# alexkeroro86/SampleNeRFRO

Measured on AMD Instinct MI355X. Metric: rays/sec (train step), higher is better.
Workload: dtype f16x3/fp32-acc

## Files before the change

### include/rnerf.h

```cpp
#ifndef RNERF_H_
#define RNERF_H_

#include <stddef.h>
#include <stdint.h>

#ifdef __cplusplus
extern "C" {
#endif

#define RNERF_VERSION 4

enum rnerf_status {
  RNERF_OK = 0,
  RNERF_ERR_ARG = -1,
  RNERF_ERR_HIP = -2,
  RNERF_ERR_UNSUPPORTED = -3
};

enum rnerf_precision {
  RNERF_PREC_F32 = 0,
  RNERF_PREC_F16X3 = 1,
  RNERF_PREC_BF16X3 = 2,
  RNERF_PREC_F16 = 3,
  RNERF_PREC_BF16 = 4,
  RNERF_PREC_F16X2 = 5,
  RNERF_PREC_F16F8 = 6
};

enum rnerf_backward {
  RNERF_BWD_BF16 = 0,
  RNERF_BWD_F16 = 1,
  RNERF_BWD_F16X3 = 2,
  RNERF_BWD_F16X2 = 2,
  RNERF_BWD_F16X3_LO8 = 4
};

typedef struct rnerf_grid {
  int32_t dims[3];
  double nmin[3];
  double nmax[3];
  int32_t layout;
} rnerf_grid;

enum rnerf_table_layout {
  RNERF_TABLE_REFERENCE = 0,
  RNERF_TABLE_BRICKS = 1
};
size_t rnerf_grid_table_floats(const rnerf_grid* g);

#define RNERF_NERFMLP_PARAMS 595844
#define RNERF_BKGDMLP_PARAMS 56963
#define RNERF_SO3MLP_PARAMS 65411

const char* rnerf_last_error(void);
int rnerf_version(void);
int rnerf_device_cus(void);

int rnerf_grid_prefilter(const float* src, float* dst, float* tmp, const int32_t dims[3], int ksize, double ksigma,
                         void* stream);

int rnerf_grid_build_table(const float* grid, float* table, const rnerf_grid* g, void* stream);

int rnerf_grid_query(const float* table, const rnerf_grid* g, const float* pts, int64_t n, float* out, int32_t* idx,
                     void* stream);

int rnerf_march(const float* table, const rnerf_grid* g, const float* origins, const float* viewdirs, int32_t B,
                double near, double far, int32_t num_nodes, float* path_pd, float* path_dr, float* path_ior,
                int32_t* vox, void* stream);

size_t rnerf_nerfmlp_packed_bytes(int precision);
int rnerf_nerfmlp_pack(const float* params, int precision, void* packed, void* stream);

int rnerf_nerfmlp_forward(const void* packed, int precision, const float* rows_pd, const float* rows_dr,
                          const int32_t* node_of_sample, int32_t S, int32_t B, float* out_raw, int32_t max_workgroups, void* stream);

int rnerf_bkgd_forward(const float* params, const float* dirs, int32_t dir_stride, int64_t n, double rgb_padding,
                       float* out_rgb, void* stream);

int rnerf_composite(const float* raw, const float* rows_pd, const float* rows_dr, const int32_t* node_of_sample,
                    int32_t S, int32_t B, const float* bkgd, int white_bkgd, double rgb_padding, double sigma_bias,
                    float* rgb, float* dist, float* acc, float* trans, float* trans_bkgd, float* weights,
                    float* alpha, int mask_mode, const double* bbox, void* stream);

int rnerf_resample(const float* path_pd, const float* path_dr, int32_t num_nodes, int32_t B, const int32_t* jitter,
                   int32_t S, const float* weights, const float* u, int32_t u_per_ray, int32_t num_fine, float* rows_pd,
                   float* rows_dr, int32_t* node_idx, float* scratch, void* stream);

int rnerf_stratified_u(const uint32_t* key, int32_t B, int32_t num_fine, float* u, void* stream);

int rnerf_voxelize(const double* verts, const int32_t* faces, const int32_t* bin_start, const int32_t* bin_tris, int32_t num_bins,
                   const double* bin_origin_size, const rnerf_grid* g, int32_t num_samples, double ior_inside, double ior_outside,
                   int32_t* count, float* out, int32_t* overflow, void* stream);

int rnerf_voxelize_samples(const double* verts, const int32_t* faces, const int32_t* bin_start, const int32_t* bin_tris, int32_t num_bins,
                           const double* bin_origin_size, const rnerf_grid* g, int32_t num_samples, uint8_t* inside, int32_t* overflow, void* stream);
int rnerf_voxelize_majority(const uint8_t* in_z, const uint8_t* in_x, const uint8_t* in_y, int32_t num_voxels, int32_t num_samples,
                            double ior_inside, double ior_outside, int32_t* count, float* out, void* stream);

int rnerf_so3_query(const float* table, const rnerf_grid* g, const float* so3_params, const float* window10, const float* pts,
                    const float* condition, int64_t n, float* out4, float* pred_grad, void* stream);

size_t rnerf_so3_packed_bytes(void);
int rnerf_march_all(const float* table, const rnerf_grid* g, const float* so3_params, void* so3_packed, const float* window10, const float* origins,
                    const float* viewdirs, int32_t B, double near, double far, int32_t num_nodes, float* path_pd, float* path_dr,
                    float* path_ior, const int32_t* ray_order, void* stream);

int rnerf_generate_rays(const float* camtoworld, int32_t opencv, double fx, double fy, double cx, double cy, double pixel_center,
                        int32_t W, int32_t row0, int32_t rows, float* origins, float* directions, float* viewdirs, void* stream);

int rnerf_sample_batch(const float* camtoworlds, int32_t n_img, int32_t opencv, double fx, double fy, double cx, double cy, double pixel_center,
                       int32_t W, int32_t H, const float* images, int32_t channels, const int64_t* ray_indices, int32_t B, float* origins,
                       float* directions, float* viewdirs, float* pixels, int32_t* bad_count, void* stream);

int rnerf_integrated_pos_enc(const float* rows_pd, const float* rows_dr, const int32_t* node_of_sample, int32_t S, int32_t B, const float* radii,
                             double near, int32_t min_deg, int32_t max_deg, float* out_mean4, float* out_cov4, float* out_enc, void* stream);

int rnerf_loss_reduce(const float* rgb_c, const float* rgb_f, const float* trans_f, const float* trans_bkgd_f,
                      const float* pixels, int32_t B, float* sums, void* stream);

size_t rnerf_env_smooth_sum_floats(int32_t ps);
int rnerf_env_smooth_backward(const float* rgb_env, int32_t ps, double grad_scale, float* d_out, float* loss_sum, void* stream);
int rnerf_train_stats(const float* sums, int32_t B, int32_t two_levels, double bg_scale, const float* env_loss_sum, int32_t ps, double env_on,
                      const float* theta, int64_t n_theta, double frozen_sq, int64_t n_all, float* stats8, void* stream);
int rnerf_theta_sumsq(const float* theta, int64_t n_theta, float* stats8, void* stream);

int rnerf_composite_backward(const float* raw, const float* rows_pd, const float* rows_dr, const int32_t* node_of_sample,
                             int32_t S, int32_t B, const float* bkgd, double rgb_padding, double sigma_bias, const float* rgb,
                             const float* pixels, const float* trans, const float* trans_bkgd, const float* sums,
                             double mse_scale, double bg_scale, float* d_raw, float* d_bkgd, int accumulate_bkgd, int white_bkgd,
                             int mask_mode, const double* bbox, void* stream);

size_t rnerf_nerfmlp_save_bytes(int64_t rows, int backward);
size_t rnerf_nerfmlp_dy_bytes(int64_t rows, int backward);
size_t rnerf_nerfmlp_bwd_packed_bytes(void);
size_t rnerf_nerfmlp_wgrad_workspace_bytes(void);
int rnerf_nerfmlp_forward_train(const void* packed, int precision, const float* rows_pd, const float* rows_dr,
                                const int32_t* node_of_sample, int32_t S, int32_t B, float* out_raw, void* save, int backward,
                                int32_t max_workgroups , void* stream);
int rnerf_nerfmlp_pack_bwd(const float* params, int backward, void* packed_bwd, void* stream);
int rnerf_nerfmlp_dgrad(const void* packed_bwd, const void* packed_fwd, int fwd_precision, int backward, const void* save, const float* d_raw,
                        int64_t rows, void* dy, void* stream);
int rnerf_nerfmlp_wgrad(int fwd_precision, int backward, const void* save, const void* dy, int64_t rows, float* grads, void* workspace,
                        void* stream);

size_t rnerf_bkgd_save_bytes(int64_t n);
size_t rnerf_bkgd_dy_bytes(int64_t n);
int rnerf_bkgd_forward_train(const float* params, const float* dirs, int32_t dir_stride, int64_t n, double rgb_padding,
                             float* out_rgb, void* save, void* stream);
int rnerf_bkgd_backward(const float* params, const void* save, const float* d_out, int64_t n, double rgb_padding, void* dy,
                        float* grads, float* d_dirs, void* stream);

int rnerf_march_all_train(const float* table, const rnerf_grid* g, const float* so3_params, void* so3_packed, const float* window10, const float* origins,
                          const float* viewdirs, int32_t B, double near, double far, int32_t num_nodes, float* path_pd, float* path_dr,
                          float* path_rdn, int32_t* pair_count, int32_t pair_cap, int32_t* pair_id, float* pair_x, float* pair_g,
                          int32_t* pair_of_node, const int32_t* ray_order, void* stream);
size_t rnerf_so3_save_bytes(int64_t n);
size_t rnerf_so3_dy_bytes(int64_t nb);
int rnerf_so3_forward_train(const float* so3_params, const float* window10, const float* pts4, int64_t n, void* save, void* stream);
int rnerf_so3_backward(const float* so3_params, const float* window10, const float* pts4, const void* save, int64_t n_save, const float* d_raw4,
                       int64_t nb, void* dy, float* dx4, float* grads, void* stream);
int rnerf_so3_pair_jacobian(const float* table, const rnerf_grid* g, const float* pair_x, const float* pair_g, const float* raw4, const float* J4,
                            int64_t np, float* A12, float* P12, void* stream);
int rnerf_march_adjoint(const float* table, const rnerf_grid* g, const float* path_pd, const float* path_rdn, const int32_t* pair_of_node,
                        const float* A12, const float* P12, const float* a_pos, const float* a_dir, const int32_t* sample_of_node, int32_t B,
                        double near, double far, int32_t num_nodes, float* v4, void* stream);
int rnerf_nerfmlp_input_grad(const float* params, int backward, const void* dy, const float* rows_pd, const float* rows_dr,
                             const int32_t* node_of_sample, int32_t S, int32_t B, float* d_pos4, float* d_dir4, void* stream);


typedef struct rnerf_model {
  const float* table;
  rnerf_grid grid;
  double near, far;
  int32_t num_coarse;
  int32_t num_fine;
  int32_t num_path;
  int32_t precision;
  int32_t white_bkgd;
  int32_t bd_cut;
  double rgb_padding, sigma_bias;
  double bd_cut_bbox[6];
  const void* packed_coarse;
  const void* packed_fine;
  const float* bkgd_params;
} rnerf_model;

#define RNERF_LEVEL_FLOATS 9

int rnerf_rng_split3(uint32_t* rng_state, uint32_t* keys4, void* stream);
int rnerf_rng_forward(const uint32_t* keys4, int32_t num_coarse, int32_t num_path, int32_t use_random_choice, int32_t* jitter, uint32_t* key_u,
                      void* stream);
int rnerf_stratified_u_dev(const uint32_t* key_dev, int32_t B, int32_t num_fine, float* u, void* stream);

size_t rnerf_forward_workspace_bytes(const rnerf_model* m, int32_t B);
int rnerf_forward(const rnerf_model* m, const float* origins, const float* viewdirs, int32_t B, const int32_t* jitter, const float* u_fine,
                  int32_t u_per_ray, const float* path_pd, const float* path_dr, float* out_coarse, float* out_fine, void* workspace,
                  int32_t max_workgroups, void* stream);

typedef struct rnerf_train_cfg {
  int32_t backward;
  int32_t randomized;
  int32_t use_random_choice;
  int32_t bg_patch_size;
  double bg_weight, bg_smooth_weight, annealed_alpha;
  double frozen_sq;
  int64_t frozen_count;
  void* aux_stream;
  void* grads_stream;
} rnerf_train_cfg;
typedef struct rnerf_prefetch {
  const float* origins;
  const float* viewdirs;
  float* path_pd;
  float* path_dr;
  void* side_stream;
} rnerf_prefetch;
size_t rnerf_train_workspace_bytes(const rnerf_model* m, const rnerf_train_cfg* c, int32_t B);
int rnerf_train_forward_backward(const rnerf_model* m, const rnerf_train_cfg* c, const float* theta, const float* origins, const float* viewdirs,
                                 const float* pixels, const float* env_dirs, int32_t B, const uint32_t* keys4, const int32_t* jitter_override,
                                 const float* u_override, int32_t u_per_ray, const float* path_pd, const float* path_dr, float* grads,
                                 void* workspace, int32_t max_workgroups, const rnerf_prefetch* next, void* stream);

#define RNERF_ADAM_SCRATCH_FLOATS 3076
typedef struct rnerf_adam_cfg {
  double lr_init, lr_final, lr_delay_mult;
  int64_t max_steps, lr_delay_steps;
  double b1, b2, eps;
  double weight_decay_mult, grad_max_val, grad_max_norm;
  int64_t n_all;
  double lr_override;
  int32_t use_lr_override;
  int32_t skip_nonfinite;
} rnerf_adam_cfg;
int rnerf_adam_update(const rnerf_adam_cfg* c, float* theta, float* mu, float* nu, float* grads, int64_t n_theta, const float* frozen_params,
                      int64_t n_frozen, int32_t* step_counter, float* scratch, void* stream);
int rnerf_adam_update_fused(const rnerf_adam_cfg* c, float* theta, float* mu, float* nu, float* grads, int64_t n_theta,
                            const float* frozen_params, int64_t n_frozen, int32_t* step_counter, float* scratch, float* nonfinite_out,
                            void* stream);

int rnerf_graph_begin(void* stream);
int rnerf_graph_end(void* stream, void** graph_exec);
int rnerf_graph_launch(void* graph_exec, void* stream);
int rnerf_graph_destroy(void* graph_exec);
int rnerf_fork(void* main_stream, void* side_stream);
int rnerf_join(void* main_stream, void* side_stream);

size_t rnerf_ssim_workspace_bytes(int64_t n, int32_t H, int32_t W, int32_t C, int32_t filter_size);
int rnerf_ssim(const float* img0, const float* img1, int64_t n, int32_t H, int32_t W, int32_t C, int32_t filter_size, double filter_sigma,
               double max_val, double k1, double k2, float* map, float* mean, void* workspace, void* stream);

size_t rnerf_flip_workspace_bytes(int64_t n, int32_t H, int32_t W, double pixels_per_degree);
int rnerf_flip(const float* reference, const float* test, int64_t n, int32_t H, int32_t W, double pixels_per_degree, float* map,
               float* mean, void* workspace, void* stream);

size_t rnerf_visual_hull_workspace_bytes(int64_t num_views, int32_t height, int32_t width);
int rnerf_visual_hull_pack(const uint8_t* masks, int64_t num_views, int32_t height, int32_t width, void* workspace, void* stream);
int rnerf_visual_hull_count(const uint8_t* masks, int64_t num_views, int32_t height, int32_t width, const double* pv, const rnerf_grid* g,
                            int32_t accumulate, int32_t* count, void* workspace, void* stream);
int rnerf_visual_hull_finalize(const int32_t* count, const rnerf_grid* g, int64_t total_views, double threshold, double ior_inside,
                               double ior_outside, float* out, void* stream);

#ifdef __cplusplus
}
#endif
#endif
```

### samplenerfro_amd/_lib.py

```python
from __future__ import annotations

import ctypes as C
import os
from typing import Optional

HERE = os.path.dirname(os.path.abspath(__file__))
LIB_PATH = os.path.join(HERE, "lib", "librnerf.so")

PREC_F32, PREC_F16X3, PREC_BF16X3, PREC_F16, PREC_BF16, PREC_F16X2, PREC_F16F8 = 0, 1, 2, 3, 4, 5, 6
PRECISIONS = {"f32": PREC_F32, "f16x3": PREC_F16X3, "bf16x3": PREC_BF16X3, "f16": PREC_F16, "bf16": PREC_BF16, "f16x2": PREC_F16X2, "f16f8": PREC_F16F8}
BWD_BF16, BWD_F16, BWD_F16X2 = 0, 1, 2
BWD_F16X3 = BWD_F16X2
BWD_F16X3_LO8 = 4
BACKWARDS = {"f16x3": BWD_F16X3, "f16x3lo8": BWD_F16X3_LO8, "f16": BWD_F16, "bf16": BWD_BF16, "f32": BWD_F16X3, "tf32": BWD_F16}
BACKWARD_NAMES = {BWD_F16X3: "f16x3", BWD_F16X3_LO8: "f16x3lo8", BWD_F16: "f16", BWD_BF16: "bf16"}
TWO_PLANE_BACKWARDS = (BWD_F16X3, BWD_F16X3_LO8)
ABI_VERSION = 4
NERFMLP_PARAMS = 595844
BKGDMLP_PARAMS = 56963
SO3MLP_PARAMS = 65411


class RnerfError(RuntimeError):
    pass


TABLE_LAYOUTS = {"reference": 0, "bricks": 1}


class Grid(C.Structure):
    _fields_ = [("dims", C.c_int32 * 3), ("nmin", C.c_double * 3), ("nmax", C.c_double * 3), ("layout", C.c_int32)]

    @classmethod
    def make(cls, ndim, nmin, nmax, layout="reference") -> "Grid":
        g = cls()
        for i in range(3):
            g.dims[i] = int(ndim[i]); g.nmin[i] = float(nmin[i]); g.nmax[i] = float(nmax[i])
        g.layout = TABLE_LAYOUTS[layout] if isinstance(layout, str) else int(layout)
        return g


class Model(C.Structure):
    _fields_ = [("table", C.c_void_p), ("grid", Grid), ("near", C.c_double), ("far", C.c_double), ("num_coarse", C.c_int32),
                ("num_fine", C.c_int32), ("num_path", C.c_int32), ("precision", C.c_int32), ("white_bkgd", C.c_int32), ("bd_cut", C.c_int32),
                ("rgb_padding", C.c_double), ("sigma_bias", C.c_double), ("bd_cut_bbox", C.c_double * 6), ("packed_coarse", C.c_void_p),
                ("packed_fine", C.c_void_p), ("bkgd_params", C.c_void_p)]


class TrainCfg(C.Structure):
    _fields_ = [("backward", C.c_int32), ("randomized", C.c_int32), ("use_random_choice", C.c_int32), ("bg_patch_size", C.c_int32),
                ("bg_weight", C.c_double), ("bg_smooth_weight", C.c_double), ("annealed_alpha", C.c_double), ("frozen_sq", C.c_double),
                ("frozen_count", C.c_int64), ("aux_stream", C.c_void_p), ("grads_stream", C.c_void_p)]


class AdamCfg(C.Structure):
    _fields_ = [("lr_init", C.c_double), ("lr_final", C.c_double), ("lr_delay_mult", C.c_double), ("max_steps", C.c_int64),
                ("lr_delay_steps", C.c_int64), ("b1", C.c_double), ("b2", C.c_double), ("eps", C.c_double), ("weight_decay_mult", C.c_double),
                ("grad_max_val", C.c_double), ("grad_max_norm", C.c_double), ("n_all", C.c_int64), ("lr_override", C.c_double),
                ("use_lr_override", C.c_int32), ("skip_nonfinite", C.c_int32)]


class Prefetch(C.Structure):
    _fields_ = [("origins", C.c_void_p), ("viewdirs", C.c_void_p), ("path_pd", C.c_void_p), ("path_dr", C.c_void_p), ("side_stream", C.c_void_p)]


LEVEL_FLOATS = 9
ADAM_SCRATCH_FLOATS = 3076
_vp, _i32, _i64, _dbl = C.c_void_p, C.c_int32, C.c_int64, C.c_double
_GP = C.POINTER(Grid)
_MP, _TP, _AP = C.POINTER(Model), C.POINTER(TrainCfg), C.POINTER(AdamCfg)

SIGNATURES = {
    "rnerf_last_error": (C.c_char_p, []),
    "rnerf_version": (C.c_int, []),
    "rnerf_device_cus": (C.c_int, []),
    "rnerf_grid_prefilter": (C.c_int, [_vp, _vp, _vp, C.POINTER(_i32 * 3), C.c_int, _dbl, _vp]),
    "rnerf_grid_table_floats": (C.c_size_t, [_GP]),
    "rnerf_grid_build_table": (C.c_int, [_vp, _vp, _GP, _vp]),
    "rnerf_grid_query": (C.c_int, [_vp, _GP, _vp, _i64, _vp, _vp, _vp]),
    "rnerf_march": (C.c_int, [_vp, _GP, _vp, _vp, _i32, _dbl, _dbl, _i32, _vp, _vp, _vp, _vp, _vp]),
    "rnerf_nerfmlp_packed_bytes": (C.c_size_t, [C.c_int]),
    "rnerf_nerfmlp_pack": (C.c_int, [_vp, C.c_int, _vp, _vp]),
    "rnerf_nerfmlp_forward": (C.c_int, [_vp, C.c_int, _vp, _vp, _vp, _i32, _i32, _vp, _i32, _vp]),
    "rnerf_bkgd_forward": (C.c_int, [_vp, _vp, _i32, _i64, _dbl, _vp, _vp]),
    "rnerf_composite": (C.c_int, [_vp, _vp, _vp, _vp, _i32, _i32, _vp, C.c_int, _dbl, _dbl,
                                  _vp, _vp, _vp, _vp, _vp, _vp, _vp, C.c_int, C.POINTER(C.c_double * 6), _vp]),
    "rnerf_loss_reduce": (C.c_int, [_vp, _vp, _vp, _vp, _vp, _i32, _vp, _vp]),
    "rnerf_env_smooth_sum_floats": (C.c_size_t, [_i32]),
    "rnerf_env_smooth_backward": (C.c_int, [_vp, _i32, _dbl, _vp, _vp, _vp]),
    "rnerf_train_stats": (C.c_int, [_vp, _i32, _i32, _dbl, _vp, _i32, _dbl, _vp, _i64, _dbl, _i64, _vp, _vp]),
    "rnerf_composite_backward": (C.c_int, [_vp, _vp, _vp, _vp, _i32, _i32, _vp, _dbl, _dbl, _vp, _vp, _vp, _vp, _vp, _dbl, _dbl,
                                           _vp, _vp, C.c_int, C.c_int, C.c_int, C.POINTER(C.c_double * 6), _vp]),
    "rnerf_nerfmlp_save_bytes": (C.c_size_t, [_i64, C.c_int]),
    "rnerf_nerfmlp_dy_bytes": (C.c_size_t, [_i64, C.c_int]),
    "rnerf_nerfmlp_bwd_packed_bytes": (C.c_size_t, []),
    "rnerf_nerfmlp_wgrad_workspace_bytes": (C.c_size_t, []),
    "rnerf_nerfmlp_forward_train": (C.c_int, [_vp, C.c_int, _vp, _vp, _vp, _i32, _i32, _vp, _vp, C.c_int, _i32, _vp]),
    "rnerf_nerfmlp_pack_bwd": (C.c_int, [_vp, C.c_int, _vp, _vp]),
    "rnerf_nerfmlp_dgrad": (C.c_int, [_vp, _vp, C.c_int, C.c_int, _vp, _vp, _i64, _vp, _vp]),
    "rnerf_nerfmlp_wgrad": (C.c_int, [C.c_int, C.c_int, _vp, _vp, _i64, _vp, _vp, _vp]),
    "rnerf_voxelize": (C.c_int, [_vp, _vp, _vp, _vp, _i32, _vp, _GP, _i32, _dbl, _dbl, _vp, _vp, _vp, _vp]),
    "rnerf_voxelize_samples": (C.c_int, [_vp, _vp, _vp, _vp, _i32, _vp, _GP, _i32, _vp, _vp, _vp]),
    "rnerf_voxelize_majority": (C.c_int, [_vp, _vp, _vp, _i32, _i32, _dbl, _dbl, _vp, _vp, _vp]),
    "rnerf_so3_query": (C.c_int, [_vp, _GP, _vp, _vp, _vp, _vp, _i64, _vp, _vp, _vp]),
    "rnerf_march_all": (C.c_int, [_vp, _GP, _vp, _vp, _vp, _vp, _vp, _i32, _dbl, _dbl, _i32, _vp, _vp, _vp, _vp, _vp]),
    "rnerf_generate_rays": (C.c_int, [_vp, _i32, _dbl, _dbl, _dbl, _dbl, _dbl, _i32, _i32, _i32, _vp, _vp, _vp, _vp]),
    "rnerf_sample_batch": (C.c_int, [_vp, _i32, _i32, _dbl, _dbl, _dbl, _dbl, _dbl, _i32, _i32, _vp, _i32, _vp, _i32, _vp, _vp, _vp, _vp, _vp, _vp]),
    "rnerf_stratified_u": (C.c_int, [_vp, _i32, _i32, _vp, _vp]),
    "rnerf_bkgd_save_bytes": (C.c_size_t, [_i64]),
    "rnerf_bkgd_dy_bytes": (C.c_size_t, [_i64]),
    "rnerf_bkgd_forward_train": (C.c_int, [_vp, _vp, _i32, _i64, _dbl, _vp, _vp, _vp]),
    "rnerf_bkgd_backward": (C.c_int, [_vp, _vp, _vp, _i64, _dbl, _vp, _vp, _vp, _vp]),
    "rnerf_theta_sumsq": (C.c_int, [_vp, _i64, _vp, _vp]),
    "rnerf_march_all_train": (C.c_int, [_vp, _GP, _vp, _vp, _vp, _vp, _vp, _i32, _dbl, _dbl, _i32, _vp, _vp, _vp, _vp, _i32, _vp, _vp, _vp, _vp, _vp, _vp]),
    "rnerf_so3_packed_bytes": (C.c_size_t, []),
    "rnerf_so3_save_bytes": (C.c_size_t, [_i64]),
    "rnerf_so3_dy_bytes": (C.c_size_t, [_i64]),
    "rnerf_so3_forward_train": (C.c_int, [_vp, _vp, _vp, _i64, _vp, _vp]),
    "rnerf_so3_backward": (C.c_int, [_vp, _vp, _vp, _vp, _i64, _vp, _i64, _vp, _vp, _vp, _vp]),
    "rnerf_so3_pair_jacobian": (C.c_int, [_vp, _GP, _vp, _vp, _vp, _vp, _i64, _vp, _vp, _vp]),
    "rnerf_march_adjoint": (C.c_int, [_vp, _GP, _vp, _vp, _vp, _vp, _vp, _vp, _vp, _vp, _i32, _dbl, _dbl, _i32, _vp, _vp]),
    "rnerf_nerfmlp_input_grad": (C.c_int, [_vp, C.c_int, _vp, _vp, _vp, _vp, _i32, _i32, _vp, _vp, _vp]),
    "rnerf_resample": (C.c_int, [_vp, _vp, _i32, _i32, _vp, _i32, _vp, _vp, _i32, _i32, _vp, _vp, _vp, _vp, _vp]),
    "rnerf_integrated_pos_enc": (C.c_int, [_vp, _vp, _vp, _i32, _i32, _vp, _dbl, _i32, _i32, _vp, _vp, _vp, _vp]),
    "rnerf_rng_split3": (C.c_int, [_vp, _vp, _vp]),
    "rnerf_rng_forward": (C.c_int, [_vp, _i32, _i32, _i32, _vp, _vp, _vp]),
    "rnerf_stratified_u_dev": (C.c_int, [_vp, _i32, _i32, _vp, _vp]),
    "rnerf_forward_workspace_bytes": (C.c_size_t, [_MP, _i32]),
    "rnerf_forward": (C.c_int, [_MP, _vp, _vp, _i32, _vp, _vp, _i32, _vp, _vp, _vp, _vp, _vp, _i32, _vp]),
    "rnerf_train_workspace_bytes": (C.c_size_t, [_MP, _TP, _i32]),
    "rnerf_train_forward_backward": (C.c_int, [_MP, _TP, _vp, _vp, _vp, _vp, _vp, _i32, _vp, _vp, _vp, _i32, _vp, _vp, _vp, _vp, _i32, C.POINTER(Prefetch), _vp]),
    "rnerf_adam_update": (C.c_int, [_AP, _vp, _vp, _vp, _vp, _i64, _vp, _i64, _vp, _vp, _vp]),
    "rnerf_adam_update_fused": (C.c_int, [_AP, _vp, _vp, _vp, _vp, _i64, _vp, _i64, _vp, _vp, _vp, _vp]),
    "rnerf_graph_begin": (C.c_int, [_vp]),
    "rnerf_graph_end": (C.c_int, [_vp, C.POINTER(C.c_void_p)]),
    "rnerf_graph_launch": (C.c_int, [_vp, _vp]),
    "rnerf_graph_destroy": (C.c_int, [_vp]),
    "rnerf_fork": (C.c_int, [_vp, _vp]),
    "rnerf_join": (C.c_int, [_vp, _vp]),
    "rnerf_ssim_workspace_bytes": (C.c_size_t, [_i64, _i32, _i32, _i32, _i32]),
    "rnerf_ssim": (C.c_int, [_vp, _vp, _i64, _i32, _i32, _i32, _i32, _dbl, _dbl, _dbl, _dbl, _vp, _vp, _vp, _vp]),
    "rnerf_flip_workspace_bytes": (C.c_size_t, [_i64, _i32, _i32, _dbl]),
    "rnerf_flip": (C.c_int, [_vp, _vp, _i64, _i32, _i32, _dbl, _vp, _vp, _vp, _vp]),
    "rnerf_visual_hull_workspace_bytes": (C.c_size_t, [_i64, _i32, _i32]),
    "rnerf_visual_hull_pack": (C.c_int, [_vp, _i64, _i32, _i32, _vp, _vp]),
    "rnerf_visual_hull_count": (C.c_int, [_vp, _i64, _i32, _i32, _vp, _GP, _i32, _vp, _vp, _vp]),
    "rnerf_visual_hull_finalize": (C.c_int, [_vp, _GP, _i64, _dbl, _dbl, _dbl, _vp, _vp]),
}

_lib: Optional[C.CDLL] = None


def load(path: Optional[str] = None) -> C.CDLL:
    global _lib
    if _lib is not None and path is None:
        return _lib
    p = path or LIB_PATH
    if not os.path.exists(p):
        raise RnerfError(f"{p} not found: build it with `python -m samplenerfro_amd.build` "
                         "(there is no CPU fallback for the hot path)")
    lib = C.CDLL(p)
    for name, (res, args) in SIGNATURES.items():
        fn = getattr(lib, name)
        fn.restype = res
        fn.argtypes = args
    got = lib.rnerf_version()
    if got != ABI_VERSION:
        raise RnerfError(f"{p} speaks ABI version {got}, this binding was written for {ABI_VERSION} (include/rnerf.h RNERF_VERSION): rebuild with "
                         "`python -m samplenerfro_amd.build --force`")
    if path is None or _lib is None:
        _lib = lib
    return lib


def check(status: int, what: str = "") -> None:
    if status != 0:
        msg = load().rnerf_last_error()
        raise RnerfError(f"{what} failed ({status}): {msg.decode() if msg else '?'}")


def ptr(t) -> Optional[int]:
    if t is None:
        return None
    return t.data_ptr()


def current_stream() -> int:
    import torch
    return torch.cuda.current_stream().cuda_stream
```

### samplenerfro_amd/csrc/bkgd16.hip

```cpp
#include "mfma_ops.h"
#include "bkgd_layout.h"
#include "so3_layout.h"

namespace rnerf {

__device__ __forceinline__ void bkgd16_split2(float a, float b, uint32_t& hi, uint32_t& lo) { split2<true>(a, b, hi, lo); }
__device__ __forceinline__ void bkgd16_split8(const float (&w)[8], uint4& hi, uint4& lo) {
  uint32_t h[4], l[4];
#pragma unroll
  for (int p = 0; p < 4; ++p) bkgd16_split2(w[2 * p], w[2 * p + 1], h[p], l[p]);
  hi = make_uint4(h[0], h[1], h[2], h[3]); lo = make_uint4(l[0], l[1], l[2], l[3]);
}
template <int NS, bool FIRST, typename WF, typename LF, typename XF>
__device__ __forceinline__ void bkgd16_layer(f32x16 (&acc)[4], WF wload, LF live, bool half0, XF xop) {
  constexpr int DEPTH = 2;
  f32x2 w[DEPTH + 1][16];
  auto load = [&](int s, f32x2 (&dst)[16]) {
#pragma unroll
    for (int t = 0; t < 4; ++t)
#pragma unroll
      for (int j = 0; j < 8; ++j)
        if (live(s, j) != 0) dst[4 * t + (j >> 1)][j & 1] = wload(s, t, j);
  };
#pragma unroll
  for (int s = 0; s < DEPTH && s < NS; ++s) load(s, w[s]);
  f32x16 zero;
#pragma unroll
  for (int r = 0; r < 16; ++r) zero[r] = 0.f;
#pragma unroll
  for (int s = 0; s < NS; ++s) {
    if (s + DEPTH < NS) load(s + DEPTH, w[(s + DEPTH) % (DEPTH + 1)]);
    RNERF_PIN();
    uint4 bh, bl;
    xop(s, bh, bl);
#pragma unroll
    for (int t = 0; t < 4; ++t) {
      uint32_t hh[4], ll[4];
#pragma unroll
      for (int p = 0; p < 4; ++p) {
        const int l0 = live(s, 2 * p), l1 = live(s, 2 * p + 1);
        if (l0 == 0 && l1 == 0) { hh[p] = 0u; ll[p] = 0u; continue; }
        f32x2 q = w[s % (DEPTH + 1)][4 * t + p];
        if (l0 == 0) q[0] = 0.f;
        if (l1 == 0) q[1] = 0.f;
        q = q * 256.0f;
        if (l0 == 2) q[0] = half0 ? q[0] : 0.f;
        if (l1 == 2) q[1] = half0 ? q[1] : 0.f;
        bkgd16_split2(q[0], q[1], hh[p], ll[p]);
      }
      const uint4 ah = make_uint4(hh[0], hh[1], hh[2], hh[3]), al = make_uint4(ll[0], ll[1], ll[2], ll[3]);
      acc[t] = mfma16<true>(ah, bh, FIRST && s == 0 ? zero : acc[t]);
      acc[t] = mfma16<true>(ah, bl, acc[t]);
      acc[t] = mfma16<true>(al, bh, acc[t]);
    }
    RNERF_PIN();
  }
}
struct Bkgd16Lane {
  const float* p0;
  const float* prev;
  const float* dir;
  const float* sp;
  bool half0;
};
__device__ __forceinline__ Bkgd16Lane bkgd16_lane(const float* __restrict__ params, int m, int h) {
  return {params + m, params + m + 4 * 128 * h, params + m + 12 * 128 * h, params + m + 2 * 128 * h, h == 0};
}
template <bool BIAS>
__device__ __forceinline__ void bkgd16_prev_layer(f32x16 (&acc)[4], const f32x16 (&x)[4], const Bkgd16Lane& L, int koff, int boff) {
  bkgd16_layer<BIAS ? 9 : 8, true>(acc,
      [&](int s, int t, int j) { return s < 8 ? L.prev[koff + (16 * s + 8 * (j >> 2) + (j & 3)) * 128 + 32 * t] : L.p0[boff + 32 * t]; },
      [&](int s, int j) { return s < 8 ? 1 : (j == 0 ? 2 : 0); }, L.half0,
      [&](int s, uint4& bh, uint4& bl) {
    if (s < 8) {
      float xv[8];
#pragma unroll
      for (int j = 0; j < 8; ++j) xv[j] = x[s >> 1][8 * (s & 1) + j];
      bkgd16_split8(xv, bh, bl);
    } else {
      bh = make_uint4(L.half0 ? 0x3c00u : 0u, 0u, 0u, 0u);
      bl = make_uint4(0u, 0u, 0u, 0u);
    }
  });
}
template <bool FIRST>
__device__ __forceinline__ void bkgd16_dir_layer(f32x16 (&acc)[4], const float (&enc)[14], const Bkgd16Lane& L, int koff, int boff) {
  bkgd16_layer<2, FIRST>(acc,
      [&](int s, int t, int j) {
        const int q = 8 * s + j;
        return q < 12 ? L.dir[koff + (3 + q) * 128 + 32 * t] : (q == 12 ? L.sp[koff + 32 * t] : (q == 13 ? L.p0[koff + 128 + 32 * t] : L.p0[boff + 32 * t]));
      },
      [&](int s, int j) { const int q = 8 * s + j; return q < 13 ? 1 : (q < 15 ? 2 : 0); }, L.half0,
      [&](int s, uint4& bh, uint4& bl) {
    float xv[8];
#pragma unroll
    for (int j = 0; j < 8; ++j) xv[j] = 8 * s + j < 14 ? enc[8 * s + j] : (8 * s + j == 14 && L.half0 ? 1.0f : 0.f);
    bkgd16_split8(xv, bh, bl);
  });
}

template <bool TRAIN>
__global__ void __launch_bounds__(64) bkgd16_fwd_kernel(const float* __restrict__ params, const float* __restrict__ dirs, int dir_stride,
                                                        long long n, float pad_scale, float pad, float* __restrict__ out_rgb,
                                                        float* __restrict__ save) {
  const int lane = threadIdx.x & 63, m = lane & 31, h = lane >> 5;
  long long row = (long long)blockIdx.x * 32 + m;
  const bool ok = row < n;
  if (!ok) row = n - 1;
  const float v0 = dirs[row * dir_stride], v1 = dirs[row * dir_stride + 1], v2 = dirs[row * dir_stride + 2];
  float enc[14];
  const float phase = h ? 1.5707963705062866f : 0.0f;
#pragma unroll
  for (int q = 0; q < 12; ++q) {
    const int d = q / 3, c = q % 3;
    const float x = c == 0 ? v0 : (c == 1 ? v1 : v2);
    enc[q] = sinf(fadd(fmul(x, (float)(1 << d)), phase));
  }
  enc[12] = h ? v2 : v0;
  enc[13] = h ? 0.f : v1;
  auto save_x = [&](int k, const f32x16 (&xx)[4]) {
    if constexpr (TRAIN) {
      if (ok) {
        float* dst = save + (size_t)n * 28 + (size_t)(k - 1) * n * 128 + (size_t)row * 128;
#pragma unroll
        for (int t = 0; t < 4; ++t)
#pragma unroll
          for (int g = 0; g < 4; ++g)
            *(float4*)(dst + 32 * t + 8 * g + 4 * h) = make_float4(xx[t][4 * g], xx[t][4 * g + 1], xx[t][4 * g + 2], xx[t][4 * g + 3]);
      }
    }
  };
  if constexpr (TRAIN) {
    if (ok) {
#pragma unroll
      for (int q = 0; q < 14; ++q) { const int f = h ? dir_feature(q, 1) : dir_feature(q, 0); if (f >= 0) save[(size_t)row * 28 + f] = enc[q]; }
      if (h == 1) save[(size_t)row * 28 + 27] = 0.f;
    }
  }
  constexpr float INV = 1.0f / 256.0f;
  f32x16 acc[4], x[4];
  auto relu_to_x = [&]() {
#pragma unroll
    for (int t = 0; t < 4; ++t)
#pragma unroll
      for (int r = 0; r < 16; ++r) { const float y = acc[t][r] * INV; x[t][r] = y < 0.f ? 0.f : y; }
  };
  const Bkgd16Lane L = bkgd16_lane(params, m, h);
  bkgd16_dir_layer<true>(acc, enc, L, bkgd_koff(0), bkgd_boff(0));
  relu_to_x();
  save_x(1, x);
  bkgd16_prev_layer<true>(acc, x, L, bkgd_koff(1), bkgd_boff(1));
  relu_to_x();
  save_x(2, x);
  bkgd16_prev_layer<true>(acc, x, L, bkgd_koff(2), bkgd_boff(2));
  relu_to_x();
  save_x(3, x);
  bkgd16_prev_layer<false>(acc, x, L, bkgd_koff(3), 0);
  bkgd16_dir_layer<false>(acc, enc, L, bkgd_koff(3) + 128 * 128, bkgd_boff(3));
  relu_to_x();
  if constexpr (TRAIN) save_x(4, x);
  float o[3] = {0.f, 0.f, 0.f};
  const float* __restrict__ k4 = params + bkgd_koff(4);
#pragma unroll
  for (int t = 0; t < 4; ++t)
#pragma unroll
    for (int r = 0; r < 16; ++r) {
      const float v = x[t][r];
      const int f = 32 * t + (r & 3) + 8 * (r >> 2) + 4 * h;
      o[0] = fmaf(v, k4[f * 3 + 0], o[0]); o[1] = fmaf(v, k4[f * 3 + 1], o[1]); o[2] = fmaf(v, k4[f * 3 + 2], o[2]);
    }
#pragma unroll
  for (int c = 0; c < 3; ++c) {
    o[c] = o[c] + __shfl_xor(o[c], 32) + params[bkgd_boff(4) + c];
    o[c] = fsub(fmul(fdiv(1.0f, fadd(1.0f, expf(-o[c]))), pad_scale), pad);
  }
  if (ok && h == 0) {
    out_rgb[3 * row] = o[0]; out_rgb[3 * row + 1] = o[1]; out_rgb[3 * row + 2] = o[2];
    if constexpr (TRAIN) { float* so = save + (size_t)n * (28 + 4 * 128) + (size_t)row * 3; so[0] = o[0]; so[1] = o[1]; so[2] = o[2]; }
  }
}

int launch_bkgd16_fwd(bool train, const float* params, const float* dirs, int dir_stride, long long n, float pad_scale, float pad, float* out_rgb,
                      float* save, hipStream_t st) {
  const dim3 grid((unsigned)((n + 31) / 32));
  if (train) hipLaunchKernelGGL(bkgd16_fwd_kernel<true>, grid, dim3(64), 0, st, params, dirs, dir_stride, n, pad_scale, pad, out_rgb, save);
  else hipLaunchKernelGGL(bkgd16_fwd_kernel<false>, grid, dim3(64), 0, st, params, dirs, dir_stride, n, pad_scale, pad, out_rgb, save);
  RNERF_CHECK_LAUNCH();
  return RNERF_OK;
}

template <bool FIRST>
__device__ __forceinline__ void so3_16_enc_layer(f32x16 (&acc)[4], const float (&enc)[30], const float* __restrict__ pe, const Bkgd16Lane& L, int koff, int boff) {
  bkgd16_layer<4, FIRST>(acc,
      [&](int s, int t, int j) { const int p = 8 * s + j; return p < 30 ? pe[koff + 2 * p * 128 + 32 * t] : L.p0[boff + 32 * t]; },
      [&](int s, int j) { const int p = 8 * s + j; return p < 30 ? 1 : (p == 30 ? 2 : 0); }, L.half0,
      [&](int s, uint4& bh, uint4& bl) {
    float xv[8];
#pragma unroll
    for (int j = 0; j < 8; ++j) { const int p = 8 * s + j; xv[j] = p < 30 ? enc[p < 30 ? p : 0] : ((p == 30 && L.half0) ? 1.0f : 0.f); }
    bkgd16_split8(xv, bh, bl);
  });
}

__global__ void __launch_bounds__(64) so3_16_fwd_train_kernel(const float* __restrict__ params, So3Window win, const float4* __restrict__ pts, long long n,
                                                              float* __restrict__ save) {
  const int lane = threadIdx.x & 63, m = lane & 31, h = lane >> 5;
  long long row = (long long)blockIdx.x * 32 + m;
  const bool ok = row < n;
  if (!ok) row = n - 1;
  const float4 pt = pts[row];
  float enc[30];
  so3_encode(pt.x, pt.y, pt.z, win, h, enc);
  if (ok) {
#pragma unroll
    for (int p = 0; p < 30; ++p) save[(size_t)row * 60 + 2 * p + h] = enc[p];
  }
  auto save_x = [&](int k, const f32x16 (&xx)[4]) {
    so3_store_mask(save, n, row, k, xx, h, ok);
    if (ok) {
      float* dst = save + (size_t)n * 60 + (size_t)(k - 1) * n * 128 + (size_t)row * 128;
#pragma unroll
      for (int t = 0; t < 4; ++t)
#pragma unroll
        for (int g = 0; g < 4; ++g)
          *(float4*)(dst + 32 * t + 8 * g + 4 * h) = make_float4(xx[t][4 * g], xx[t][4 * g + 1], xx[t][4 * g + 2], xx[t][4 * g + 3]);
    }
  };
  constexpr float INV = 1.0f / 256.0f;
  f32x16 acc[4], x[4];
  auto relu_to_x = [&]() {
#pragma unroll
    for (int t = 0; t < 4; ++t)
#pragma unroll
      for (int r = 0; r < 16; ++r) { const float y = acc[t][r] * INV; x[t][r] = y < 0.f ? 0.f : y; }
  };
  const Bkgd16Lane L = bkgd16_lane(params, m, h);
  const float* __restrict__ pe = params + m + 128 * h;
  so3_16_enc_layer<true>(acc, enc, pe, L, so3_koff(0), so3_boff(0));
  relu_to_x();
  save_x(1, x);
  bkgd16_prev_layer<true>(acc, x, L, so3_koff(1), so3_boff(1));
  relu_to_x();
  save_x(2, x);
  bkgd16_prev_layer<true>(acc, x, L, so3_koff(2), so3_boff(2));
  relu_to_x();
  save_x(3, x);
  bkgd16_prev_layer<false>(acc, x, L, so3_koff(3), 0);
  so3_16_enc_layer<false>(acc, enc, pe, L, so3_koff(3) + 128 * 128, so3_boff(3));
  relu_to_x();
  save_x(4, x);
  float o[3] = {0.f, 0.f, 0.f};
  const float* __restrict__ k4 = params + so3_koff(4);
#pragma unroll
  for (int t = 0; t < 4; ++t)
#pragma unroll
    for (int r = 0; r < 16; ++r) {
      const int f = 32 * t + (r & 3) + 8 * (r >> 2) + 4 * h;
      o[0] = fmaf(x[t][r], k4[f * 3 + 0], o[0]); o[1] = fmaf(x[t][r], k4[f * 3 + 1], o[1]); o[2] = fmaf(x[t][r], k4[f * 3 + 2], o[2]);
    }
#pragma unroll
  for (int c = 0; c < 3; ++c) o[c] = o[c] + __shfl_xor(o[c], 32) + params[so3_boff(4) + c];
  if (ok && h == 0) *(float4*)(save + (size_t)n * (60 + 4 * 128) + (size_t)row * 4) = make_float4(o[0], o[1], o[2], 0.f);
}

int launch_so3_16_fwd_train(const float* params, So3Window win, const float* pts4, long long n, float* save, hipStream_t st) {
  hipLaunchKernelGGL(so3_16_fwd_train_kernel, dim3((unsigned)((n + 31) / 32)), dim3(64), 0, st, params, win, (const float4*)pts4, n, save);
  RNERF_CHECK_LAUNCH();
  return RNERF_OK;
}

}
```

### samplenerfro_amd/csrc/bkgd_layout.h

```cpp
#pragma once
#include "nerfmlp_layout.h"

namespace rnerf {

__host__ __device__ constexpr DenseShape bkgd_dense(int d) {
  constexpr DenseShape t[5] = {{27, 128}, {128, 128}, {128, 128}, {155, 128}, {128, 3}};
  return t[d];
}
__host__ __device__ constexpr int bkgd_koff(int d) {
  int o = 0;
  for (int i = 0; i < d; ++i) o += bkgd_dense(i).in * bkgd_dense(i).out + bkgd_dense(i).out;
  return o;
}
__host__ __device__ constexpr int bkgd_boff(int d) { return bkgd_koff(d) + bkgd_dense(d).in * bkgd_dense(d).out; }
static_assert(bkgd_koff(5) == RNERF_BKGDMLP_PARAMS, "bkgd MLP parameter count");

__host__ __device__ constexpr int dir_feature(int q, int h) { return q < 12 ? (h ? 15 + q : 3 + q) : (q == 12 ? (h ? 2 : 0) : (h ? -1 : 1)); }

__host__ __device__ constexpr size_t bkgd_save_floats(long long n) { return (size_t)n * (28 + 4 * 128 + 3); }
__host__ __device__ constexpr size_t bkgd_dy_floats(long long n) { return (size_t)n * (5 * 128) + (size_t)((n + 255) / 256) * RNERF_BKGDMLP_PARAMS; }

int launch_bkgd16_fwd(bool train, const float* params, const float* dirs, int dir_stride, long long n, float pad_scale, float pad, float* out_rgb,
                      float* save, hipStream_t st);

}
```

### samplenerfro_amd/csrc/mlp.hip

```cpp
#include "common.h"
#include "nerfmlp_layout.h"
#include "mfma_ops.h"
#include "bkgd_layout.h"
#include "so3_layout.h"

#include <stdlib.h>
#include <type_traits>
#include <vector>
#include <stdio.h>

namespace rnerf {


#define GLOBAL_AS __attribute__((address_space(1)))
#define LDS_AS __attribute__((address_space(3)))

struct MfmaLayer { int dense, ks, nt, kind; };
__host__ __device__ constexpr MfmaLayer mfma_layer(int l) {
  constexpr MfmaLayer t[10] = {{0, 4, 8, 0},  {1, 16, 8, 1}, {2, 16, 8, 1}, {3, 16, 8, 1}, {4, 16, 8, 1},
                               {5, 20, 8, 2}, {6, 16, 8, 1}, {7, 16, 8, 1}, {9, 16, 8, 1}, {10, 18, 4, 3}};
  return t[l];
}
__host__ __device__ constexpr int layer_blocks_before(int l) {
  int o = 0;
// ... 1548 lines not shown
    }
    wait_vmcnt<0>();
  }
  constexpr size_t ldn = (size_t)NT * 32;
  const int m = lane & 31, h = lane >> 5;
  if (active) {
#pragma unroll
    for (int i = 0; i < TK; ++i)
#pragma unroll
      for (int j = 0; j < TN; ++j)
#pragma unroll
        for (int r = 0; r < 16; ++r) {
          const int row = (r & 3) + 8 * (r >> 2) + 4 * h;
          pg[(size_t)((wk * TK + i) * 32 + row) * ldn + (wn * TN + j) * 32 + m] = acc[i][j][r];
        }
    if constexpr (SH::EXTRA) {
#pragma unroll
      for (int r = 0; r < 16; ++r) {
        const int row = (r & 3) + 8 * (r >> 2) + 4 * h;
        pg[(size_t)((wk * TK + wn) * 32 + row) * ldn + (NT - 1) * 32 + m] = acce[r];
      }
    }
    const float bsum = accb + __shfl_xor(accb, 32);
    if (wk < TN && h == 0) pbias[(wn * TN + wk) * 32 + m] = bsum;
  }
}

template <int KT, int NT> struct WgTr8 {
  static constexpr int NHI = KT + NT, NLX = (KT + 1) / 2, NLD = (NT + 1) / 2;
  static constexpr int NBLK = NHI + NLX + NLD, NDMA = (NBLK + 7) / 8, STEP_BYTES = (NBLK + 1) * 1024;
  static constexpr int LOX = NHI * 1024, LOD = (NHI + NLX) * 1024, SCALES = NBLK * 1024;
};
constexpr int WGTR8_NBUF = 4;
constexpr int wgtr8_lds_bytes() { return WGTR8_NBUF * WgTr8<10, 8>::STEP_BYTES; }
__device__ __forceinline__ int2v tr_read8b(const char* p) {
  typedef __attribute__((address_space(3))) int2v lds_int2;
  return __builtin_amdgcn_ds_read_tr8_b64_v2i32((lds_int2*)p);
}

template <int KT, int NT>
__device__ __forceinline__ void wgrad_body_tr8(const uint4* __restrict__ saved, const uint4* __restrict__ dy, long long R, float* __restrict__ pg,
                                                float* __restrict__ pbias, const WgTrSegs sg, int g, int G, char* smem) {
  using SH = WgTrShape<KT, NT>;
  using L8 = WgTr8<KT, NT>;
  constexpr int TK = SH::TK, TN = SH::TN;
  constexpr int NHI = L8::NHI, NBLK = L8::NBLK, NDMA = L8::NDMA, STEP_BYTES = L8::STEP_BYTES;
  constexpr int WGTR_NBUF = WGTR8_NBUF, AHEAD = WGTR_NBUF - 1;
  const int tid = threadIdx.x, lane = tid & 63;
  const int wave = __builtin_amdgcn_readfirstlane(tid >> 6);
  const int wk = wave / SH::WN, wn = wave % SH::WN;
  const bool active = wave < SH::WK * SH::WN;
  const float* __restrict__ rs = (const float*)(dy + dy_plane_uint4(R, 2));
  const float mref = rs[R];
  const float inv_mref = mref > 0.f ? 1.0f / mref : 0.f;
  auto x_slots = [&](int t, int& s0, int& s1) { s0 = t < sg.KTa ? sg.qx + 2 * t : sg.qx2 + 2 * (t - sg.KTa); s1 = s0 + 1; };
  auto d_slots = [&](int nt, int& s0, int& s1) {
    const int rel = nt < sg.NTa ? 2 * nt : 2 * (nt - sg.NTa);
    const int qb = nt < sg.NTa ? sg.qd : sg.qd2, ks = nt < sg.NTa ? sg.KSd : sg.KSd2;
    s0 = qb + (rel < ks ? rel : ks - 1);
    s1 = qb + (rel + 1 < ks ? rel + 1 : ks - 1);
  };
  const char* sbase[NDMA];
  unsigned tstride[NDMA], hstride[NDMA], voff[NDMA], lds_blk[NDMA];
#pragma unroll
  for (int i = 0; i < NDMA; ++i) {
    int b = wave + 8 * i;
    b = b < NBLK ? b : NBLK - 1;
    lds_blk[i] = (unsigned)b * 1024u;
    if (b < NHI) {
      const int r = lane >> 2, a = (lane >> 1) & 1, h = lane & 1;
      int s0, s1;
      const bool is_x = b < KT;
      if (is_x) x_slots(b, s0, s1); else d_slots(b - KT, s0, s1);
      sbase[i] = (const char*)((is_x ? saved : dy) + sv_addr(__builtin_amdgcn_readfirstlane(s0), 0, 0, 0));
      voff[i] = (unsigned)((sv_addr(a ? __builtin_amdgcn_readfirstlane(s1 - s0) : 0, 0, r, h)) * sizeof(uint4));
      tstride[i] = (unsigned)((is_x ? SAVE_SLOTS : DY_SLOTS) * 64 * sizeof(uint4));
      hstride[i] = (unsigned)(32 * sizeof(uint4));
    } else {
      const int lb = b - NHI;
      const bool is_x = lb < L8::NLX;
      const int t0 = 2 * (is_x ? lb : lb - L8::NLX) + (lane >> 5);
      const int r = (lane & 31) >> 1, a = lane & 1;
      int s0, s1;
      if (is_x) x_slots(t0 < KT ? t0 : KT - 1, s0, s1); else d_slots(t0 < NT ? t0 : NT - 1, s0, s1);
      sbase[i] = is_x ? (const char*)(saved + sv_lo0(R)) : (const char*)(dy + dy_plane_uint4(R, 1));
      voff[i] = (unsigned)(((a ? s1 : s0) * 32 + r) * 16);
      tstride[i] = (unsigned)((is_x ? SAVE_SLOTS : DY_SLOTS) * 32 * 16);
      hstride[i] = 16u * 16u;
    }
  }
  const float* rs_src = rs + 4 * (lane & 3);
  const long long n_t32 = R / 32;
  const int my_tiles = g < n_t32 ? (int)((n_t32 - 1 - g) / G) + 1 : 0;
  const int n_steps = 2 * my_tiles;
  auto issue = [&](int s) {
    const int sc = s < n_steps ? s : n_steps - 1;
    const size_t t32 = (size_t)g + (size_t)(sc >> 1) * G;
    const unsigned ring = (unsigned)(s % WGTR_NBUF) * STEP_BYTES;
#pragma unroll
    for (int i = 0; i < NDMA; ++i)
      glds16_nt_s(sbase[i] + t32 * tstride[i] + (sc & 1) * hstride[i], voff[i], __builtin_amdgcn_readfirstlane(ring + lds_blk[i]));
    if (wave == 0) glds16_nt((const char*)(rs_src + t32 * 32 + (sc & 1) * 16), __builtin_amdgcn_readfirstlane(ring + L8::SCALES));
  };
  const f32x16 zero = {0, 0, 0, 0, 0, 0, 0, 0, 0, 0, 0, 0, 0, 0, 0, 0};
  f32x16 acc[TK][TN], acce = zero;
  float accb = 0.f;
#pragma unroll
  for (int i = 0; i < TK; ++i)
#pragma unroll
    for (int j = 0; j < TN; ++j) acc[i][j] = zero;
  if (n_steps > 0) {
#pragma unroll
    for (int s = 0; s < AHEAD; ++s) issue(s);
    const unsigned lane_off = (unsigned)((8 * (lane >> 5) + ((lane & 15) >> 2)) * 64 + ((lane >> 4) & 1) * 32 + (lane & 3) * 8);
    const unsigned lane_off8 = (unsigned)((8 * (lane >> 5) + ((lane & 15) >> 1)) * 32 + ((lane >> 4) & 1) * 16 + (lane & 1) * 8);
    const int kh = lane >> 5;
    for (int s = 0; s < n_steps; ++s) {
      if (wave == 0) wait_vmcnt<(AHEAD - 1) * (NDMA + 1)>(); else
      wait_vmcnt<(AHEAD - 1) * NDMA>();
      __syncthreads();
      issue(s + AHEAD);
      if (active) {
        const char* ring0 = smem + (s % WGTR_NBUF) * STEP_BYTES;
        const char* ring = ring0 + lane_off;
        const char* ring8 = ring0 + lane_off8;
        const float4 s0 = *(const float4*)(ring0 + L8::SCALES + kh * 32), s1 = *(const float4*)(ring0 + L8::SCALES + kh * 32 + 16);
        const half8 sc8 = {(_Float16)(s0.x * inv_mref), (_Float16)(s0.y * inv_mref), (_Float16)(s0.z * inv_mref), (_Float16)(s0.w * inv_mref),
                           (_Float16)(s1.x * inv_mref), (_Float16)(s1.y * inv_mref), (_Float16)(s1.z * inv_mref), (_Float16)(s1.w * inv_mref)};
        half8 beh, bel;
        if constexpr (SH::EXTRA) {
          beh = tr_read8(ring + (KT + NT - 1) * 1024);
          bel = lo8_decode(tr_read8b(ring8 + L8::LOD + (NT - 1) * 512), LO8_SCALE_D);
        }
        static_assert(SH::WK >= TN, "bias owners");
        auto read_a = [&](int i, half8& h, half8& l) {
          const int t = wk * TK + i;
          h = tr_read8(ring + t * 1024) * sc8;
          l = lo8_decode(tr_read8b(ring8 + L8::LOX + t * 512), LO8_SCALE_X) * sc8;
        };
        auto read_b = [&](int j, half8& h, half8& l) {
          const int nt = wn * TN + j;
          h = tr_read8(ring + (KT + nt) * 1024);
          l = lo8_decode(tr_read8b(ring8 + L8::LOD + nt * 512), LO8_SCALE_D);
        };
        auto dot8 = [&](const half8& x, float c) -> float {
#pragma unroll
          for (int k = 0; k < 4; ++k) c = __builtin_amdgcn_fdot2(half2v{sc8[2 * k], sc8[2 * k + 1]}, half2v{x[2 * k], x[2 * k + 1]}, c, false);
          return c;
        };
        auto bias_row = [&](int j, const half8& h, const half8& l) {
          if (wk == j) { accb = dot8(h, accb); accb = dot8(l, accb); }
        };
        half8 ae_h, ae_l;
        if constexpr (TK > TN) {
          half8 bh[TN], bl[TN];
#pragma unroll
          for (int j = 0; j < TN; ++j) read_b(j, bh[j], bl[j]);
          half8 an_h, an_l;
          read_a(0, an_h, an_l);
#pragma unroll
          for (int i = 0; i < TK; ++i) {
            const half8 ah = an_h, al = an_l;
            if (i + 1 < TK) read_a(i + 1, an_h, an_l);
#pragma unroll
            for (int j = 0; j < TN; ++j) acc[i][j] = mfma_h8(ah, bh[j], acc[i][j]);
#pragma unroll
            for (int j = 0; j < TN; ++j) acc[i][j] = mfma_h8(ah, bl[j], acc[i][j]);
#pragma unroll
            for (int j = 0; j < TN; ++j) acc[i][j] = mfma_h8(al, bh[j], acc[i][j]);
          }
#pragma unroll
          for (int j = 0; j < TN; ++j) bias_row(j, bh[j], bl[j]);
        } else {
          constexpr int NCH = WGTR_NCH < TN ? WGTR_NCH : TN;
          static_assert(TN % NCH == 0, "n-tile chunks");
          half8 ah[TK], al[TK];
#pragma unroll
          for (int i = 0; i < TK; ++i) read_a(i, ah[i], al[i]);
#pragma unroll
          for (int c = 0; c < TN / NCH; ++c) {
            half8 bh[NCH], bl[NCH];
#pragma unroll
            for (int jj = 0; jj < NCH; ++jj) read_b(c * NCH + jj, bh[jj], bl[jj]);
#pragma unroll
            for (int i = 0; i < TK; ++i)
#pragma unroll
              for (int jj = 0; jj < NCH; ++jj) acc[i][c * NCH + jj] = mfma_h8(ah[i], bh[jj], acc[i][c * NCH + jj]);
#pragma unroll
            for (int i = 0; i < TK; ++i)
#pragma unroll
              for (int jj = 0; jj < NCH; ++jj) acc[i][c * NCH + jj] = mfma_h8(ah[i], bl[jj], acc[i][c * NCH + jj]);
#pragma unroll
            for (int i = 0; i < TK; ++i)
#pragma unroll
              for (int jj = 0; jj < NCH; ++jj) acc[i][c * NCH + jj] = mfma_h8(al[i], bh[jj], acc[i][c * NCH + jj]);
#pragma unroll
            for (int jj = 0; jj < NCH; ++jj) bias_row(c * NCH + jj, bh[jj], bl[jj]);
          }
          if constexpr (SH::EXTRA) { ae_h = wn ? ah[1] : ah[0]; ae_l = wn ? al[1] : al[0]; }
        }
        if constexpr (SH::EXTRA) {
          static_assert(!SH::EXTRA || TK <= TN, "the extra tile reads the resident A fragments");
          acce = mfma_h8(ae_h, beh, acce);
          acce = mfma_h8(ae_h, bel, acce);
          acce = mfma_h8(ae_l, beh, acce);
        }
      }
    }
    wait_vmcnt<0>();
  }
  constexpr size_t ldn = (size_t)NT * 32;
  const int m = lane & 31, h = lane >> 5;
  if (active) {
#pragma unroll
    for (int i = 0; i < TK; ++i)
#pragma unroll
      for (int j = 0; j < TN; ++j)
#pragma unroll
        for (int r = 0; r < 16; ++r) {
          const int row = (r & 3) + 8 * (r >> 2) + 4 * h;
          pg[(size_t)((wk * TK + i) * 32 + row) * ldn + (wn * TN + j) * 32 + m] = acc[i][j][r];
        }
    if constexpr (SH::EXTRA) {
#pragma unroll
      for (int r = 0; r < 16; ++r) {
        const int row = (r & 3) + 8 * (r >> 2) + 4 * h;
        pg[(size_t)((wk * TK + wn) * 32 + row) * ldn + (NT - 1) * 32 + m] = acce[r];
      }
    }
    const float bsum = accb + __shfl_xor(accb, 32);
    if (wk < TN && h == 0) pbias[(wn * TN + wk) * 32 + m] = bsum;
  }
}

constexpr int WGRAD_VGPRS = 112;
template <int NP>
__global__ void __launch_bounds__(512) __attribute__((amdgpu_num_vgpr(WGRAD_VGPRS)))
nerfmlp_wgrad_tr_kernel(const uint4* __restrict__ saved, const uint4* __restrict__ dy, long long R, float* __restrict__ workspace, const WgradTable tab,
                        long long* __restrict__ trace) {
  extern __shared__ __attribute__((aligned(16))) char smem[];
  if (trace && threadIdx.x == 0) trace[2 * blockIdx.x] = (long long)__builtin_amdgcn_s_memrealtime();
  int j = 0;
  while ((int)blockIdx.x >= tab.wg0[j + 1]) ++j;
  const WgradJob job = tab.job[j];
  const int g = blockIdx.x - tab.wg0[j], G = tab.wg0[j + 1] - tab.wg0[j];
  const int KT = job.KT, NT = job.NT;
  float* pg = workspace + tab.poff[j] + (size_t)g * (size_t)KT * 32 * NT * 32;
  float* pb = workspace + tab.pboff[j] + (size_t)g * NT * 32;
  const WgTrSegs sg = {tab.qx[j], job.KTa, tab.qx2[j], tab.qd[j], job.NTa, tab.KSd[j], tab.qd2[j], tab.KSd2[j]};
#define RNERF_WGRAD_CASE(KT_, NT_)                                                                                                  \
  if (KT == (KT_) && NT == (NT_)) {                                                                                                 \
    wgrad_body_tr<NP, KT_, NT_>(saved, dy, R, pg, pb, sg, g, G, smem);                                                              \
    if (trace && threadIdx.x == 0) trace[2 * blockIdx.x + 1] = (long long)__builtin_amdgcn_s_memrealtime();                         \
    return;                                                                                                                         \
  }
  RNERF_WGRAD_CASE(8, 8) RNERF_WGRAD_CASE(2, 8) RNERF_WGRAD_CASE(10, 8) RNERF_WGRAD_CASE(8, 9) RNERF_WGRAD_CASE(9, 4) RNERF_WGRAD_CASE(4, 1)
#undef RNERF_WGRAD_CASE
  __builtin_trap();
}

__global__ void __launch_bounds__(512) __attribute__((amdgpu_num_vgpr(WGRAD_VGPRS)))
nerfmlp_wgrad_tr8_kernel(const uint4* __restrict__ saved, const uint4* __restrict__ dy, long long R, float* __restrict__ workspace, const WgradTable tab,
                         long long* __restrict__ trace) {
  extern __shared__ __attribute__((aligned(16))) char smem[];
  if (trace && threadIdx.x == 0) trace[2 * blockIdx.x] = (long long)__builtin_amdgcn_s_memrealtime();
  int j = 0;
  while ((int)blockIdx.x >= tab.wg0[j + 1]) ++j;
  const WgradJob job = tab.job[j];
  const int g = blockIdx.x - tab.wg0[j], G = tab.wg0[j + 1] - tab.wg0[j];
  const int KT = job.KT, NT = job.NT;
  float* pg = workspace + tab.poff[j] + (size_t)g * (size_t)KT * 32 * NT * 32;
  float* pb = workspace + tab.pboff[j] + (size_t)g * NT * 32;
  const WgTrSegs sg = {tab.qx[j], job.KTa, tab.qx2[j], tab.qd[j], job.NTa, tab.KSd[j], tab.qd2[j], tab.KSd2[j]};
#define RNERF_WGRAD_CASE(KT_, NT_)                                                                                                  \
  if (KT == (KT_) && NT == (NT_)) {                                                                                                 \
    wgrad_body_tr8<KT_, NT_>(saved, dy, R, pg, pb, sg, g, G, smem);                                                                 \
    if (trace && threadIdx.x == 0) trace[2 * blockIdx.x + 1] = (long long)__builtin_amdgcn_s_memrealtime();                         \
    return;                                                                                                                         \
  }
  RNERF_WGRAD_CASE(8, 8) RNERF_WGRAD_CASE(2, 8) RNERF_WGRAD_CASE(10, 8) RNERF_WGRAD_CASE(8, 9) RNERF_WGRAD_CASE(9, 4) RNERF_WGRAD_CASE(4, 1)
#undef RNERF_WGRAD_CASE
  __builtin_trap();
}

template <bool X_F16>
__global__ void __launch_bounds__(512)
nerfmlp_wgrad_kernel(const uint4* __restrict__ saved, const uint4* __restrict__ dy, long long R, long long total_rows, int n_chunks,
                      float* __restrict__ workspace, const WgradTable tab) {
  extern __shared__ __attribute__((aligned(16))) char smem[];
  int j = 0;
  while ((int)blockIdx.x >= tab.wg0[j + 1]) ++j;
  const int qx = tab.qx[j], KSx = tab.KSx[j], qd = tab.qd[j], KSd = tab.KSd[j];
  const int g = blockIdx.x - tab.wg0[j], G = tab.wg0[j + 1] - tab.wg0[j];
  const int KT = KSx >> 1, NT = (KSd + 1) >> 1;
  float* pg = workspace + tab.poff[j] + (size_t)g * (size_t)KT * 32 * NT * 32;
  float* pb = workspace + tab.pboff[j] + (size_t)g * NT * 32;
#define RNERF_WGRAD_CASE(KT_, KSD_)                                                                                                 \
  if (KSx == 2 * (KT_) && KSd == (KSD_)) { wgrad_body<X_F16, KT_, KSD_>(saved, dy, R, total_rows, n_chunks, pg, pb, qx, qd, g, G, smem); return; }
  RNERF_WGRAD_CASE(8, 16) RNERF_WGRAD_CASE(2, 16) RNERF_WGRAD_CASE(8, 1) RNERF_WGRAD_CASE(8, 8) RNERF_WGRAD_CASE(1, 8) RNERF_WGRAD_CASE(4, 1)
#undef RNERF_WGRAD_CASE
  __builtin_trap();
}

__global__ void __launch_bounds__(256) wgrad_reduce_kernel(const float* __restrict__ workspace, const WgradTable tab, float* __restrict__ grads,
                                                           const float* __restrict__ out_scale) {
  const float osc = out_scale ? *out_scale : 1.0f;
  const int jb = blockIdx.y;
  const WgradJob job = tab.job[jb];
  const int n_wg = tab.wg0[jb + 1] - tab.wg0[jb];
  const float* __restrict__ partial = workspace + tab.poff[jb];
  const float* __restrict__ partial_bias = workspace + tab.pboff[jb];
  const int ldn = job.NT * 32, rows = job.KT * 32;
  const int e = blockIdx.x * blockDim.x + threadIdx.x;
  auto out_feature = [&](int J, int& dense) -> int {
    int nt = J >> 5;
    const int c = J & 31, a = c >> 4, hh = (c >> 3) & 1, j = c & 7;
    const bool segb = nt >= job.NTa;
    const int dkind = segb ? job.dkind2 : job.dkind;
    dense = segb ? job.dense2 : job.dense;
    if (segb) nt -= job.NTa;
    if (dkind == 0) { const int n = prev_feature(2 * nt + a, hh, j); return n < nerf_dense(dense).out ? n : -1; }
    if (a != 0 || hh != 0 || nt != 0) return -1;
    if (dkind == 1) return j == 0 ? 0 : -1;
    return (j >= 1 && j <= 3) ? j - 1 : -1;
  };
  auto sum_over = [&](const float* __restrict__ p, size_t stride) -> float {
    float s0 = 0.f, s1 = 0.f, s2 = 0.f, s3 = 0.f;
    int g = 0;
    for (; g + 4 <= n_wg; g += 4) { s0 += p[(size_t)g * stride]; s1 += p[(size_t)(g + 1) * stride]; s2 += p[(size_t)(g + 2) * stride]; s3 += p[(size_t)(g + 3) * stride]; }
    for (; g < n_wg; ++g) s0 += p[(size_t)g * stride];
    return (s0 + s1) + (s2 + s3);
  };
  if (e < rows * ldn) {
    const int I = e / ldn, J = e % ldn;
    int kt = I >> 5;
    const int c = I & 31, a = c >> 4, hh = (c >> 3) & 1, j = c & 7;
    const bool segb = kt >= job.KTa;
    const int xkind = segb ? job.xkind2 : job.xkind, row_off = segb ? job.row_off2 : job.row_off;
    if (segb) kt -= job.KTa;
    const int s = 2 * kt + a;
    int fin = xkind == 1 ? prev_feature(s, hh, j) : (xkind == 0 ? pe_feature(8 * s + j, hh) : view_feature(8 * s + j, hh));
    int dense;
    const int fout = out_feature(J, dense);
    if (fin >= 0 && fout >= 0) {
      fin += row_off;
      if (fin < nerf_dense(dense).in) grads[nerf_koff(dense) + fin * nerf_dense(dense).out + fout] = sum_over(partial + e, (size_t)rows * ldn) * osc;
    }
  }
  if (job.write_bias && e < ldn) {
    int dense;
    const int fout = out_feature(e, dense);
    if (fout >= 0 && (e >> 5) < job.NTa) grads[nerf_boff(dense) + fout] = sum_over(partial_bias + e, (size_t)ldn) * osc;
    if (job.bias_sigma && e == 0) grads[nerf_boff(8)] = sum_over(partial_bias, (size_t)ldn) * osc;
  }
}

template <int NSTEP, int NT, typename WF, typename XF>
__device__ __forceinline__ void mfma_f32_stream(f32x16* acc, WF wload, XF xop) {
  constexpr int BS = 4, NB = (NSTEP + BS - 1) / BS;
  float w[2][BS * NT];
#pragma unroll
  for (int i = 0; i < BS; ++i)
#pragma unroll
    for (int t = 0; t < NT; ++t) w[0][i * NT + t] = i < NSTEP ? wload(i, t) : 0.f;
#pragma unroll
  for (int b = 0; b < NB; ++b) {
    if (b + 1 < NB) {
#pragma unroll
      for (int i = 0; i < BS; ++i)
#pragma unroll
        for (int t = 0; t < NT; ++t) w[(b + 1) & 1][i * NT + t] = (b + 1) * BS + i < NSTEP ? wload((b + 1) * BS + i, t) : 0.f;
    }
    RNERF_PIN();
#pragma unroll
    for (int i = 0; i < BS; ++i) {
      if (b * BS + i < NSTEP) {
#pragma unroll
        for (int t = 0; t < NT; ++t) acc[t] = __builtin_amdgcn_mfma_f32_32x32x2f32(w[b & 1][i * NT + t], xop(b * BS + i), acc[t], 0, 0, 0);
      }
    }
    RNERF_PIN();
  }
}

template <int NSTEP, int NT, typename WF4, typename XF>
__device__ __forceinline__ void mfma_f32_stream4(f32x16* acc, WF4 wload4, XF xop) {
  static_assert(NSTEP % 4 == 0, "whole batches");
  constexpr int NB = NSTEP / 4;
  float4 w[2][NT];
#pragma unroll
  for (int t = 0; t < NT; ++t) w[0][t] = wload4(0, t);
#pragma unroll
  for (int b = 0; b < NB; ++b) {
    if (b + 1 < NB) {
#pragma unroll
      for (int t = 0; t < NT; ++t) w[(b + 1) & 1][t] = wload4(b + 1, t);
    }
    RNERF_PIN();
#pragma unroll
    for (int i = 0; i < 4; ++i)
#pragma unroll
      for (int t = 0; t < NT; ++t) {
        const float4 q = w[b & 1][t];
        acc[t] = __builtin_amdgcn_mfma_f32_32x32x2f32(i == 0 ? q.x : (i == 1 ? q.y : (i == 2 ? q.z : q.w)), xop(4 * b + i), acc[t], 0, 0, 0);
      }
    RNERF_PIN();
  }
}

__device__ __forceinline__ void small_init_bias(f32x16 (&acc)[4], const float* __restrict__ bias, int h) {
#pragma unroll
  for (int t = 0; t < 4; ++t)
#pragma unroll
    for (int r = 0; r < 16; ++r) acc[t][r] = bias[32 * t + (r & 3) + 8 * (r >> 2) + 4 * h];
}

__device__ __forceinline__ void small_prev_layer(f32x16 (&acc)[4], const f32x16 (&x)[4], const float* __restrict__ kern, int m, int h) {
  const float* __restrict__ kl = kern + 4 * h * 128 + m;
  mfma_f32_stream<64, 4>(acc, [&](int st, int t) { return kl[(32 * (st >> 4) + (st & 3) + 8 * ((st & 15) >> 2)) * 128 + 32 * t]; },
                         [&](int st) { return x[st >> 4][st & 15]; });
}

__device__ __forceinline__ void so3_enc_layer(f32x16 (&acc)[4], const float (&enc)[30], const float* __restrict__ kern, int m, int h) {
  const float* __restrict__ kl = kern + h * 128 + m;
  mfma_f32_stream<30, 4>(acc, [&](int p, int t) { return kl[2 * p * 128 + 32 * t]; }, [&](int p) { return enc[p]; });
}

__device__ __forceinline__ void so3_eval(const float* __restrict__ params, float px, float py, float pz, const So3Window& win, int m, int h,
                                         float (&raw)[3]) {
  float enc[30];
  const float HALF_PI = 1.5707963705062866f;
#pragma unroll
  for (int p = 0; p < 30; ++p) {
    const int d = p / 3, k = p % 3;
    const float x = k == 0 ? (h ? py : px) : (k == 1 ? (h ? px : pz) : (h ? pz : py));
    const float phase = k == 0 ? 0.f : (k == 1 ? (h ? HALF_PI : 0.f) : HALF_PI);
    const float xb = fmul(x, (float)(1 << d));
    enc[p] = fmul(sinf(k == 0 ? xb : fadd(xb, phase)), win.w[d]);
  }
  f32x16 acc[4], x[4];
  small_init_bias(acc, params + so3_boff(0), h);
  so3_enc_layer(acc, enc, params + so3_koff(0), m, h);
#pragma unroll
  for (int t = 0; t < 4; ++t)
#pragma unroll
    for (int r = 0; r < 16; ++r) x[t][r] = fmaxf(acc[t][r], 0.f);
#pragma unroll 1
  for (int l = 1; l <= 2; ++l) {
    small_init_bias(acc, params + (l == 1 ? so3_boff(1) : so3_boff(2)), h);
    small_prev_layer(acc, x, params + (l == 1 ? so3_koff(1) : so3_koff(2)), m, h);
#pragma unroll
    for (int t = 0; t < 4; ++t)
#pragma unroll
      for (int r = 0; r < 16; ++r) x[t][r] = fmaxf(acc[t][r], 0.f);
  }
  small_init_bias(acc, params + so3_boff(3), h);
  small_prev_layer(acc, x, params + so3_koff(3), m, h);
  so3_enc_layer(acc, enc, params + so3_koff(3) + 128 * 128, m, h);
  float o[3] = {0.f, 0.f, 0.f};
  const float* __restrict__ k4 = params + so3_koff(4);
#pragma unroll
  for (int t = 0; t < 4; ++t)
#pragma unroll
    for (int r = 0; r < 16; ++r) {
      const float v = fmaxf(acc[t][r], 0.f);
      const int f = 32 * t + (r & 3) + 8 * (r >> 2) + 4 * h;
      o[0] = fmaf(v, k4[f * 3 + 0], o[0]); o[1] = fmaf(v, k4[f * 3 + 1], o[1]); o[2] = fmaf(v, k4[f * 3 + 2], o[2]);
    }
#pragma unroll
  for (int c = 0; c < 3; ++c) raw[c] = o[c] + __shfl_xor(o[c], 32) + params[so3_boff(4) + c];
}

constexpr int kSo3KSteps = 16;
constexpr int kSo3Blocks = kSo3KSteps * 8;
constexpr float SO3_WSCALE = 256.f;
__host__ __device__ constexpr int so3s_row(int ks, int g, int j, int* layer) {
  const int l = ks < 2 ? 0 : (ks < 6 ? 1 : (ks < 10 ? 2 : 3));
  const int s = ks - (l == 0 ? 0 : (l == 1 ? 2 : (l == 2 ? 6 : 10)));
  *layer = l;
  const bool enc = l == 0 || (l == 3 && s >= 4);
  if (enc) { const int f = 32 * (l == 0 ? s : s - 4) + 8 * g + j; return f < 60 ? (l == 0 ? f : 128 + f) : -1; }
  return 32 * s + (j < 4 ? 4 * g + j : 16 + 4 * g + (j - 4));
}

__global__ void so3_pack16_kernel(const float* __restrict__ params, uint4* __restrict__ packed) {
  const int gid = blockIdx.x * blockDim.x + threadIdx.x;
  if (gid >= kSo3Blocks * 64) return;
  const int blk = gid >> 6, lane = gid & 63;
  const int ks = blk >> 3, t = blk & 7;
  const int n_out = 16 * t + (lane & 15), g = lane >> 4;
  float w[8];
  for (int j = 0; j < 8; ++j) {
    int l = 0;
    const int row = so3s_row(ks, g, j, &l);
    w[j] = row < 0 ? 0.f : params[(l == 0 ? so3_koff(0) : (l == 1 ? so3_koff(1) : (l == 2 ? so3_koff(2) : so3_koff(3)))) + row * 128 + n_out] * SO3_WSCALE;
  }
  uint32_t hi[4], lo[4];
  for (int p = 0; p < 4; ++p) split2<true>(w[2 * p], w[2 * p + 1], hi[p], lo[p]);
  packed[(size_t)blk * 128 + lane] = make_uint4(hi[0], hi[1], hi[2], hi[3]);
  packed[(size_t)blk * 128 + 64 + lane] = make_uint4(lo[0], lo[1], lo[2], lo[3]);
}

struct So3Ops { uint4 h, l; };
__device__ __forceinline__ So3Ops so3_split_ops(const float (&x)[8]) {
  uint32_t hh[4], ll[4];
#pragma unroll
  for (int p = 0; p < 4; ++p) split2<true>(x[2 * p], x[2 * p + 1], hh[p], ll[p]);
  So3Ops o; o.h = make_uint4(hh[0], hh[1], hh[2], hh[3]); o.l = make_uint4(ll[0], ll[1], ll[2], ll[3]);
  return o;
}

struct So3Shared {
  uint4 enc[2][2][64];
  uint4 x[3][4][2][64];
  float4 out[4][16];
  float4 pos[16];
  float bias[4][128];
  float k4[128][4];
  float tail[16];
  int done;
};

typedef float f32x4 __attribute__((ext_vector_type(4)));
__device__ __forceinline__ f32x4 so3_mfma16(const uint4 a, const uint4 b, const f32x4 c) {
  typedef _Float16 h8 __attribute__((ext_vector_type(8)));
  return __builtin_amdgcn_mfma_f32_16x16x32_f16(__builtin_bit_cast(h8, a), __builtin_bit_cast(h8, b), c, 0, 0, 0);
}

__device__ __forceinline__ void so3_shared_init(So3Shared& sh, const float* __restrict__ params, const So3Window& win, int tid) {
  for (int i = tid; i < 4 * 128; i += 256) { const int l = i >> 7, n = i & 127; sh.bias[l][n] = params[(l == 0 ? so3_boff(0) : (l == 1 ? so3_boff(1) : (l == 2 ? so3_boff(2) : so3_boff(3)))) + n]; }
  for (int i = tid; i < 128 * 3; i += 256) sh.k4[i / 3][i % 3] = params[so3_koff(4) + i];
  if (tid < 3) sh.tail[tid] = params[so3_boff(4) + tid];
  if (tid < 10) sh.tail[4 + tid] = win.w[tid];
  if (tid == 0) sh.done = 0;
}

__device__ __forceinline__ void so3_eval_wg(So3Shared& sh, const uint4 (&wh)[kSo3KSteps][2], const uint4 (&wl)[kSo3KSteps][2], int wave, int lane) {
  const int c = lane & 15, g = lane >> 4;
  const float HALF_PI = 1.5707963705062866f;
  const f32x4 zero = {0, 0, 0, 0};
  constexpr float INV = 1.0f / SO3_WSCALE;
  const float4 pt = sh.pos[c];
  {
    const int s = wave >> 1, j0 = 4 * (wave & 1);
    float v[4];
#pragma unroll
    for (int j = 0; j < 4; ++j) {
      const int f = 32 * s + 8 * g + j0 + j;
      const bool in = f < 60;
      const int fc = in ? f : 0;
      const int d = fc / 6, jj = fc - 6 * d, c3 = jj >= 3 ? jj - 3 : jj;
      const float x = c3 == 0 ? pt.x : (c3 == 1 ? pt.y : pt.z);
      const float xb = fmul(x, (float)(1 << d));
      const float e = fmul(pe_sin(jj >= 3 ? fadd(xb, HALF_PI) : xb), sh.tail[4 + d]);
      v[j] = in ? e : 0.f;
    }
    uint32_t h0, l0, h1, l1;
    split2<true>(v[0], v[1], h0, l0); split2<true>(v[2], v[3], h1, l1);
    uint2* eh = (uint2*)&sh.enc[s][0][lane] + (wave & 1);
    uint2* el = (uint2*)&sh.enc[s][1][lane] + (wave & 1);
    *eh = make_uint2(h0, h1); *el = make_uint2(l0, l1);
  }
  __syncthreads();
  f32x4 a0 = zero, a1 = zero;
  auto kstep = [&](int ks, const uint4 bh, const uint4 bl) {
    a0 = so3_mfma16(wh[ks][0], bh, a0); a1 = so3_mfma16(wh[ks][1], bh, a1);
    a0 = so3_mfma16(wh[ks][0], bl, a0); a1 = so3_mfma16(wh[ks][1], bl, a1);
    a0 = so3_mfma16(wl[ks][0], bh, a0); a1 = so3_mfma16(wl[ks][1], bh, a1);
  };
  auto enc_layer = [&](int ks0) {
    uint4 eh[2], el[2];
#pragma unroll
    for (int s = 0; s < 2; ++s) { eh[s] = sh.enc[s][0][lane]; el[s] = sh.enc[s][1][lane]; }
    RNERF_PIN();
#pragma unroll
    for (int s = 0; s < 2; ++s) kstep(ks0 + s, eh[s], el[s]);
  };
  auto hand_over = [&](int l) {
    const float4 b0 = *(const float4*)&sh.bias[l][32 * wave + 4 * g], b1 = *(const float4*)&sh.bias[l][32 * wave + 16 + 4 * g];
    float v[8];
    v[0] = fmaxf(fmaf(a0[0], INV, b0.x), 0.f); v[1] = fmaxf(fmaf(a0[1], INV, b0.y), 0.f); v[2] = fmaxf(fmaf(a0[2], INV, b0.z), 0.f); v[3] = fmaxf(fmaf(a0[3], INV, b0.w), 0.f);
    v[4] = fmaxf(fmaf(a1[0], INV, b1.x), 0.f); v[5] = fmaxf(fmaf(a1[1], INV, b1.y), 0.f); v[6] = fmaxf(fmaf(a1[2], INV, b1.z), 0.f); v[7] = fmaxf(fmaf(a1[3], INV, b1.w), 0.f);
    const So3Ops o = so3_split_ops(v);
    sh.x[l][wave][0][lane] = o.h; sh.x[l][wave][1][lane] = o.l;
  };
  auto layer = [&](int l, int ks0) {
    uint4 bh[4], bl[4];
#pragma unroll
    for (int s = 0; s < 4; ++s) { bh[s] = sh.x[l][s][0][lane]; bl[s] = sh.x[l][s][1][lane]; }
    RNERF_PIN();
    a0 = zero; a1 = zero;
#pragma unroll
    for (int s = 0; s < 4; ++s) kstep(ks0 + s, bh[s], bl[s]);
  };
  enc_layer(0);
  hand_over(0);
  __syncthreads();
  layer(0, 2);
  hand_over(1);
  __syncthreads();
  layer(1, 6);
  hand_over(2);
  __syncthreads();
  layer(2, 10);
  enc_layer(14);
  float o[3] = {0.f, 0.f, 0.f};
#pragma unroll
  for (int j = 0; j < 8; ++j) {
    const int f = 32 * wave + (j < 4 ? 4 * g + j : 16 + 4 * g + (j - 4));
    const float v = fmaxf(fmaf(j < 4 ? a0[j & 3] : a1[j & 3], INV, sh.bias[3][f]), 0.f);
    const float4 k = *(const float4*)&sh.k4[f][0];
    o[0] = fmaf(v, k.x, o[0]); o[1] = fmaf(v, k.y, o[1]); o[2] = fmaf(v, k.z, o[2]);
  }
#pragma unroll
  for (int q = 0; q < 3; ++q) { o[q] = o[q] + __shfl_xor(o[q], 16); o[q] = o[q] + __shfl_xor(o[q], 32); }
  if (g == 0) sh.out[wave][c] = make_float4(o[0], o[1], o[2], 0.f);
  __syncthreads();
}

__device__ __forceinline__ void so3_rotate(const float (&raw)[3], const float (&g)[3], float (&pred)[3]) {
  const float theta = fsqrt(fmaxf(fadd(fadd(fmul(raw[0], raw[0]), fmul(raw[1], raw[1])), fmul(raw[2], raw[2])), 1e-6f));
  const float e[3] = {fdiv(raw[0], theta), fdiv(raw[1], theta), fdiv(raw[2], theta)};
  const float a = fsqrt(fmaxf(fadd(fadd(fmul(g[0], g[0]), fmul(g[1], g[1])), fmul(g[2], g[2])), 1e-6f));
  const float v[3] = {fdiv(g[0], a), fdiv(g[1], a), fdiv(g[2], a)};
  const float ct = cosf(theta), st = sinf(theta);
  const float cr[3] = {fsub(fmul(e[1], v[2]), fmul(e[2], v[1])), fsub(fmul(e[2], v[0]), fmul(e[0], v[2])), fsub(fmul(e[0], v[1]), fmul(e[1], v[0]))};
  const float dot = fadd(fadd(fmul(e[0], v[0]), fmul(e[1], v[1])), fmul(e[2], v[2]));
  const float k = fmul(fsub(1.0f, ct), dot);
#pragma unroll
  for (int c = 0; c < 3; ++c) pred[c] = fmul(a, fadd(fadd(fmul(ct, v[c]), fmul(st, cr[c])), fmul(k, e[c])));
}

__global__ void __launch_bounds__(64) so3_query_kernel(const float4* __restrict__ table, GridParams gp, const float* __restrict__ params,
                                                       So3Window win, const float* __restrict__ pts, const float* __restrict__ cond, long long n,
                                                       float4* __restrict__ out4, float* __restrict__ pred_out) {
  const int lane = threadIdx.x & 63, m = lane & 31, h = lane >> 5;
  long long row = (long long)blockIdx.x * 32 + m;
  const bool ok = row < n;
  if (!ok) row = n - 1;
  const float px = pts[3 * row], py = pts[3 * row + 1], pz = pts[3 * row + 2];
  const float4 c = trilinear(table, gp, px, py, pz, nullptr);
  float raw[3], pred[3];
  so3_eval(params, px, py, pz, win, m, h, raw);
  const float g[3] = {cond ? cond[3 * row] : c.y, cond ? cond[3 * row + 1] : c.z, cond ? cond[3 * row + 2] : c.w};
  so3_rotate(raw, g, pred);
  if (ok && h == 0) { out4[row] = c; pred_out[3 * row] = pred[0]; pred_out[3 * row + 1] = pred[1]; pred_out[3 * row + 2] = pred[2]; }
}

__global__ void __launch_bounds__(256, 1) march_all_kernel(const float4* __restrict__ table4, GridParams gp, const float* __restrict__ params,
                                                          const uint4* __restrict__ packed16, So3Window win, const float* __restrict__ origins, const float* __restrict__ viewdirs,
                                                          int B, float near, float step, int num_nodes, float4* __restrict__ path_pd4,
                                                          float4* __restrict__ path_dr4, float4* __restrict__ path_ior4,
                                                          float4* __restrict__ path_rdn4, int* __restrict__ pair_count, int pair_cap,
                                                          int2* __restrict__ pair_id, float4* __restrict__ pair_x4, float4* __restrict__ pair_g4,
                                                          int* __restrict__ pair_of_node, const int* __restrict__ ray_order) {
  __shared__ So3Shared sh;
  const int lane = threadIdx.x & 63;
// ... 479 lines not shown
  }
  if (with_safe && safe_stream_offset(precision) != 0)
    hipLaunchKernelGGL(nerfmlp_pack_kernel<RNERF_PREC_BF16X3>, dim3(grid), dim3(block), 0, st, params, (char*)packed + safe_stream_offset(precision));
  RNERF_CHECK_LAUNCH();
  return RNERF_OK;
}
}

extern "C" int rnerf_nerfmlp_pack(const float* params, int precision, void* packed, void* stream) {
  RNERF_CHECK_ARG(params && packed, "rnerf_nerfmlp_pack: null pointer");
  RNERF_CHECK_ARG(prec_ok(precision), "rnerf_nerfmlp_pack: unsupported precision %d", precision);
  RNERF_CHECK_ARG(((uintptr_t)packed & 15) == 0, "rnerf_nerfmlp_pack: packed must be 16-byte aligned");
  return nerfmlp_pack_impl(params, precision, packed, true, (hipStream_t)stream, true);
}

constexpr size_t SAVE_QUEUE_BYTES = 8192;
static size_t save_payload_bytes(long long padded, bool with_lo) {
  return (size_t)(SAVE_TOTAL + (with_lo ? SAVE_SLOTS : 0)) * (size_t)padded * 2 * sizeof(uint4);
}

template <int PREC, int MODE = 0, int TRAIN = 0>
static int launch_fwd_mode(const void* packed, const float* rows_pd, const float* rows_dr, const int32_t* node_of_sample, int32_t B,
                           long long total_rows, float* out_raw, hipStream_t st, void* save = nullptr, int max_wg = 0, const float* gate = nullptr,
                           int gate_skip_if = 0) {
  using PP = Prec<PREC>;
  const int n_tiles = (int)((total_rows + 255) / 256);
  int dev = 0, cus = 0;
  RNERF_CHECK_HIP(hipGetDevice(&dev));
  RNERF_CHECK_HIP(hipDeviceGetAttribute(&cus, hipDeviceAttributeMultiprocessorCount, dev));
  const int lim = (max_wg > 0 && max_wg < cus) ? max_wg : cus;
  if constexpr (MODE == 0 && (PREC == RNERF_PREC_F16X3 || PREC == RNERF_PREC_F16F8)) {
    static const bool half_ok = [] { const char* e = RNERF_ENV("RNERF_FWD_HALF_TILES"); return !(e && e[0] == '0'); }();
    if (half_ok && 2 * n_tiles <= lim) {
      const size_t lds1 = 2 * (size_t)PP::SLAB;
      static DeviceOnce attr1_set;
      if (attr1_set.need()) {
        RNERF_CHECK_HIP(hipFuncSetAttribute((const void*)nerfmlp_fwd_kernel<PREC, 0, TRAIN, true>, hipFuncAttributeMaxDynamicSharedMemorySize, (int)lds1));
        attr1_set.set();
      }
      hipLaunchKernelGGL((nerfmlp_fwd_kernel<PREC, 0, TRAIN, true>), dim3(2 * n_tiles), dim3(256), lds1, st, (const char*)packed, (const float4*)rows_pd,
                         (const float4*)rows_dr, node_of_sample, B, total_rows, 2 * n_tiles, (float4*)out_raw, (uint4*)save, (long long)n_tiles * 256,
                         (int*)nullptr, gate, gate_skip_if);
      RNERF_CHECK_LAUNCH();
      return RNERF_OK;
    }
  }
  const int grid = n_tiles < lim ? n_tiles : lim;
  const size_t lds = 2 * (size_t)PP::SLAB + 4 * 32768;
  static DeviceOnce attr_set;
  if (attr_set.need()) {
    RNERF_CHECK_HIP(hipFuncSetAttribute((const void*)nerfmlp_fwd_kernel<PREC, MODE, TRAIN>, hipFuncAttributeMaxDynamicSharedMemorySize, (int)lds));
    attr_set.set();
  }
  int* tileq = nullptr;
  if (TRAIN != 0 && grid < cus && grid < n_tiles) {
    tileq = (int*)((char*)save + save_payload_bytes((long long)n_tiles * 256, TRAIN >= 2));
    RNERF_CHECK_HIP(hipMemsetAsync(tileq, 0, sizeof(int), st));
  }
  hipLaunchKernelGGL((nerfmlp_fwd_kernel<PREC, MODE, TRAIN>), dim3(grid), dim3(256), lds, st, (const char*)packed, (const float4*)rows_pd,
                     (const float4*)rows_dr, node_of_sample, B, total_rows, n_tiles, (float4*)out_raw, (uint4*)save,
                     (long long)n_tiles * 256, tileq, gate, gate_skip_if);
  RNERF_CHECK_LAUNCH();
  return RNERF_OK;
}

template <int PREC>
static int launch_fwd(const void* packed, const float* rows_pd, const float* rows_dr, const int32_t* node_of_sample, int32_t B,
                      long long total_rows, float* out_raw, hipStream_t st, int max_wg, const float* gate = nullptr, int gate_skip_if = 0) {
  return launch_fwd_mode<PREC>(packed, rows_pd, rows_dr, node_of_sample, B, total_rows, out_raw, st, nullptr, max_wg, gate, gate_skip_if);
}

extern "C" int rnerf_nerfmlp_forward(const void* packed, int precision, const float* rows_pd, const float* rows_dr,
                                     const int32_t* node_of_sample, int32_t S, int32_t B, float* out_raw, int32_t max_workgroups,
                                     void* stream) {
  RNERF_CHECK_ARG(packed && rows_pd && rows_dr && out_raw, "rnerf_nerfmlp_forward: null pointer");
  RNERF_CHECK_ARG(max_workgroups >= 0, "rnerf_nerfmlp_forward: max_workgroups must be >= 0");
  RNERF_CHECK_ARG(prec_ok(precision), "rnerf_nerfmlp_forward: unsupported precision %d", precision);
  RNERF_CHECK_ARG(S >= 1 && B >= 1, "rnerf_nerfmlp_forward: need S >= 1 and B >= 1");
  RNERF_CHECK_ARG((((uintptr_t)packed | (uintptr_t)rows_pd | (uintptr_t)rows_dr | (uintptr_t)out_raw) & 15) == 0,
                  "rnerf_nerfmlp_forward: buffers must be 16-byte aligned");
  const long long total = (long long)S * B;
  hipStream_t st = (hipStream_t)stream;
  switch (precision) {
    case RNERF_PREC_F32: return launch_fwd_f32(packed, rows_pd, rows_dr, node_of_sample, B, total, out_raw, st);
    case RNERF_PREC_F16X3:
      RNERF_TRY_(launch_fwd<RNERF_PREC_F16X3>(packed, rows_pd, rows_dr, node_of_sample, B, total, out_raw, st, max_workgroups));
      return launch_fwd_mode<RNERF_PREC_BF16X3, 512>((const char*)packed + safe_stream_offset(precision), rows_pd, rows_dr, node_of_sample, B, total, out_raw, st, nullptr, max_workgroups);
    case RNERF_PREC_F16X2:
      RNERF_TRY_(launch_fwd<RNERF_PREC_F16X2>(packed, rows_pd, rows_dr, node_of_sample, B, total, out_raw, st, max_workgroups));
      return launch_fwd_mode<RNERF_PREC_BF16X3, 512>((const char*)packed + safe_stream_offset(precision), rows_pd, rows_dr, node_of_sample, B, total, out_raw, st, nullptr, max_workgroups);
    case RNERF_PREC_F16F8: {
      const float* flag = (const float*)((const char*)packed + Prec<RNERF_PREC_F16F8>::STREAM_BYTES) + AUX_FLAG;
      RNERF_TRY_(launch_fwd<RNERF_PREC_F16F8>(packed, rows_pd, rows_dr, node_of_sample, B, total, out_raw, st, max_workgroups, flag, 1));
      RNERF_TRY_(launch_fwd<RNERF_PREC_F16X3>((const char*)packed + kF8Fallback, rows_pd, rows_dr, node_of_sample, B, total, out_raw, st, max_workgroups, flag, 0));
      return launch_fwd_mode<RNERF_PREC_BF16X3, 512>((const char*)packed + safe_stream_offset(precision), rows_pd, rows_dr, node_of_sample, B, total, out_raw, st, nullptr, max_workgroups);
    }
    case RNERF_PREC_BF16X3: return launch_fwd<RNERF_PREC_BF16X3>(packed, rows_pd, rows_dr, node_of_sample, B, total, out_raw, st, max_workgroups);
    case RNERF_PREC_F16:
      RNERF_TRY_(launch_fwd<RNERF_PREC_F16>(packed, rows_pd, rows_dr, node_of_sample, B, total, out_raw, st, max_workgroups));
      return launch_fwd_mode<RNERF_PREC_BF16X3, 512>((const char*)packed + safe_stream_offset(precision), rows_pd, rows_dr, node_of_sample, B, total, out_raw, st, nullptr, max_workgroups);
    default: return launch_fwd<RNERF_PREC_BF16>(packed, rows_pd, rows_dr, node_of_sample, B, total, out_raw, st, max_workgroups);
  }
}

static bool bwd_ok(int b) { return b == RNERF_BWD_BF16 || b == RNERF_BWD_F16 || b == RNERF_BWD_F16X2 || b == RNERF_BWD_F16X3_LO8; }
static bool bwd_two_planes(int b) { return b == RNERF_BWD_F16X2 || b == RNERF_BWD_F16X3_LO8; }
static bool train_combo_ok(int precision, int backward) {
  return precision == RNERF_PREC_F16X3 || (precision == RNERF_PREC_F16 && !bwd_two_planes(backward)) ||
         (precision == RNERF_PREC_BF16X3 && backward == RNERF_BWD_BF16);
}
static size_t train_stream_bytes(int precision) {
  return precision == RNERF_PREC_F16 ? Prec<RNERF_PREC_F16>::STREAM_BYTES : (precision == RNERF_PREC_BF16X3 ? Prec<RNERF_PREC_BF16X3>::STREAM_BYTES : Prec<RNERF_PREC_F16X3>::STREAM_BYTES);
}

extern "C" size_t rnerf_nerfmlp_save_bytes(int64_t rows, int backward) {
  const int64_t padded = (rows + 255) / 256 * 256;
  return save_payload_bytes(padded, bwd_two_planes(backward)) + SAVE_QUEUE_BYTES;
}

extern "C" int rnerf_nerfmlp_forward_train(const void* packed, int precision, const float* rows_pd, const float* rows_dr,
                                           const int32_t* node_of_sample, int32_t S, int32_t B, float* out_raw, void* save,
                                           int backward, int32_t max_workgroups, void* stream) {
  RNERF_CHECK_ARG(packed && rows_pd && rows_dr && out_raw && save, "rnerf_nerfmlp_forward_train: null pointer");
  RNERF_CHECK_ARG(max_workgroups >= 0, "rnerf_nerfmlp_forward_train: max_workgroups must be >= 0");
  RNERF_CHECK_ARG(bwd_ok(backward), "rnerf_nerfmlp_forward_train: unknown backward mode %d", backward);
  RNERF_CHECK_ARG(train_combo_ok(precision, backward),
                  "rnerf_nerfmlp_forward_train: the training forward is built for precision f16x3, f16 with the single-plane backward modes, and bf16x3 with backward bf16");
  RNERF_CHECK_ARG(S >= 1 && B >= 1, "rnerf_nerfmlp_forward_train: need S >= 1 and B >= 1");
  RNERF_CHECK_ARG((((uintptr_t)packed | (uintptr_t)rows_pd | (uintptr_t)rows_dr | (uintptr_t)out_raw | (uintptr_t)save) & 15) == 0,
                  "rnerf_nerfmlp_forward_train: buffers must be 16-byte aligned");
  const long long total = (long long)S * B;
  hipStream_t st = (hipStream_t)stream;
  if (backward == RNERF_BWD_F16X2) return launch_fwd_mode<RNERF_PREC_F16X3, 0, 2>(packed, rows_pd, rows_dr, node_of_sample, B, total, out_raw, st, save, max_workgroups);
  if (backward == RNERF_BWD_F16X3_LO8) return launch_fwd_mode<RNERF_PREC_F16X3, 0, 3>(packed, rows_pd, rows_dr, node_of_sample, B, total, out_raw, st, save, max_workgroups);
  if (precision == RNERF_PREC_BF16X3) return launch_fwd_mode<RNERF_PREC_BF16X3, 0, 1>(packed, rows_pd, rows_dr, node_of_sample, B, total, out_raw, st, save, max_workgroups);
  if (precision == RNERF_PREC_F16) return launch_fwd_mode<RNERF_PREC_F16, 0, 1>(packed, rows_pd, rows_dr, node_of_sample, B, total, out_raw, st, save, max_workgroups);
  return launch_fwd_mode<RNERF_PREC_F16X3, 0, 1>(packed, rows_pd, rows_dr, node_of_sample, B, total, out_raw, st, save, max_workgroups);
}

extern "C" size_t rnerf_nerfmlp_bwd_packed_bytes(void) { return (size_t)kBwdBlocks * 2 * 1024; }
extern "C" size_t rnerf_nerfmlp_dy_bytes(int64_t rows, int backward) {
  const int64_t padded = (rows + 255) / 256 * 256;
  const int np = bwd_two_planes(backward) ? 2 : 1;
  return dy_plane_uint4(padded, np) * sizeof(uint4) + (backward == RNERF_BWD_BF16 ? 0 : ((size_t)padded + 4) * sizeof(float));
}

extern "C" int rnerf_nerfmlp_pack_bwd(const float* params, int backward, void* packed_bwd, void* stream) {
  RNERF_CHECK_ARG(params && packed_bwd, "rnerf_nerfmlp_pack_bwd: null pointer");
  RNERF_CHECK_ARG(bwd_ok(backward), "rnerf_nerfmlp_pack_bwd: unknown backward mode %d", backward);
  const int threads = kBwdBlocks * 64;
  if (backward == RNERF_BWD_BF16)
    hipLaunchKernelGGL(nerfmlp_pack_bwd_kernel<RNERF_PREC_BF16X3>, dim3((threads + 255) / 256), dim3(256), 0, (hipStream_t)stream, params, (char*)packed_bwd);
  else
    hipLaunchKernelGGL(nerfmlp_pack_bwd_kernel<RNERF_PREC_F16X3>, dim3((threads + 255) / 256), dim3(256), 0, (hipStream_t)stream, params, (char*)packed_bwd);
  RNERF_CHECK_LAUNCH();
  return RNERF_OK;
}

void* rnerf::nerfmlp_dgrad_scale_ref(int backward, void* dy, int64_t rows) {
  const long long R = (rows + 255) / 256 * 256;
  if (bwd_two_planes(backward)) return (char*)dy + dy_plane_uint4(R, Bwd<RNERF_BWD_F16X2>::NP) * sizeof(uint4) + (size_t)R * sizeof(float);
  if (backward == RNERF_BWD_F16) return (char*)dy + dy_plane_uint4(R, Bwd<RNERF_BWD_F16>::NP) * sizeof(uint4) + (size_t)R * sizeof(float);
  return nullptr;
}

template <int BWD>
static int launch_dgrad(const void* packed_bwd, const float* fwd_aux, const void* save, const float* d_raw, int64_t rows, void* dy, hipStream_t st,
                        bool zero_ref = true, bool allow_half = true) {
  using PB = Prec<Bwd<BWD>::PREC>;
  const int n_tiles = (int)((rows + 255) / 256);
  int dev = 0, cus = 0;
  RNERF_CHECK_HIP(hipGetDevice(&dev));
  RNERF_CHECK_HIP(hipDeviceGetAttribute(&cus, hipDeviceAttributeMultiprocessorCount, dev));
  const int grid = n_tiles < cus ? n_tiles : cus;
  const size_t lds = 2 * (size_t)PB::SLAB + 4 * 32768;
  static DeviceOnce attr_set;
  if (attr_set.need()) {
    RNERF_CHECK_HIP(hipFuncSetAttribute((const void*)nerfmlp_dgrad_kernel<BWD>, hipFuncAttributeMaxDynamicSharedMemorySize, (int)lds));
    attr_set.set();
  }
  const long long R = (long long)n_tiles * 256;
  if (Bwd<BWD>::F16 && zero_ref) RNERF_CHECK_HIP(hipMemsetAsync(nerfmlp_dgrad_scale_ref(BWD == kBwdF16OnePass ? RNERF_BWD_F16 : BWD, dy, rows), 0, 4 * sizeof(float), st));
  if constexpr (BWD == RNERF_BWD_F16X2 || BWD == RNERF_BWD_F16 || BWD == kBwdF16OnePass || BWD == RNERF_BWD_F16X3_LO8) {
    static const int half_lim = [] { const char* e = RNERF_ENV("RNERF_DGRAD_HALF_TILES"); return e ? atoi(e) : -1; }();
    if (allow_half && half_lim != 0 && 2 * n_tiles <= (half_lim > 1 ? half_lim : cus)) {
      const size_t lds1 = 2 * (size_t)PB::SLAB;
      static DeviceOnce attr1_set;
      if (attr1_set.need()) {
        RNERF_CHECK_HIP(hipFuncSetAttribute((const void*)nerfmlp_dgrad_kernel<BWD, true>, hipFuncAttributeMaxDynamicSharedMemorySize, (int)lds1));
        attr1_set.set();
      }
      hipLaunchKernelGGL((nerfmlp_dgrad_kernel<BWD, true>), dim3(2 * n_tiles), dim3(256), lds1, st, (const char*)packed_bwd, fwd_aux, (const uint4*)save, R,
                         (const float4*)d_raw, (long long)rows, 2 * n_tiles, (uint4*)dy);
      RNERF_CHECK_LAUNCH();
      return RNERF_OK;
    }
  }
  hipLaunchKernelGGL(nerfmlp_dgrad_kernel<BWD>, dim3(grid), dim3(256), lds, st, (const char*)packed_bwd, fwd_aux, (const uint4*)save, R,
                     (const float4*)d_raw, (long long)rows, n_tiles, (uint4*)dy);
  RNERF_CHECK_LAUNCH();
  return RNERF_OK;
}

namespace rnerf {
int nerfmlp_dgrad_impl(const void* packed_bwd, const void* packed_fwd, int fwd_precision, int backward, const void* save, const float* d_raw, int64_t rows,
                       void* dy, bool zero_ref, bool allow_half, hipStream_t st) {
  RNERF_CHECK_ARG(packed_bwd && packed_fwd && save && d_raw && dy, "rnerf_nerfmlp_dgrad: null pointer");
  RNERF_CHECK_ARG(train_combo_ok(fwd_precision, backward), "rnerf_nerfmlp_dgrad: forward precision must be f16x3 (f16 with a single-plane backward mode; bf16x3 with backward bf16)");
  RNERF_CHECK_ARG(bwd_ok(backward), "rnerf_nerfmlp_dgrad: unknown backward mode %d", backward);
  RNERF_CHECK_ARG(rows >= 1, "rnerf_nerfmlp_dgrad: rows must be >= 1");
  const float* fwd_aux = (const float*)((const char*)packed_fwd + train_stream_bytes(fwd_precision));
  if (backward == RNERF_BWD_F16X2) return launch_dgrad<RNERF_BWD_F16X2>(packed_bwd, fwd_aux, save, d_raw, rows, dy, st, zero_ref, allow_half);
  if (backward == RNERF_BWD_F16X3_LO8) return launch_dgrad<RNERF_BWD_F16X3_LO8>(packed_bwd, fwd_aux, save, d_raw, rows, dy, st, zero_ref, allow_half);
  if (backward == RNERF_BWD_F16 && fwd_precision == RNERF_PREC_F16) return launch_dgrad<kBwdF16OnePass>(packed_bwd, fwd_aux, save, d_raw, rows, dy, st, zero_ref, allow_half);
  if (backward == RNERF_BWD_F16) return launch_dgrad<RNERF_BWD_F16>(packed_bwd, fwd_aux, save, d_raw, rows, dy, st, zero_ref, allow_half);
  return launch_dgrad<RNERF_BWD_BF16>(packed_bwd, fwd_aux, save, d_raw, rows, dy, st, zero_ref, allow_half);
}
}

extern "C" int rnerf_nerfmlp_dgrad(const void* packed_bwd, const void* packed_fwd, int fwd_precision, int backward, const void* save,
                                   const float* d_raw, int64_t rows, void* dy, void* stream) {
  return nerfmlp_dgrad_impl(packed_bwd, packed_fwd, fwd_precision, backward, save, d_raw, rows, dy, true, true, (hipStream_t)stream);
}

struct WgradPlan { int qx, KSx, qd, KSd; WgradJob job; int qx2, qd2, KSd2; };
static constexpr WgradJob job1(int dense, int xkind, int row_off, int dkind, int KT, int NT, int wb, int bias_sigma = 0) {
  return WgradJob{dense, xkind, row_off, dkind, KT, NT, wb, KT, 0, 0, NT, 0, 0, bias_sigma};
}
static const WgradPlan kWgradPlan[15] = {
    {SAVE_PE, 4, 0, 16, job1(0, 0, 0, 0, 2, 8, 1), 0, 0, 0},
    {SAVE_L1 + 0, 16, 16, 16, job1(1, 1, 0, 0, 8, 8, 1), 0, 0, 0},   {SAVE_L1 + 16, 16, 32, 16, job1(2, 1, 0, 0, 8, 8, 1), 0, 0, 0},
    {SAVE_L1 + 32, 16, 48, 16, job1(3, 1, 0, 0, 8, 8, 1), 0, 0, 0},  {SAVE_L1 + 48, 16, 64, 16, job1(4, 1, 0, 0, 8, 8, 1), 0, 0, 0},
    {SAVE_L1 + 64, 16, 80, 16, job1(5, 1, 0, 0, 8, 8, 1), 0, 0, 0},  {SAVE_PE, 4, 80, 16, job1(5, 0, 256, 0, 2, 8, 0), 0, 0, 0},
    {SAVE_L1 + 80, 16, 96, 16, job1(6, 1, 0, 0, 8, 8, 1), 0, 0, 0},  {SAVE_L1 + 96, 16, 112, 16, job1(7, 1, 0, 0, 8, 8, 1), 0, 0, 0},
    {SAVE_L1 + 112, 16, 128, 16, job1(9, 1, 0, 0, 8, 8, 1), 0, 0, 0}, {SAVE_L1 + 112, 16, DY_HEADS, 1, job1(8, 1, 0, 1, 8, 1, 1), 0, 0, 0},
    {SAVE_L1 + 128, 16, DY_L9, 8, job1(10, 1, 0, 0, 8, 4, 1), 0, 0, 0}, {SAVE_VIEW, 2, DY_L9, 8, job1(10, 2, 256, 0, 1, 4, 0), 0, 0, 0},
    {SAVE_RGBIN, 8, DY_HEADS, 1, job1(11, 1, 0, 2, 4, 1, 1), 0, 0, 0},
    {0, 0, 0, 0, job1(0, 0, 0, 0, 0, 0, 0), 0, 0, 0}};
static const WgradPlan kWgradPlanTr[12] = {
    {SAVE_PE, 4, 0, 16, job1(0, 0, 0, 0, 2, 8, 1), 0, 0, 0},
    {SAVE_L1 + 0, 16, 16, 16, job1(1, 1, 0, 0, 8, 8, 1), 0, 0, 0},   {SAVE_L1 + 16, 16, 32, 16, job1(2, 1, 0, 0, 8, 8, 1), 0, 0, 0},
    {SAVE_L1 + 32, 16, 48, 16, job1(3, 1, 0, 0, 8, 8, 1), 0, 0, 0},  {SAVE_L1 + 48, 16, 64, 16, job1(4, 1, 0, 0, 8, 8, 1), 0, 0, 0},
    {SAVE_L1 + 64, 20, 80, 16, WgradJob{5, 1, 0, 0, 10, 8, 1,  8,  0,  256,  8, 0, 0, 0}, SAVE_PE, 0, 0},
    {SAVE_L1 + 80, 16, 96, 16, job1(6, 1, 0, 0, 8, 8, 1), 0, 0, 0},  {SAVE_L1 + 96, 16, 112, 16, job1(7, 1, 0, 0, 8, 8, 1), 0, 0, 0},
    {SAVE_L1 + 112, 16, 128, 16, WgradJob{9, 1, 0, 0, 8, 9, 1, 8, 0, 0,  8,  8,  1, 0}, 0, DY_HEADS, 1},
    {SAVE_L1 + 128, 18, DY_L9, 8, WgradJob{10, 1, 0, 0, 9, 4, 1,  8,  2,  256, 4, 0, 0, 0}, SAVE_VIEW, 0, 0},
    {SAVE_RGBIN, 8, DY_HEADS, 1, job1(11, 1, 0, 2, 4, 1, 1,  1), 0, 0, 0},
    {0, 0, 0, 0, job1(0, 0, 0, 0, 0, 0, 0), 0, 0, 0}};

static size_t build_wgrad_table(int cus, WgradTable& t, bool legacy, int mult = 0) {
  const WgradPlan* plan = legacy ? kWgradPlan : kWgradPlanTr;
  int n = 0;
  double cost[16], total = 0;
  for (; plan[n].KSx != 0; ++n) {
    const WgradJob& jb = plan[n].job;
    cost[n] = legacy ? 2.0 * jb.KT * jb.NT + 2 * (jb.KT + jb.NT) + 16 : jb.KT + jb.NT + 1;
    total += cost[n];
  }
  t.n = n;
  const int budget = (mult > 0 ? mult : (legacy ? 4 : 2)) * cus;
  size_t off = 0;
  int wg = 0;
  for (int i = 0; i < n; ++i) {
    const WgradPlan& p = plan[i];
    int share = (int)(budget * cost[i] / total + 0.5);
    if (share < 8) share = 8;
    t.qx[i] = p.qx; t.KSx[i] = p.KSx; t.qd[i] = p.qd; t.KSd[i] = p.KSd; t.job[i] = p.job;
    t.qx2[i] = p.qx2; t.qd2[i] = p.qd2; t.KSd2[i] = p.KSd2;
    t.wg0[i] = wg; wg += share;
    t.poff[i] = (long long)off; off += (size_t)share * p.job.KT * 32 * p.job.NT * 32;
    t.pboff[i] = (long long)off; off += (size_t)share * p.job.NT * 32;
  }
  t.wg0[n] = wg;
  return off;
}

static int device_cus() {
  int dev = 0, cus = 256;
  if (hipGetDevice(&dev) == hipSuccess) hipDeviceGetAttribute(&cus, hipDeviceAttributeMultiprocessorCount, dev);
  return cus;
}

constexpr long long kWgradSmallRows = 24576;
struct WgradTables { WgradTable legacy, tr, tr_small; size_t partial_floats; int max_wgs; };
static const WgradTables& wgrad_tables() {
  static const WgradTables tables = [] {
    WgradTables w;
    const size_t a = build_wgrad_table(device_cus(), w.legacy, true), b = build_wgrad_table(device_cus(), w.tr, false);
    const size_t s = build_wgrad_table(device_cus(), w.tr_small, false, 1);
    w.partial_floats = a > b ? a : b;
    if (s > w.partial_floats) w.partial_floats = s;
    w.max_wgs = w.legacy.wg0[w.legacy.n] > w.tr.wg0[w.tr.n] ? w.legacy.wg0[w.legacy.n] : w.tr.wg0[w.tr.n];
    if (w.tr_small.wg0[w.tr_small.n] > w.max_wgs) w.max_wgs = w.tr_small.wg0[w.tr_small.n];
    return w;
  }();
  return tables;
}

extern "C" size_t rnerf_nerfmlp_wgrad_workspace_bytes(void) {
  const WgradTables& w = wgrad_tables();
  return w.partial_floats * sizeof(float) + (size_t)w.max_wgs * 2 * sizeof(long long);
}

extern "C" int rnerf_nerfmlp_wgrad(int fwd_precision, int backward, const void* save, const void* dy, int64_t rows, float* grads, void* workspace,
                                   void* stream) {
  RNERF_CHECK_ARG(save && dy && grads && workspace, "rnerf_nerfmlp_wgrad: null pointer");
  RNERF_CHECK_ARG(train_combo_ok(fwd_precision, backward), "rnerf_nerfmlp_wgrad: forward precision must be f16x3 (f16 with a single-plane backward mode; bf16x3 with backward bf16)");
  RNERF_CHECK_ARG(bwd_ok(backward), "rnerf_nerfmlp_wgrad: unknown backward mode %d", backward);
  RNERF_CHECK_ARG(rows >= 1, "rnerf_nerfmlp_wgrad: rows must be >= 1");
  const WgradTables& w = wgrad_tables();
  static DeviceOnce ready;
  if (ready.need()) {
    RNERF_CHECK_HIP(hipFuncSetAttribute((const void*)nerfmlp_wgrad_kernel<true>, hipFuncAttributeMaxDynamicSharedMemorySize, 131072));
    RNERF_CHECK_HIP(hipFuncSetAttribute((const void*)nerfmlp_wgrad_kernel<false>, hipFuncAttributeMaxDynamicSharedMemorySize, 131072));
    RNERF_CHECK_HIP(hipFuncSetAttribute((const void*)nerfmlp_wgrad_tr_kernel<1>, hipFuncAttributeMaxDynamicSharedMemorySize, wgtr_lds_bytes<1>()));
    RNERF_CHECK_HIP(hipFuncSetAttribute((const void*)nerfmlp_wgrad_tr_kernel<2>, hipFuncAttributeMaxDynamicSharedMemorySize, wgtr_lds_bytes<2>()));
    RNERF_CHECK_HIP(hipFuncSetAttribute((const void*)nerfmlp_wgrad_tr8_kernel, hipFuncAttributeMaxDynamicSharedMemorySize, wgtr8_lds_bytes()));
    ready.set();
  }
  const long long R = (rows + 255) / 256 * 256;
  hipStream_t st = (hipStream_t)stream;
  const float* out_scale = nullptr;
  static const bool tracing = RNERF_ENV("RNERF_WGRAD_TRACE") != nullptr;
  long long* trace = tracing ? (long long*)((char*)workspace + w.partial_floats * sizeof(float)) : nullptr;
  const WgradTable& tab = backward == RNERF_BWD_BF16 ? w.legacy : (rows <= kWgradSmallRows ? w.tr_small : w.tr);
  if (backward == RNERF_BWD_BF16) {
    const int n_chunks = (int)((rows + 127) / 128);
    if (fwd_precision == RNERF_PREC_BF16X3)
      hipLaunchKernelGGL(nerfmlp_wgrad_kernel<false>, dim3(tab.wg0[tab.n]), dim3(512), 131072, st, (const uint4*)save, (const uint4*)dy, R,
                         (long long)rows, n_chunks, (float*)workspace, tab);
    else
      hipLaunchKernelGGL(nerfmlp_wgrad_kernel<true>, dim3(tab.wg0[tab.n]), dim3(512), 131072, st, (const uint4*)save, (const uint4*)dy, R,
                         (long long)rows, n_chunks, (float*)workspace, tab);
  } else if (backward == RNERF_BWD_F16) {
    hipLaunchKernelGGL(nerfmlp_wgrad_tr_kernel<1>, dim3(tab.wg0[tab.n]), dim3(512), wgtr_lds_bytes<1>(), st, (const uint4*)save, (const uint4*)dy, R,
                       (float*)workspace, tab, trace);
    out_scale = (const float*)((const uint4*)dy + dy_plane_uint4(R, 1)) + R;
  } else if (backward == RNERF_BWD_F16X3_LO8) {
    hipLaunchKernelGGL(nerfmlp_wgrad_tr8_kernel, dim3(tab.wg0[tab.n]), dim3(512), wgtr8_lds_bytes(), st, (const uint4*)save, (const uint4*)dy, R,
                       (float*)workspace, tab, trace);
    out_scale = (const float*)((const uint4*)dy + dy_plane_uint4(R, 2)) + R;
  } else {
    hipLaunchKernelGGL(nerfmlp_wgrad_tr_kernel<2>, dim3(tab.wg0[tab.n]), dim3(512), wgtr_lds_bytes<2>(), st, (const uint4*)save, (const uint4*)dy, R,
                       (float*)workspace, tab, trace);
    out_scale = (const float*)((const uint4*)dy + dy_plane_uint4(R, 2)) + R;
  }
  int max_elems = 0;
  for (int j = 0; j < tab.n; ++j) max_elems = tab.job[j].KT * tab.job[j].NT * 1024 > max_elems ? tab.job[j].KT * tab.job[j].NT * 1024 : max_elems;
  hipLaunchKernelGGL(wgrad_reduce_kernel, dim3((max_elems + 255) / 256, tab.n), dim3(256), 0, st, (const float*)workspace, tab, grads, out_scale);
  RNERF_CHECK_LAUNCH();
  if (trace && backward != RNERF_BWD_BF16) {
    const int n_wg = tab.wg0[tab.n];
    std::vector<long long> h(2 * (size_t)n_wg);
    RNERF_CHECK_HIP(hipStreamSynchronize(st));
    RNERF_CHECK_HIP(hipMemcpy(h.data(), trace, h.size() * sizeof(long long), hipMemcpyDeviceToHost));
    long long t0 = h[0];
    for (int i = 0; i < n_wg; ++i) t0 = h[2 * i] < t0 ? h[2 * i] : t0;
    for (int j = 0; j < tab.n; ++j) {
      long long a = -1, b = 0; double busy = 0;
      for (int i = tab.wg0[j]; i < tab.wg0[j + 1]; ++i) { a = (a < 0 || h[2 * i] < a) ? h[2 * i] : a; b = h[2 * i + 1] > b ? h[2 * i + 1] : b; busy += (double)(h[2 * i + 1] - h[2 * i]); }
      fprintf(stderr, "[wgrad trace] job %2d (KT %d NT %d) wgs %4d  first start %9lld  last end %9lld  mean wg ticks (100 MHz) %7.0f\n", j, tab.job[j].KT, tab.job[j].NT,
              tab.wg0[j + 1] - tab.wg0[j], a - t0, b - t0, busy / (tab.wg0[j + 1] - tab.wg0[j]));
    }
  }
  return RNERF_OK;
}

extern "C" int rnerf_bkgd_forward(const float* params, const float* dirs, int32_t dir_stride, int64_t n, double rgb_padding,
                                  float* out_rgb, void* stream) {
  RNERF_CHECK_ARG(params && dirs && out_rgb, "rnerf_bkgd_forward: null pointer");
  RNERF_CHECK_ARG(dir_stride >= 3, "rnerf_bkgd_forward: dir_stride must be >= 3");
  RNERF_CHECK_ARG(n >= 1, "rnerf_bkgd_forward: n must be >= 1");
  return launch_bkgd16_fwd(false, params, dirs, dir_stride, (long long)n, (float)(1 + 2 * rgb_padding), (float)rgb_padding, out_rgb, nullptr, (hipStream_t)stream);
}

extern "C" size_t rnerf_bkgd_save_bytes(int64_t n) { return bkgd_save_floats(n) * sizeof(float); }
extern "C" size_t rnerf_bkgd_dy_bytes(int64_t n) { return bkgd_dy_floats(n) * sizeof(float); }

extern "C" int rnerf_bkgd_forward_train(const float* params, const float* dirs, int32_t dir_stride, int64_t n, double rgb_padding,
                                        float* out_rgb, void* save, void* stream) {
  RNERF_CHECK_ARG(params && dirs && out_rgb && save, "rnerf_bkgd_forward_train: null pointer");
  RNERF_CHECK_ARG(dir_stride >= 3 && n >= 1, "rnerf_bkgd_forward_train: need dir_stride >= 3 and n >= 1");
  return launch_bkgd16_fwd(true, params, dirs, dir_stride, (long long)n, (float)(1 + 2 * rgb_padding), (float)rgb_padding, out_rgb, (float*)save, (hipStream_t)stream);
}

extern "C" int rnerf_bkgd_backward(const float* params, const void* save, const float* d_out, int64_t n, double rgb_padding, void* dy,
                                   float* grads, float* d_dirs, void* stream) {
  RNERF_CHECK_ARG(params && save && d_out && dy && grads, "rnerf_bkgd_backward: null pointer");
  RNERF_CHECK_ARG(n >= 1, "rnerf_bkgd_backward: n must be >= 1");
  hipStream_t st = (hipStream_t)stream;
  const float* sv = (const float*)save;
  float* dyf = (float*)dy;
  hipLaunchKernelGGL(bkgd_dgrad_kernel, dim3((unsigned)((n + 31) / 32)), dim3(64), 0, st, params, sv, d_out, (long long)n, (float)(1 + 2 * rgb_padding),
                     (float)rgb_padding, dyf, (float4*)d_dirs);
  RNERF_CHECK_LAUNCH();
  const unsigned chunks = (unsigned)((n + 255) / 256);
  float* partial = dyf + (size_t)n * 5 * 128;
  hipLaunchKernelGGL(bkgd_wgrad_kernel<0>, dim3(((chunks + 7) / 8) * 8 * SmallNet<0>::UNITS), dim3(256), 0, st, sv, (const float*)dyf, (long long)n, partial);
  hipLaunchKernelGGL(bkgd_wgrad_reduce_kernel<RNERF_BKGDMLP_PARAMS>, dim3((RNERF_BKGDMLP_PARAMS + 255) / 256), dim3(256), 0, st, (const float*)partial, (int)chunks,
                     grads);
  RNERF_CHECK_LAUNCH();
  return RNERF_OK;
}

extern "C" int rnerf_so3_query(const float* table, const rnerf_grid* g, const float* so3_params, const float* window10, const float* pts,
                               const float* condition, int64_t n, float* out4, float* pred_grad, void* stream) {
  RNERF_CHECK_ARG(table && g && so3_params && window10 && pts && out4 && pred_grad, "rnerf_so3_query: null pointer");
  RNERF_CHECK_ARG(n >= 1, "rnerf_so3_query: n must be >= 1");
  GridParams gp;
  RNERF_CHECK_ARG(make_grid_params(g, &gp), "rnerf_so3_query: bad grid");
  So3Window w;
  for (int i = 0; i < 10; ++i) w.w[i] = window10[i];
  hipLaunchKernelGGL(so3_query_kernel, dim3((unsigned)((n + 31) / 32)), dim3(64), 0, (hipStream_t)stream, (const float4*)table, gp, so3_params, w,
                     pts, condition, (long long)n, (float4*)out4, pred_grad);
  RNERF_CHECK_LAUNCH();
  return RNERF_OK;
}

extern "C" size_t rnerf_so3_packed_bytes(void) { return (size_t)kSo3Blocks * 128 * sizeof(uint4); }

extern "C" int rnerf_march_all(const float* table, const rnerf_grid* g, const float* so3_params, void* so3_packed, const float* window10, const float* origins,
                               const float* viewdirs, int32_t B, double near, double far, int32_t num_nodes, float* path_pd, float* path_dr,
                               float* path_ior, const int32_t* ray_order, void* stream) {
  RNERF_CHECK_ARG(table && g && so3_params && so3_packed && window10 && origins && viewdirs && path_pd && path_dr, "rnerf_march_all: null pointer");
  RNERF_CHECK_ARG(B > 0 && num_nodes >= 2, "rnerf_march_all: need B > 0 and num_nodes >= 2");
  GridParams gp;
  RNERF_CHECK_ARG(make_grid_params(g, &gp), "rnerf_march_all: bad grid");
  So3Window w;
  for (int i = 0; i < 10; ++i) w.w[i] = window10[i];
  RNERF_CHECK_ARG(grid_fits_u32(gp), "rnerf_march_all: grid too large for 32-bit byte offsets (needs a table < 4 GiB)");
  const float stepf = (float)((far - near) / (num_nodes - 1));
  hipLaunchKernelGGL(so3_pack16_kernel, dim3((kSo3Blocks * 64 + 255) / 256), dim3(256), 0, (hipStream_t)stream, so3_params, (uint4*)so3_packed);
  hipLaunchKernelGGL(march_all_kernel, dim3((unsigned)((B + 15) / 16)), dim3(256), 0, (hipStream_t)stream, (const float4*)table, gp, so3_params,
                     (const uint4*)so3_packed, w, origins, viewdirs, B, (float)near, stepf, num_nodes, (float4*)path_pd, (float4*)path_dr, (float4*)path_ior,
                     (float4*)nullptr, (int*)nullptr, 0, (int2*)nullptr, (float4*)nullptr, (float4*)nullptr, (int*)nullptr, (const int*)ray_order);
  RNERF_CHECK_LAUNCH();
  return RNERF_OK;
}

#include "ior_train_api.inc"
```

### samplenerfro_amd/csrc/pipeline.hip

```cpp
#include "common.h"

#include <math.h>
#include <mutex>
#include <utility>
#include <vector>

namespace rnerf {
static int current_device_cus() {
  static int cache[64] = {0};
  int dev = 0;
  if (hipGetDevice(&dev) != hipSuccess || dev < 0 || dev >= 64) return 256;
  if (cache[dev] == 0) {
    int cus = 0;
    cache[dev] = (hipDeviceGetAttribute(&cus, hipDeviceAttributeMultiprocessorCount, dev) == hipSuccess && cus > 0) ? cus : 256;
  }
  return cache[dev];
}

namespace {
constexpr size_t kPoolCap = 32;
struct EventPool { std::vector<hipEvent_t> free_[64]; };
thread_local EventPool tl_pool;
inline hipError_t pool_get(hipEvent_t* e) {
  int dev = 0;
// ... 132 lines not shown
    float v = g[i];
    if (wd2 != 0.f) v = v + theta[i] * wd2;
    const bool nf = !(fabsf(v) <= 3.402823466e38f);
    bad += nf;
    if (max_val > 0.f && !nf) v = fminf(fmaxf(v, -max_val), max_val);
    g[i] = v;
    s += v * v;
  }
  __shared__ float red[4];
  __shared__ int redb[4];
  for (int o = 32; o > 0; o >>= 1) { s += __shfl_down(s, o); bad += __shfl_down(bad, o); }
  if ((threadIdx.x & 63) == 0) { red[threadIdx.x >> 6] = s; redb[threadIdx.x >> 6] = bad; }
  __syncthreads();
  if (threadIdx.x == 0) {
    if (want_norm) partial[blockIdx.x] = (red[0] + red[1]) + (red[2] + red[3]);
    bad_partial[blockIdx.x] = (float)((redb[0] + redb[1]) + (redb[2] + redb[3]));
    if (step_inc && blockIdx.x == 0) *step_inc = *step_inc + 1;
  }
}
__global__ void __launch_bounds__(256) adam_frozen_sq_kernel(const float* __restrict__ frozen, long long n, float wd2, float max_val,
                                                             float* __restrict__ partial) {
  float s = 0.f;
  for (long long i = (long long)blockIdx.x * blockDim.x + threadIdx.x; i < n; i += (long long)gridDim.x * blockDim.x) {
    float v = frozen[i] * wd2;
    if (max_val > 0.f) v = fminf(fmaxf(v, -max_val), max_val);
    s += v * v;
  }
  __shared__ float red[4];
  for (int o = 32; o > 0; o >>= 1) s += __shfl_down(s, o);
  if ((threadIdx.x & 63) == 0) red[threadIdx.x >> 6] = s;
  __syncthreads();
  if (threadIdx.x == 0) partial[blockIdx.x] = (red[0] + red[1]) + (red[2] + red[3]);
}
struct AdamSched { double lr_init, lr_final, lr_delay_mult, max_steps, lr_delay_steps, b1, b2, max_norm, lr_override; int use_override, skip_nonfinite; };
__device__ __forceinline__ void adam_scalars_block(const AdamSched& c, int count, const float* __restrict__ partial, int n_partial,
                                                   const float* __restrict__ bad_partial, double* red, float* out) {
  double s = 0.0;
  for (int i = threadIdx.x; i < n_partial; i += 256) s += (double)partial[i];
  red[threadIdx.x] = s;
  __syncthreads();
  for (int o = 128; o > 0; o >>= 1) { if ((int)threadIdx.x < o) red[threadIdx.x] += red[threadIdx.x + o]; __syncthreads(); }
  const double sumsq = red[0];
  __syncthreads();
  double nb = 0.0;
  if (bad_partial) for (int i = threadIdx.x; i < ADAM_BLOCKS; i += 256) nb += (double)bad_partial[i];
  red[threadIdx.x] = nb;
  __syncthreads();
  for (int o = 128; o > 0; o >>= 1) { if ((int)threadIdx.x < o) red[threadIdx.x] += red[threadIdx.x + o]; __syncthreads(); }
  if (threadIdx.x != 0) return;
  const double t = (double)count + 1.0;
  double lr;
  if (c.use_override) {
    lr = c.lr_override;
  } else {
    double delay = 1.0;
    if (c.lr_delay_steps > 0) {
      const double x = fmin(fmax((double)count / c.lr_delay_steps, 0.0), 1.0);
      delay = c.lr_delay_mult + (1.0 - c.lr_delay_mult) * sin(0.5 * 3.141592653589793 * x);
    }
    const double start = fmin(fmax((double)count, 0.0), 1.0);
    const double tt = fmin(fmax(fmax((double)count, 0.0) / c.max_steps, 0.0), 1.0);
    lr = start * delay * exp(log(c.lr_init) * (1.0 - tt) + log(c.lr_final) * tt);
  }
  const double bad = red[0];
  out[0] = (float)(-lr / (1.0 - pow(c.b1, t)));
  out[1] = (c.skip_nonfinite && bad > 0.0) ? -1.0f : (float)(1.0 / (1.0 - pow(c.b2, t)));
  float mult = 1.0f;
  if (c.max_norm > 0) {
    const float norm = sqrtf((float)sumsq);
    mult = fminf((float)c.max_norm / (1e-7f + norm), 1.0f);
  }
  out[2] = mult;
  out[3] = (float)bad;
}
__global__ void __launch_bounds__(256) adam_scalars_kernel(AdamSched c, int* __restrict__ step, const float* __restrict__ partial, int n_partial,
                                                           const float* __restrict__ bad_partial, float* __restrict__ scal) {
  __shared__ double red[256];
  const int count = *step;
  adam_scalars_block(c, count, partial, n_partial, bad_partial, red, scal);
  if (threadIdx.x == 0) *step = count + 1;
}
__global__ void __launch_bounds__(256) adam_apply_kernel(float* __restrict__ theta, float* __restrict__ mu, float* __restrict__ nu,
                                                         const float* __restrict__ g, long long n, float b1, float b2, float eps,
                                                         float* __restrict__ scal, int count_bad) {
  const float a = scal[0], c2 = scal[1], mult = scal[2];
  if (c2 < 0.f) return;
  int bad = 0;
  for (long long i = (long long)blockIdx.x * blockDim.x + threadIdx.x; i < n; i += (long long)gridDim.x * blockDim.x) {
    const float gi = g[i] * mult;
    bad += !(fabsf(gi) <= 3.402823466e38f);
    const float m = mu[i] * b1 + gi * (1.0f - b1);
    const float v = nu[i] * b2 + (gi * gi) * (1.0f - b2);
    mu[i] = m; nu[i] = v;
    theta[i] = theta[i] + a * (m / (sqrtf(v * c2) + eps));
  }
  if (count_bad && __builtin_amdgcn_ballot_w64(bad != 0) != 0) {
    for (int o = 32; o > 0; o >>= 1) bad += __shfl_down(bad, o);
    if ((threadIdx.x & 63) == 0 && bad) atomicAdd(&scal[3], (float)bad);
  }
}

__global__ void __launch_bounds__(256) adam_apply_fused_kernel(AdamSched c, const int* __restrict__ step, const float* __restrict__ partial,
                                                               int n_partial, const float* __restrict__ bad_partial, float* __restrict__ theta,
                                                               float* __restrict__ mu, float* __restrict__ nu, const float* __restrict__ g,
                                                               long long n, float b1, float b2, float eps, float* __restrict__ scal,
                                                               float* __restrict__ count_out) {
  __shared__ double red[256];
  __shared__ float sc[4];
  adam_scalars_block(c, *step - 1, partial, n_partial, bad_partial, red, sc);
  __syncthreads();
  const float a = sc[0], c2 = sc[1], mult = sc[2];
  if (blockIdx.x == 0 && threadIdx.x == 0) {
    scal[0] = a; scal[1] = c2; scal[2] = mult; scal[3] = sc[3];
    if (count_out) *count_out = sc[3];
  }
  if (c2 < 0.f) return;
  for (long long i = (long long)blockIdx.x * blockDim.x + threadIdx.x; i < n; i += (long long)gridDim.x * blockDim.x) {
    const float gi = g[i] * mult;
    const float m = mu[i] * b1 + gi * (1.0f - b1);
    const float v = nu[i] * b2 + (gi * gi) * (1.0f - b2);
    mu[i] = m; nu[i] = v;
    theta[i] = theta[i] + a * (m / (sqrtf(v * c2) + eps));
  }
}

struct Carver {
  char* base; size_t off;
  explicit Carver(void* b) : base((char*)b), off(0) {}
  template <typename T> T* take(size_t count) {
    off = (off + 255) & ~(size_t)255;
    T* p = (T*)(base ? base + off : nullptr);
    off += count * sizeof(T);
    return p;
  }
  void* bytes(size_t n) { return (void*)take<char>(n); }
};

struct FwdBuffers {
  float *path_pd, *path_dr, *bk_dirs, *bkgd, *raw_c, *weights, *u, *rows_pd, *rows_dr, *scratch, *raw_f, *tmp_level, *tmp_level2;
};
static size_t carve_forward(const rnerf_model* m, int32_t B, bool own_path, void* ws, FwdBuffers* f) {
  Carver c(ws);
  const size_t Nc = m->num_coarse, Nf = m->num_fine, N = Nc * (size_t)m->num_path, S = Nc + Nf;
  f->path_pd = own_path ? c.take<float>(N * B * 4) : nullptr;
  f->path_dr = own_path ? c.take<float>(N * B * 4) : nullptr;
  f->bk_dirs = c.take<float>((size_t)B * 4);
  f->bkgd = c.take<float>((size_t)B * 3);
  f->raw_c = c.take<float>(Nc * B * 4);
  f->weights = c.take<float>(Nc * B);
  f->u = f->rows_pd = f->rows_dr = f->scratch = f->raw_f = f->tmp_level = f->tmp_level2 = nullptr;
  if (Nf > 0) {
    f->u = c.take<float>(Nf * (size_t)B);
    f->rows_pd = c.take<float>(S * B * 4);
    f->rows_dr = c.take<float>(S * B * 4);
    f->scratch = c.take<float>(S * B);
    f->raw_f = c.take<float>(S * B * 4);
    if (m->bd_cut) { f->tmp_level = c.take<float>((size_t)RNERF_LEVEL_FLOATS * B); f->tmp_level2 = c.take<float>((size_t)RNERF_LEVEL_FLOATS * B); }
  }
  return (c.off + 255) & ~(size_t)255;
}

static int check_model(const rnerf_model* m, int32_t B, const char* who) {
  RNERF_CHECK_ARG(m, "%s: null model", who);
  RNERF_CHECK_ARG(m->table, "%s: model.table is null", who);
  RNERF_CHECK_ARG(B >= 1, "%s: B must be >= 1", who);
  RNERF_CHECK_ARG(m->num_coarse >= 3 && m->num_fine >= 0 && m->num_path >= 1, "%s: need num_coarse >= 3, num_fine >= 0, num_path >= 1", who);
  RNERF_CHECK_ARG((long long)m->num_coarse * m->num_path >= 2, "%s: need at least two eikonal nodes", who);
  return RNERF_OK;
}

static inline int level_mask_mode(const rnerf_model* m) { return m->bd_cut == 2 ? 3 : 0; }
static inline const double* level_mask_box(const rnerf_model* m) { return m->bd_cut == 2 ? m->bd_cut_bbox : nullptr; }
struct Level { float *rgb, *dist, *acc, *trans, *tb; };
static Level level_of(float* out, int32_t B) { return Level{out, out + 3 * (size_t)B, out + 4 * (size_t)B, out + 5 * (size_t)B, out + 6 * (size_t)B}; }

static int bd_cut_pair(const rnerf_model* m, const float* raw_f, const float* rows_pd, const float* rows_dr, int32_t S, int32_t B, const float* bkgd,
                       Level out, float* tmp1, float* tmp2, void* stream) {
  Level a = level_of(tmp1, B), b = level_of(tmp2, B);
  int rc = rnerf_composite(raw_f, rows_pd, rows_dr, nullptr, S, B, nullptr, m->white_bkgd, m->rgb_padding, m->sigma_bias, a.rgb, a.dist, a.acc, out.trans,
                           a.tb, nullptr, nullptr, 1, m->bd_cut_bbox, stream);
  if (rc) return rc;
  rc = rnerf_composite(raw_f, rows_pd, rows_dr, nullptr, S, B, bkgd, m->white_bkgd, m->rgb_padding, m->sigma_bias, b.rgb, b.dist, b.acc, b.trans, b.tb, nullptr,
                       nullptr, 2, m->bd_cut_bbox, stream);
  if (rc) return rc;
  hipLaunchKernelGGL(bd_cut_mul_kernel, dim3((3 * B + 255) / 256), dim3(256), 0, (hipStream_t)stream, out.trans, b.rgb, B, out.tb);
  RNERF_CHECK_LAUNCH();
  return RNERF_OK;
}

static int make_u(const rnerf_model* m, int32_t B, int randomized, const uint32_t* key_u_dev, float* u, int32_t* per_ray, void* stream) {
  const double eps = 1.1920928955078125e-07;
  if (randomized) {
    *per_ray = 1;
    return rnerf_stratified_u_dev(key_u_dev, B, m->num_fine, u, stream);
  }
  *per_ray = 0;
  hipLaunchKernelGGL(linspace_u_kernel, dim3((m->num_fine + 255) / 256), dim3(256), 0, (hipStream_t)stream, m->num_fine, 1.0 - eps, u);
  RNERF_CHECK_LAUNCH();
  return RNERF_OK;
}

}

using namespace rnerf;

#define RNERF_TRY(expr)        \
  do {                         \
    int rc_ = (expr);          \
    if (rc_ != RNERF_OK) return rc_; \
  } while (0)

extern "C" int rnerf_rng_split3(uint32_t* rng_state, uint32_t* keys4, void* stream) {
  RNERF_CHECK_ARG(rng_state && keys4, "rnerf_rng_split3: null pointer");
  hipLaunchKernelGGL(rng_split3_kernel, dim3(1), dim3(64), 0, (hipStream_t)stream, rng_state, keys4);
  RNERF_CHECK_LAUNCH();
  return RNERF_OK;
}

extern "C" int rnerf_rng_forward(const uint32_t* keys4, int32_t num_coarse, int32_t num_path, int32_t use_random_choice, int32_t* jitter, uint32_t* key_u,
                                 void* stream) {
  RNERF_CHECK_ARG(keys4 && jitter, "rnerf_rng_forward: null pointer");
  RNERF_CHECK_ARG(num_coarse >= 1 && num_path >= 1, "rnerf_rng_forward: need num_coarse >= 1 and num_path >= 1");
  hipLaunchKernelGGL(rng_forward_kernel, dim3((num_coarse + 255) / 256), dim3(256), 0, (hipStream_t)stream, keys4, num_coarse, num_path, use_random_choice,
                     jitter, key_u);
  RNERF_CHECK_LAUNCH();
  return RNERF_OK;
}

extern "C" int rnerf_stratified_u_dev(const uint32_t* key_dev, int32_t B, int32_t num_fine, float* u, void* stream) {
  RNERF_CHECK_ARG(key_dev && u, "rnerf_stratified_u_dev: null pointer");
  RNERF_CHECK_ARG(B >= 1 && num_fine >= 1, "rnerf_stratified_u_dev: need B >= 1 and num_fine >= 1");
  const double eps = 1.1920928955078125e-07, s = 1.0 / num_fine;
  const long long half = ((long long)B * num_fine + 1) / 2;
  hipLaunchKernelGGL(stratified_u_dev_kernel, dim3((unsigned)((half + 255) / 256)), dim3(256), 0, (hipStream_t)stream, key_dev, B, num_fine, (float)s,
                     (float)(s - eps), (float)(1.0 - eps), u);
  RNERF_CHECK_LAUNCH();
  return RNERF_OK;
}

extern "C" size_t rnerf_forward_workspace_bytes(const rnerf_model* m, int32_t B) {
  if (!m || B < 1) return 0;
  FwdBuffers f;
  return carve_forward(m, B, true, nullptr, &f);
}

extern "C" int rnerf_forward(const rnerf_model* m, const float* origins, const float* viewdirs, int32_t B, const int32_t* jitter, const float* u_fine,
                             int32_t u_per_ray, const float* path_pd, const float* path_dr, float* out_coarse, float* out_fine, void* workspace,
                             int32_t max_workgroups, void* stream) {
  RNERF_TRY(check_model(m, B, "rnerf_forward"));
  RNERF_CHECK_ARG(jitter && out_coarse && workspace, "rnerf_forward: null pointer");
  RNERF_CHECK_ARG((path_pd == nullptr) == (path_dr == nullptr), "rnerf_forward: give both path_pd and path_dr or neither");
  RNERF_CHECK_ARG(path_pd || (origins && viewdirs), "rnerf_forward: origins / viewdirs are null and no marched path was given");
  RNERF_CHECK_ARG(m->packed_coarse && m->bkgd_params, "rnerf_forward: model.packed_coarse / bkgd_params are null");
  RNERF_CHECK_ARG(m->num_fine == 0 || (m->packed_fine && out_fine && u_fine), "rnerf_forward: num_fine > 0 needs packed_fine, out_fine and u_fine");
  RNERF_CHECK_ARG(((uintptr_t)workspace & 255) == 0, "rnerf_forward: workspace must be 256-byte aligned");
  const int32_t Nc = m->num_coarse, Nf = m->num_fine, N = Nc * m->num_path, S = Nc + Nf;
  FwdBuffers f;
  carve_forward(m, B, path_pd == nullptr, workspace, &f);
  if (!path_pd) {
    RNERF_TRY(rnerf_march(m->table, &m->grid, origins, viewdirs, B, m->near, m->far, N, f.path_pd, f.path_dr, nullptr, nullptr, stream));
    path_pd = f.path_pd; path_dr = f.path_dr;
  }
  hipStream_t st = (hipStream_t)stream;
  hipLaunchKernelGGL(bkgd_dirs_kernel, dim3((B + 255) / 256), dim3(256), 0, st, (const float4*)path_dr, jitter, Nc, B, (const float*)nullptr, 0, (float4*)f.bk_dirs);
  RNERF_CHECK_LAUNCH();
  RNERF_TRY(rnerf_bkgd_forward(m->bkgd_params, f.bk_dirs, 4, B, m->rgb_padding, f.bkgd, stream));
  RNERF_TRY(rnerf_nerfmlp_forward(m->packed_coarse, m->precision, path_pd, path_dr, jitter, Nc, B, f.raw_c, max_workgroups, stream));
  Level c = level_of(out_coarse, B);
  RNERF_TRY(rnerf_composite(f.raw_c, path_pd, path_dr, jitter, Nc, B, f.bkgd, m->white_bkgd, m->rgb_padding, m->sigma_bias, c.rgb, c.dist, c.acc, c.trans, c.tb,
                            Nf > 0 ? f.weights : nullptr, nullptr, level_mask_mode(m), level_mask_box(m), stream));
  if (Nf > 0) {
    RNERF_TRY(rnerf_resample(path_pd, path_dr, N, B, jitter, Nc, f.weights, u_fine, u_per_ray, Nf, f.rows_pd, f.rows_dr, nullptr, f.scratch, stream));
    RNERF_TRY(rnerf_nerfmlp_forward(m->packed_fine, m->precision, f.rows_pd, f.rows_dr, nullptr, S, B, f.raw_f, max_workgroups, stream));
    Level o = level_of(out_fine, B);
    RNERF_TRY(rnerf_composite(f.raw_f, f.rows_pd, f.rows_dr, nullptr, S, B, f.bkgd, m->white_bkgd, m->rgb_padding, m->sigma_bias, o.rgb, o.dist, o.acc, o.trans,
                              o.tb, nullptr, nullptr, level_mask_mode(m), level_mask_box(m), stream));
    if (m->bd_cut == 1) RNERF_TRY(bd_cut_pair(m, f.raw_f, f.rows_pd, f.rows_dr, S, B, f.bkgd, o, f.tmp_level, f.tmp_level2, stream));
  }
  return RNERF_OK;
}

namespace rnerf {
static bool levels_side_by_side(const rnerf_model* m, const rnerf_train_cfg* c, int32_t B) {
  if (m->num_fine <= 0 || !c->aux_stream) return false;
  const int cus = current_device_cus();
  const long long tiles_both = ((long long)m->num_coarse * B + 255) / 256 + ((long long)(m->num_coarse + m->num_fine) * B + 255) / 256;
  return tiles_both <= 2LL * cus;
}
struct TrainBuffers {
  FwdBuffers f;
  int32_t* jitter; uint32_t* key_u;
  void *packed_c, *packed_f, *packed_bwd, *packed_bwd_f, *save_c, *save_f, *save_bk, *dy, *dy_bk, *wgrad_ws;
  void *dy_c, *wgrad_ws_c;
  float *out_all, *level_c, *level_f, *sums, *d_all, *d_raw, *env_sum, *d_raw_c;
};
static size_t carve_train(const rnerf_model* m, const rnerf_train_cfg* c, int32_t B, bool own_path, void* ws, TrainBuffers* t) {
  const size_t Nc = m->num_coarse, Nf = m->num_fine, S = Nc + Nf;
  const size_t M = c->bg_smooth_weight > 0 ? (size_t)c->bg_patch_size * c->bg_patch_size : 0;
  Carver k(ws);
  const size_t N = Nc * (size_t)m->num_path;
  FwdBuffers& f = t->f;
  f.path_pd = own_path ? k.take<float>(N * B * 4) : nullptr;
  f.path_dr = own_path ? k.take<float>(N * B * 4) : nullptr;
  f.bk_dirs = k.take<float>((B + M) * 4);
  t->out_all = k.take<float>((B + M) * 3);
  f.bkgd = t->out_all;
  f.raw_c = k.take<float>(Nc * B * 4);
  f.weights = k.take<float>(Nc * B);
  f.u = f.rows_pd = f.rows_dr = f.scratch = f.raw_f = f.tmp_level = f.tmp_level2 = nullptr;
  if (Nf > 0) {
    f.u = k.take<float>(Nf * (size_t)B);
    f.rows_pd = k.take<float>(S * B * 4);
    f.rows_dr = k.take<float>(S * B * 4);
    f.scratch = k.take<float>(S * B);
    f.raw_f = k.take<float>(S * B * 4);
    if (m->bd_cut) { f.tmp_level = k.take<float>((size_t)RNERF_LEVEL_FLOATS * B); f.tmp_level2 = k.take<float>((size_t)RNERF_LEVEL_FLOATS * B); }
  }
  t->jitter = k.take<int32_t>(Nc);
  t->key_u = k.take<uint32_t>(4);
  t->packed_c = k.bytes(rnerf_nerfmlp_packed_bytes(RNERF_PREC_F16X3));
  t->packed_f = Nf > 0 ? k.bytes(rnerf_nerfmlp_packed_bytes(RNERF_PREC_F16X3)) : nullptr;
  t->packed_bwd = k.bytes(rnerf_nerfmlp_bwd_packed_bytes());
  t->packed_bwd_f = Nf > 0 ? k.bytes(rnerf_nerfmlp_bwd_packed_bytes()) : nullptr;
  t->save_c = k.bytes(rnerf_nerfmlp_save_bytes((int64_t)Nc * B, c->backward));
  t->save_f = Nf > 0 ? k.bytes(rnerf_nerfmlp_save_bytes((int64_t)S * B, c->backward)) : nullptr;
  t->save_bk = k.bytes(rnerf_bkgd_save_bytes((int64_t)(B + M)));
  t->dy = k.bytes(rnerf_nerfmlp_dy_bytes((int64_t)S * B, c->backward));
  t->dy_bk = k.bytes(rnerf_bkgd_dy_bytes((int64_t)(B + M)));
  t->wgrad_ws = k.bytes(rnerf_nerfmlp_wgrad_workspace_bytes());
  t->level_c = k.take<float>((size_t)RNERF_LEVEL_FLOATS * B);
  t->level_f = Nf > 0 ? k.take<float>((size_t)RNERF_LEVEL_FLOATS * B) : nullptr;
  t->sums = k.take<float>(4);
  t->env_sum = k.take<float>(rnerf_env_smooth_sum_floats(c->bg_smooth_weight > 0 ? c->bg_patch_size : 0));
  t->d_all = k.take<float>((B + M) * 3);
  t->d_raw = k.take<float>(S * B * 4);
  t->dy_c = t->wgrad_ws_c = nullptr; t->d_raw_c = nullptr;
  if (levels_side_by_side(m, c, B)) {
    t->dy_c = k.bytes(rnerf_nerfmlp_dy_bytes((int64_t)Nc * B, c->backward));
    t->wgrad_ws_c = k.bytes(rnerf_nerfmlp_wgrad_workspace_bytes());
    t->d_raw_c = k.take<float>(Nc * B * 4);
  }
  return (k.off + 255) & ~(size_t)255;
}
}

extern "C" size_t rnerf_train_workspace_bytes(const rnerf_model* m, const rnerf_train_cfg* c, int32_t B) {
  if (!m || !c || B < 1) return 0;
  TrainBuffers t;
  return carve_train(m, c, B, true, nullptr, &t);
}

static int mark_point(hipStream_t first, hipEvent_t* out);
static int wait_point(hipStream_t then, hipEvent_t e);

extern "C" int rnerf_train_forward_backward(const rnerf_model* m, const rnerf_train_cfg* c, const float* theta, const float* origins, const float* viewdirs,
                                            const float* pixels, const float* env_dirs, int32_t B, const uint32_t* keys4, const int32_t* jitter_override,
                                            const float* u_override, int32_t u_per_ray, const float* path_pd, const float* path_dr, float* grads,
                                            void* workspace, int32_t max_workgroups, const rnerf_prefetch* next, void* stream) {
  RNERF_TRY(check_model(m, B, "rnerf_train_forward_backward"));
  RNERF_CHECK_ARG(c && theta && pixels && grads && workspace, "rnerf_train_forward_backward: null pointer");
  RNERF_CHECK_ARG(keys4 || (jitter_override && (m->num_fine == 0 || u_override || !c->randomized)),
                  "rnerf_train_forward_backward: give keys4, or the jitter (and the stratified draws) explicitly");
  RNERF_CHECK_ARG((path_pd == nullptr) == (path_dr == nullptr), "rnerf_train_forward_backward: give both path_pd and path_dr or neither");
  RNERF_CHECK_ARG(path_pd || (origins && viewdirs), "rnerf_train_forward_backward: origins / viewdirs are null and no marched path was given");
  RNERF_CHECK_ARG(m->precision == RNERF_PREC_F16X3 || (m->precision == RNERF_PREC_F16 && c->backward != RNERF_BWD_F16X3 && c->backward != RNERF_BWD_F16X3_LO8) ||
                      (m->precision == RNERF_PREC_BF16X3 && c->backward == RNERF_BWD_BF16),
                  "rnerf_train_forward_backward: training is built on the f16x3 forward (f16: with backward f16 / bf16 only; bf16x3 + backward bf16: the range-safe step)");
  RNERF_CHECK_ARG(((uintptr_t)workspace & 255) == 0, "rnerf_train_forward_backward: workspace must be 256-byte aligned");
  const bool smooth = c->bg_smooth_weight > 0;
  RNERF_CHECK_ARG(!smooth || (env_dirs && c->bg_patch_size >= 2), "rnerf_train_forward_backward: bg_smooth_weight > 0 needs env_dirs and bg_patch_size >= 2");
  const int32_t Nc = m->num_coarse, Nf = m->num_fine, N = Nc * m->num_path, S = Nc + Nf;
  const int32_t ps = smooth ? c->bg_patch_size : 0, M = ps * ps;
  const int bwd = c->backward, prec = m->precision;
  hipStream_t st = (hipStream_t)stream;
  TrainBuffers t;
  carve_train(m, c, B, path_pd == nullptr, workspace, &t);
  FwdBuffers& f = t.f;
  const float* th_c = theta;
  const float* th_f = Nf > 0 ? theta + RNERF_NERFMLP_PARAMS : nullptr;
  const float* th_b = theta + (size_t)RNERF_NERFMLP_PARAMS * (Nf > 0 ? 2 : 1);
  const int64_t n_theta = (int64_t)RNERF_NERFMLP_PARAMS * (Nf > 0 ? 2 : 1) + RNERF_BKGDMLP_PARAMS;
  float* g_c = grads;
  float* g_f = Nf > 0 ? grads + RNERF_NERFMLP_PARAMS : nullptr;
  float* g_b = grads + (size_t)RNERF_NERFMLP_PARAMS * (Nf > 0 ? 2 : 1);
  float* stats8 = grads + n_theta;

  void* aux = c->aux_stream;
  bool pre_zeroed = false;
  struct Mark { hipEvent_t e = nullptr; ~Mark() { if (e) pool_put(e); } } fine_packed;
  if (aux) {
    RNERF_TRY(rnerf_fork(stream, aux));
    void* streams[2] = {t.packed_c, t.packed_f};
    void* dys[2] = {t.dy, t.dy_c};
    const int64_t dy_rows[2] = {(int64_t)(Nf > 0 ? S : Nc) * B, (int64_t)Nc * B};
    RNERF_TRY(nerfmlp_step_zero(prec, streams, Nf > 0 ? 2 : 1, bwd, dys, dy_rows, t.dy_c ? 2 : 1, (hipStream_t)aux));
    pre_zeroed = true;
    RNERF_TRY(nerfmlp_pack_impl(th_c, prec, t.packed_c, false, (hipStream_t)aux, false));
  }
  const int32_t* jitter = jitter_override;
  if (keys4) {
    RNERF_TRY(rnerf_rng_forward(keys4, Nc, m->num_path, c->use_random_choice, t.jitter, t.key_u, stream));
    if (!jitter_override) jitter = t.jitter;
  }
  if (!path_pd) {
    RNERF_TRY(rnerf_march(m->table, &m->grid, origins, viewdirs, B, m->near, m->far, N, f.path_pd, f.path_dr, nullptr, nullptr, stream));
    path_pd = f.path_pd; path_dr = f.path_dr;
  }
  hipLaunchKernelGGL(bkgd_dirs_kernel, dim3((B + M + 255) / 256), dim3(256), 0, st, (const float4*)path_dr, jitter, Nc, B, env_dirs, M, (float4*)f.bk_dirs);
  RNERF_CHECK_LAUNCH();
  RNERF_TRY(rnerf_bkgd_forward_train(th_b, f.bk_dirs, 4, (int64_t)B + M, m->rgb_padding, t.out_all, t.save_bk, stream));
  const float* bkgd = t.out_all;
  const float* rgb_env = t.out_all + (size_t)3 * B;
  if (aux) {
    RNERF_TRY(rnerf_join(stream, aux));
    if (Nf > 0) {
      RNERF_TRY(nerfmlp_pack_impl(th_f, prec, t.packed_f, false, (hipStream_t)aux, false));
      RNERF_TRY(mark_point((hipStream_t)aux, &fine_packed.e));
    }
    RNERF_CHECK_HIP(hipMemsetAsync(grads, 0, (size_t)(n_theta + 8) * sizeof(float), (hipStream_t)aux));
    RNERF_TRY(rnerf_nerfmlp_pack_bwd(th_c, bwd, t.packed_bwd, aux));
    if (Nf > 0) RNERF_TRY(rnerf_nerfmlp_pack_bwd(th_f, bwd, t.packed_bwd_f, aux));
    RNERF_TRY(rnerf_theta_sumsq(theta, n_theta, stats8, aux));
  } else {
    RNERF_TRY(rnerf_nerfmlp_pack(th_c, prec, t.packed_c, stream));
  }
  RNERF_TRY(rnerf_nerfmlp_forward_train(t.packed_c, prec, path_pd, path_dr, jitter, Nc, B, f.raw_c, t.save_c, bwd, max_workgroups, stream));
  Level lc = level_of(t.level_c, B);
  RNERF_TRY(rnerf_composite(f.raw_c, path_pd, path_dr, jitter, Nc, B, bkgd, m->white_bkgd, m->rgb_padding, m->sigma_bias, lc.rgb, lc.dist, lc.acc, lc.trans, lc.tb,
                            Nf > 0 ? f.weights : nullptr, nullptr, level_mask_mode(m), level_mask_box(m), stream));
  Level lf = lc;
  if (Nf > 0) {
    const float* u = u_override;
    int32_t per_ray = u_per_ray;
    if (!u) { RNERF_TRY(make_u(m, B, c->randomized, t.key_u, f.u, &per_ray, stream)); u = f.u; }
    RNERF_TRY(rnerf_resample(path_pd, path_dr, N, B, jitter, Nc, f.weights, u, per_ray, Nf, f.rows_pd, f.rows_dr, nullptr, f.scratch, stream));
    if (!aux) RNERF_TRY(rnerf_nerfmlp_pack(th_f, prec, t.packed_f, stream));
    else { hipEvent_t e = fine_packed.e; fine_packed.e = nullptr; RNERF_TRY(wait_point(st, e)); }
    RNERF_TRY(rnerf_nerfmlp_forward_train(t.packed_f, prec, f.rows_pd, f.rows_dr, nullptr, S, B, f.raw_f, t.save_f, bwd, max_workgroups, stream));
    lf = level_of(t.level_f, B);
    RNERF_TRY(rnerf_composite(f.raw_f, f.rows_pd, f.rows_dr, nullptr, S, B, bkgd, m->white_bkgd, m->rgb_padding, m->sigma_bias, lf.rgb, lf.dist, lf.acc, lf.trans,
                              lf.tb, nullptr, nullptr, level_mask_mode(m), level_mask_box(m), stream));
    if (m->bd_cut == 1) RNERF_TRY(bd_cut_pair(m, f.raw_f, f.rows_pd, f.rows_dr, S, B, bkgd, lf, f.tmp_level, f.tmp_level2, stream));
  }
  RNERF_TRY(rnerf_loss_reduce(Nf > 0 ? lc.rgb : nullptr, lf.rgb, lf.trans, lf.tb, pixels, B, t.sums, stream));
  const double bg_on = (c->bg_weight > 0 && c->annealed_alpha > 0) ? 1.0 : 0.0;
  const double mse_scale = 2.0 / (3.0 * B);
  const double env_on = c->annealed_alpha > 0 ? 1.0 : 0.0;
  if (!aux) RNERF_CHECK_HIP(hipMemsetAsync(grads, 0, (size_t)(n_theta + 8) * sizeof(float), st));
  auto march_next = [&]() -> int {
    RNERF_CHECK_ARG(next->origins && next->viewdirs && next->path_pd && next->path_dr && next->side_stream, "rnerf_train_forward_backward: incomplete rnerf_prefetch");
    RNERF_TRY(rnerf_fork(stream, next->side_stream));
    return rnerf_march(m->table, &m->grid, next->origins, next->viewdirs, B, m->near, m->far, N, next->path_pd, next->path_dr, nullptr, nullptr,
                       next->side_stream);
  };
  if (aux) RNERF_TRY(rnerf_join(stream, aux));
  float* d_first = t.d_all;
  const bool split_levels = levels_side_by_side(m, c, B);
  float* d_raw_c = split_levels ? t.d_raw_c : t.d_raw;
  void* dy_c = split_levels ? t.dy_c : t.dy;
  if (Nf > 0) {
    RNERF_TRY(rnerf_composite_backward(f.raw_f, f.rows_pd, f.rows_dr, nullptr, S, B, bkgd, m->rgb_padding, m->sigma_bias, lf.rgb, pixels, lf.trans, lf.tb, t.sums,
                                       mse_scale, c->bg_weight * bg_on, t.d_raw, d_first, 0, m->white_bkgd, m->bd_cut == 1 ? 1 : level_mask_mode(m), m->bd_cut ? m->bd_cut_bbox : nullptr, stream));
    if (split_levels) {
      RNERF_TRY(rnerf_composite_backward(f.raw_c, path_pd, path_dr, jitter, Nc, B, bkgd, m->rgb_padding, m->sigma_bias, lc.rgb, pixels, nullptr, nullptr, nullptr,
                                         mse_scale, 0.0, d_raw_c, d_first, 1, m->white_bkgd, level_mask_mode(m), level_mask_box(m), stream));
      RNERF_TRY(rnerf_fork(stream, aux));
      if (smooth) RNERF_TRY(rnerf_env_smooth_backward(rgb_env, ps, c->bg_smooth_weight * env_on, t.d_all + (size_t)3 * B, t.env_sum, aux));
      RNERF_TRY(rnerf_bkgd_backward(th_b, t.save_bk, t.d_all, (int64_t)B + M, m->rgb_padding, t.dy_bk, g_b, nullptr, aux));
      RNERF_TRY(nerfmlp_dgrad_impl(t.packed_bwd, t.packed_c, prec, bwd, t.save_c, d_raw_c, (int64_t)Nc * B, dy_c, !pre_zeroed, false, (hipStream_t)aux));
      RNERF_TRY(rnerf_nerfmlp_wgrad(prec, bwd, t.save_c, dy_c, (int64_t)Nc * B, g_c, t.wgrad_ws_c, aux));
    }
    if (!aux) RNERF_TRY(rnerf_nerfmlp_pack_bwd(th_f, bwd, t.packed_bwd_f, stream));
    RNERF_TRY(nerfmlp_dgrad_impl(t.packed_bwd_f, t.packed_f, prec, bwd, t.save_f, t.d_raw, (int64_t)S * B, t.dy, !pre_zeroed, !split_levels, st));
    if (next) RNERF_TRY(march_next());
    RNERF_TRY(rnerf_nerfmlp_wgrad(prec, bwd, t.save_f, t.dy, (int64_t)S * B, g_f, t.wgrad_ws, stream));
    if (split_levels)
      RNERF_TRY(rnerf_join(stream, aux));
    else
      RNERF_TRY(rnerf_composite_backward(f.raw_c, path_pd, path_dr, jitter, Nc, B, bkgd, m->rgb_padding, m->sigma_bias, lc.rgb, pixels, nullptr, nullptr, nullptr,
                                         mse_scale, 0.0, t.d_raw, d_first, 1, m->white_bkgd, level_mask_mode(m), level_mask_box(m), stream));
  } else {
    RNERF_TRY(rnerf_composite_backward(f.raw_c, path_pd, path_dr, jitter, Nc, B, bkgd, m->rgb_padding, m->sigma_bias, lf.rgb, pixels, lf.trans, lf.tb, t.sums,
                                       mse_scale, c->bg_weight * bg_on, t.d_raw, d_first, 0, m->white_bkgd, level_mask_mode(m), level_mask_box(m), stream));
  }
  if (!aux) RNERF_TRY(rnerf_nerfmlp_pack_bwd(th_c, bwd, t.packed_bwd, stream));
  if (!split_levels)
    RNERF_TRY(nerfmlp_dgrad_impl(t.packed_bwd, t.packed_c, prec, bwd, t.save_c, t.d_raw, (int64_t)Nc * B, t.dy, !(pre_zeroed && Nf == 0), true, st));
  if (next && Nf == 0) RNERF_TRY(march_next());
  const bool tail_on_aux = aux && !split_levels;
  void* tail = tail_on_aux ? aux : stream;
  if (tail_on_aux) RNERF_TRY(rnerf_fork(stream, aux));
  if (!split_levels && !tail_on_aux) RNERF_TRY(rnerf_nerfmlp_wgrad(prec, bwd, t.save_c, t.dy, (int64_t)Nc * B, g_c, t.wgrad_ws, stream));
  if (!tail_on_aux && c->grads_stream) RNERF_TRY(rnerf_fork(stream, c->grads_stream));
  if (!split_levels) {
    if (smooth) RNERF_TRY(rnerf_env_smooth_backward(rgb_env, ps, c->bg_smooth_weight * env_on, t.d_all + (size_t)3 * B, t.env_sum, tail));
    RNERF_TRY(rnerf_bkgd_backward(th_b, t.save_bk, t.d_all, (int64_t)B + M, m->rgb_padding, t.dy_bk, g_b, nullptr, tail));
  }
  RNERF_TRY(rnerf_train_stats(t.sums, B, Nf > 0, c->bg_weight * bg_on, smooth ? t.env_sum : nullptr, ps, env_on, aux ? nullptr : theta, n_theta, c->frozen_sq,
                              n_theta + c->frozen_count, stats8, tail));
  if (tail_on_aux) {
    RNERF_TRY(rnerf_nerfmlp_wgrad(prec, bwd, t.save_c, t.dy, (int64_t)Nc * B, g_c, t.wgrad_ws, stream));
    if (c->grads_stream) RNERF_TRY(rnerf_fork(stream, c->grads_stream));
    RNERF_TRY(rnerf_join(stream, aux));
  }
  return RNERF_OK;
}

static int adam_update_impl(const rnerf_adam_cfg* c, float* theta, float* mu, float* nu, float* grads, int64_t n_theta, const float* frozen_params,
                            int64_t n_frozen, int32_t* step_counter, float* scratch, bool fused, float* count_out, hipStream_t st) {
  const double wd2 = c->weight_decay_mult > 0 ? 2.0 * c->weight_decay_mult / (double)c->n_all : 0.0;
  const int want_norm = c->grad_max_norm > 0;
  float* scal = scratch;
  float* partial = scratch + 4;
  float* bad_partial = nullptr;
  int n_partial = 0;
  if (wd2 != 0.0 || c->grad_max_val > 0 || want_norm || c->skip_nonfinite) {
    bad_partial = scratch + 4 + 2 * ADAM_BLOCKS;
    hipLaunchKernelGGL(adam_prep_kernel, dim3(ADAM_BLOCKS), dim3(256), 0, st, (const float*)theta, grads, (long long)n_theta, (float)wd2, (float)c->grad_max_val,
                       want_norm, partial, bad_partial, fused ? step_counter : nullptr);
    if (want_norm) {
      n_partial = ADAM_BLOCKS;
      if (frozen_params && n_frozen > 0 && wd2 != 0.0) {
        hipLaunchKernelGGL(adam_frozen_sq_kernel, dim3(ADAM_BLOCKS), dim3(256), 0, st, frozen_params, (long long)n_frozen, (float)wd2, (float)c->grad_max_val,
                           partial + ADAM_BLOCKS);
        n_partial = 2 * ADAM_BLOCKS;
      }
    }
  }
  AdamSched s{c->lr_init, c->lr_final, c->lr_delay_mult, (double)c->max_steps, (double)c->lr_delay_steps, c->b1, c->b2, c->grad_max_norm, c->lr_override, c->use_lr_override != 0,
              c->skip_nonfinite != 0};
  if (fused && bad_partial) {
    hipLaunchKernelGGL(adam_apply_fused_kernel, dim3(ADAM_BLOCKS), dim3(256), 0, st, s, (const int*)step_counter, (const float*)partial, n_partial,
                       (const float*)bad_partial, theta, mu, nu, (const float*)grads, (long long)n_theta, (float)c->b1, (float)c->b2, (float)c->eps, scal, count_out);
    RNERF_CHECK_LAUNCH();
    return RNERF_OK;
  }
  hipLaunchKernelGGL(adam_scalars_kernel, dim3(1), dim3(256), 0, st, s, step_counter, (const float*)partial, n_partial, (const float*)bad_partial, scal);
  hipLaunchKernelGGL(adam_apply_kernel, dim3(ADAM_BLOCKS), dim3(256), 0, st, theta, mu, nu, (const float*)grads, (long long)n_theta, (float)c->b1, (float)c->b2,
                     (float)c->eps, scal, bad_partial == nullptr);
  RNERF_CHECK_LAUNCH();
  if (count_out) RNERF_CHECK_HIP(hipMemcpyAsync(count_out, scal + 3, sizeof(float), hipMemcpyDefault, st));
  return RNERF_OK;
}

extern "C" int rnerf_adam_update(const rnerf_adam_cfg* c, float* theta, float* mu, float* nu, float* grads, int64_t n_theta, const float* frozen_params,
                                 int64_t n_frozen, int32_t* step_counter, float* scratch, void* stream) {
  RNERF_CHECK_ARG(c && theta && mu && nu && grads && step_counter && scratch, "rnerf_adam_update: null pointer");
  RNERF_CHECK_ARG(n_theta >= 1 && c->n_all >= n_theta, "rnerf_adam_update: need n_theta >= 1 and n_all >= n_theta");
  return adam_update_impl(c, theta, mu, nu, grads, n_theta, frozen_params, n_frozen, step_counter, scratch, false, nullptr, (hipStream_t)stream);
}

extern "C" int rnerf_adam_update_fused(const rnerf_adam_cfg* c, float* theta, float* mu, float* nu, float* grads, int64_t n_theta, const float* frozen_params,
                                       int64_t n_frozen, int32_t* step_counter, float* scratch, float* nonfinite_out, void* stream) {
  RNERF_CHECK_ARG(c && theta && mu && nu && grads && step_counter && scratch, "rnerf_adam_update_fused: null pointer");
  RNERF_CHECK_ARG(n_theta >= 1 && c->n_all >= n_theta, "rnerf_adam_update_fused: need n_theta >= 1 and n_all >= n_theta");
  return adam_update_impl(c, theta, mu, nu, grads, n_theta, frozen_params, n_frozen, step_counter, scratch, true, nonfinite_out, (hipStream_t)stream);
}

namespace {
std::mutex g_ev_mu;
thread_local std::vector<hipEvent_t> tl_capture_events;
std::vector<std::pair<void*, std::vector<hipEvent_t>>> g_graph_events;
void drop_events(std::vector<hipEvent_t>& v) {
  for (hipEvent_t e : v) (void)hipEventDestroy(e);
  v.clear();
}
}

extern "C" int rnerf_graph_begin(void* stream) {
  drop_events(tl_capture_events);
  RNERF_CHECK_HIP(hipStreamBeginCapture((hipStream_t)stream, hipStreamCaptureModeThreadLocal));
  return RNERF_OK;
}

extern "C" int rnerf_graph_end(void* stream, void** graph_exec) {
  RNERF_CHECK_ARG(graph_exec, "rnerf_graph_end: null pointer");
  hipGraph_t g = nullptr;
  hipError_t err = hipStreamEndCapture((hipStream_t)stream, &g);
  if (err != hipSuccess) { drop_events(tl_capture_events); set_error("hipStreamEndCapture failed: %s", hipGetErrorString(err)); return RNERF_ERR_HIP; }
  hipGraphExec_t e = nullptr;
  err = hipGraphInstantiate(&e, g, nullptr, nullptr, 0);
  hipGraphDestroy(g);
  if (err != hipSuccess) { drop_events(tl_capture_events); set_error("hipGraphInstantiate failed: %s", hipGetErrorString(err)); return RNERF_ERR_HIP; }
  {
    std::lock_guard<std::mutex> l(g_ev_mu);
    g_graph_events.emplace_back((void*)e, std::move(tl_capture_events));
  }
  tl_capture_events.clear();
  *graph_exec = (void*)e;
  return RNERF_OK;
}

extern "C" int rnerf_graph_launch(void* graph_exec, void* stream) {
  RNERF_CHECK_ARG(graph_exec, "rnerf_graph_launch: null graph");
  RNERF_CHECK_HIP(hipGraphLaunch((hipGraphExec_t)graph_exec, (hipStream_t)stream));
  return RNERF_OK;
}

extern "C" int rnerf_graph_destroy(void* graph_exec) {
  if (!graph_exec) return RNERF_OK;
  std::vector<hipEvent_t> ev;
  {
    std::lock_guard<std::mutex> l(g_ev_mu);
    for (size_t i = 0; i < g_graph_events.size(); ++i)
      if (g_graph_events[i].first == graph_exec) { ev = std::move(g_graph_events[i].second); g_graph_events.erase(g_graph_events.begin() + i); break; }
  }
  RNERF_CHECK_HIP(hipGraphExecDestroy((hipGraphExec_t)graph_exec));
  drop_events(ev);
  return RNERF_OK;
}

static int order_after(hipStream_t first, hipStream_t then) {
  hipEvent_t e = nullptr;
  RNERF_CHECK_HIP(pool_get(&e));
  hipStreamCaptureStatus cs = hipStreamCaptureStatusNone;
  hipError_t err = hipStreamIsCapturing(first, &cs);
  if (err == hipSuccess) err = hipEventRecord(e, first);
  if (err == hipSuccess) err = hipStreamWaitEvent(then, e, 0);
  if (err != hipSuccess) {
    (void)hipEventDestroy(e);
    set_error("stream ordering failed: %s", hipGetErrorString(err));
    return RNERF_ERR_HIP;
  }
  if (cs == hipStreamCaptureStatusNone) pool_put(e);
  else tl_capture_events.push_back(e);
  return RNERF_OK;
}

static int mark_point(hipStream_t first, hipEvent_t* out) {
  hipEvent_t e = nullptr;
  RNERF_CHECK_HIP(pool_get(&e));
  const hipError_t err = hipEventRecord(e, first);
  if (err != hipSuccess) { (void)hipEventDestroy(e); set_error("stream ordering failed: %s", hipGetErrorString(err)); return RNERF_ERR_HIP; }
  *out = e;
  return RNERF_OK;
}
static int wait_point(hipStream_t then, hipEvent_t e) {
  hipStreamCaptureStatus cs = hipStreamCaptureStatusNone;
  hipError_t err = hipStreamIsCapturing(then, &cs);
  if (err == hipSuccess) err = hipStreamWaitEvent(then, e, 0);
  if (err != hipSuccess) { (void)hipEventDestroy(e); set_error("stream ordering failed: %s", hipGetErrorString(err)); return RNERF_ERR_HIP; }
  if (cs == hipStreamCaptureStatusNone) pool_put(e);
  else tl_capture_events.push_back(e);
  return RNERF_OK;
}

extern "C" int rnerf_fork(void* main_stream, void* side_stream) { return order_after((hipStream_t)main_stream, (hipStream_t)side_stream); }
extern "C" int rnerf_join(void* main_stream, void* side_stream) { return order_after((hipStream_t)side_stream, (hipStream_t)main_stream); }
```

Measured before the change: 671,900.

## Fuse bkgd dir gather, split env rows onto aux, vectorize wgrad reduce

```diff
diff --git a/include/rnerf.h b/include/rnerf.h
--- a/include/rnerf.h
+++ b/include/rnerf.h
@@ -142,11 +142,15 @@
                         int64_t rows, void* dy, void* stream);
 int rnerf_nerfmlp_wgrad(int fwd_precision, int backward, const void* save, const void* dy, int64_t rows, float* grads, void* workspace,
                         void* stream);
+int rnerf_nerfmlp_wgrad_reduce_ref(int backward, const void* dy, int64_t rows, const void* workspace, float* grads, void* stream);
 
 size_t rnerf_bkgd_save_bytes(int64_t n);
 size_t rnerf_bkgd_dy_bytes(int64_t n);
 int rnerf_bkgd_forward_train(const float* params, const float* dirs, int32_t dir_stride, int64_t n, double rgb_padding,
                              float* out_rgb, void* save, void* stream);
+int rnerf_bkgd_forward_train_rows(const float* params, const float* dirs, int32_t dir_stride, int64_t dir_row0, const float* gather_dr,
+                                  const int32_t* gather_node, int32_t gather_B, int64_t n, int64_t row0, int64_t row1, double rgb_padding,
+                                  float* out_rgb, void* save, void* stream);
 int rnerf_bkgd_backward(const float* params, const void* save, const float* d_out, int64_t n, double rgb_padding, void* dy,
                         float* grads, float* d_dirs, void* stream);
 
diff --git a/samplenerfro_amd/_lib.py b/samplenerfro_amd/_lib.py
--- a/samplenerfro_amd/_lib.py
+++ b/samplenerfro_amd/_lib.py
@@ -110,6 +110,8 @@
     "rnerf_bkgd_save_bytes": (C.c_size_t, [_i64]),
     "rnerf_bkgd_dy_bytes": (C.c_size_t, [_i64]),
     "rnerf_bkgd_forward_train": (C.c_int, [_vp, _vp, _i32, _i64, _dbl, _vp, _vp, _vp]),
+    "rnerf_bkgd_forward_train_rows": (C.c_int, [_vp, _vp, _i32, _i64, _vp, _vp, _i32, _i64, _i64, _i64, _dbl, _vp, _vp, _vp]),
+    "rnerf_nerfmlp_wgrad_reduce_ref": (C.c_int, [_i32, _vp, _i64, _vp, _vp, _vp]),
     "rnerf_bkgd_backward": (C.c_int, [_vp, _vp, _vp, _i64, _dbl, _vp, _vp, _vp, _vp]),
     "rnerf_theta_sumsq": (C.c_int, [_vp, _i64, _vp, _vp]),
     "rnerf_march_all_train": (C.c_int, [_vp, _GP, _vp, _vp, _vp, _vp, _vp, _i32, _dbl, _dbl, _i32, _vp, _vp, _vp, _vp, _i32, _vp, _vp, _vp, _vp, _vp, _vp]),
diff --git a/samplenerfro_amd/csrc/bkgd16.hip b/samplenerfro_amd/csrc/bkgd16.hip
--- a/samplenerfro_amd/csrc/bkgd16.hip
+++ b/samplenerfro_amd/csrc/bkgd16.hip
@@ -101,13 +101,21 @@
 
 template <bool TRAIN>
 __global__ void __launch_bounds__(64) bkgd16_fwd_kernel(const float* __restrict__ params, const float* __restrict__ dirs, int dir_stride,
-                                                        long long n, float pad_scale, float pad, float* __restrict__ out_rgb,
-                                                        float* __restrict__ save) {
+                                                        long long dir_row0, const float4* __restrict__ gather, const int* __restrict__ gather_node,
+                                                        int gather_B, long long n, long long row0, long long row1, float pad_scale, float pad,
+                                                        float* __restrict__ out_rgb, float* __restrict__ save) {
   const int lane = threadIdx.x & 63, m = lane & 31, h = lane >> 5;
-  long long row = (long long)blockIdx.x * 32 + m;
-  const bool ok = row < n;
-  if (!ok) row = n - 1;
-  const float v0 = dirs[row * dir_stride], v1 = dirs[row * dir_stride + 1], v2 = dirs[row * dir_stride + 2];
+  long long row = row0 + (long long)blockIdx.x * 32 + m;
+  const bool ok = row < row1;
+  if (!ok) row = row1 - 1;
+  float v0, v1, v2;
+  if (gather) {
+    const float4 d = gather[(size_t)gather_node[0] * gather_B + row];
+    v0 = d.x; v1 = d.y; v2 = d.z;
+  } else {
+    const float* __restrict__ dp = dirs + (row - dir_row0) * dir_stride;
+    v0 = dp[0]; v1 = dp[1]; v2 = dp[2];
+  }
   float enc[14];
   const float phase = h ? 1.5707963705062866f : 0.0f;
 #pragma unroll
@@ -180,13 +188,21 @@
   }
 }
 
+int launch_bkgd16_fwd_rows(bool train, const float* params, const float* dirs, int dir_stride, long long dir_row0, const float4* gather,
+                           const int* gather_node, int gather_B, long long n, long long row0, long long row1, float pad_scale, float pad,
+                           float* out_rgb, float* save, hipStream_t st) {
+  const dim3 grid((unsigned)((row1 - row0 + 31) / 32));
+  if (train) hipLaunchKernelGGL(bkgd16_fwd_kernel<true>, grid, dim3(64), 0, st, params, dirs, dir_stride, dir_row0, gather, gather_node, gather_B, n, row0, row1,
+                                pad_scale, pad, out_rgb, save);
+  else hipLaunchKernelGGL(bkgd16_fwd_kernel<false>, grid, dim3(64), 0, st, params, dirs, dir_stride, dir_row0, gather, gather_node, gather_B, n, row0, row1,
+                          pad_scale, pad, out_rgb, save);
+  RNERF_CHECK_LAUNCH();
+  return RNERF_OK;
+}
+
 int launch_bkgd16_fwd(bool train, const float* params, const float* dirs, int dir_stride, long long n, float pad_scale, float pad, float* out_rgb,
                       float* save, hipStream_t st) {
-  const dim3 grid((unsigned)((n + 31) / 32));
-  if (train) hipLaunchKernelGGL(bkgd16_fwd_kernel<true>, grid, dim3(64), 0, st, params, dirs, dir_stride, n, pad_scale, pad, out_rgb, save);
-  else hipLaunchKernelGGL(bkgd16_fwd_kernel<false>, grid, dim3(64), 0, st, params, dirs, dir_stride, n, pad_scale, pad, out_rgb, save);
-  RNERF_CHECK_LAUNCH();
-  return RNERF_OK;
+  return launch_bkgd16_fwd_rows(train, params, dirs, dir_stride, 0, nullptr, nullptr, 0, n, 0, n, pad_scale, pad, out_rgb, save, st);
 }
 
 template <bool FIRST>
diff --git a/samplenerfro_amd/csrc/bkgd_layout.h b/samplenerfro_amd/csrc/bkgd_layout.h
--- a/samplenerfro_amd/csrc/bkgd_layout.h
+++ b/samplenerfro_amd/csrc/bkgd_layout.h
@@ -22,5 +22,8 @@
 
 int launch_bkgd16_fwd(bool train, const float* params, const float* dirs, int dir_stride, long long n, float pad_scale, float pad, float* out_rgb,
                       float* save, hipStream_t st);
+int launch_bkgd16_fwd_rows(bool train, const float* params, const float* dirs, int dir_stride, long long dir_row0, const float4* gather,
+                           const int* gather_node, int gather_B, long long n, long long row0, long long row1, float pad_scale, float pad,
+                           float* out_rgb, float* save, hipStream_t st);
 
 }
diff --git a/samplenerfro_amd/csrc/mlp.hip b/samplenerfro_amd/csrc/mlp.hip
--- a/samplenerfro_amd/csrc/mlp.hip
+++ b/samplenerfro_amd/csrc/mlp.hip
@@ -1874,6 +1874,52 @@
   __builtin_trap();
 }
 
+__device__ __forceinline__ int wgrad_out_feature(const WgradJob& job, int J, int& dense) {
+  int nt = J >> 5;
+  const int c = J & 31, a = c >> 4, hh = (c >> 3) & 1, j = c & 7;
+  const bool segb = nt >= job.NTa;
+  const int dkind = segb ? job.dkind2 : job.dkind;
+  dense = segb ? job.dense2 : job.dense;
+  if (segb) nt -= job.NTa;
+  if (dkind == 0) { const int n = prev_feature(2 * nt + a, hh, j); return n < nerf_dense(dense).out ? n : -1; }
+  if (a != 0 || hh != 0 || nt != 0) return -1;
+  if (dkind == 1) return j == 0 ? 0 : -1;
+  return (j >= 1 && j <= 3) ? j - 1 : -1;
+}
+__device__ __forceinline__ int wgrad_elem_dest(const WgradJob& job, int e) {
+  const int ldn = job.NT * 32;
+  const int I = e / ldn, J = e % ldn;
+  int kt = I >> 5;
+  const int c = I & 31, a = c >> 4, hh = (c >> 3) & 1, j = c & 7;
+  const bool segb = kt >= job.KTa;
+  const int xkind = segb ? job.xkind2 : job.xkind, row_off = segb ? job.row_off2 : job.row_off;
+  if (segb) kt -= job.KTa;
+  const int s = 2 * kt + a;
+  int fin = xkind == 1 ? prev_feature(s, hh, j) : (xkind == 0 ? pe_feature(8 * s + j, hh) : view_feature(8 * s + j, hh));
+  int dense;
+  const int fout = wgrad_out_feature(job, J, dense);
+  if (fin < 0 || fout < 0) return -1;
+  fin += row_off;
+  return fin < nerf_dense(dense).in ? nerf_koff(dense) + fin * nerf_dense(dense).out + fout : -1;
+}
+__device__ __forceinline__ float wgrad_sum_over(const float* __restrict__ p, size_t stride, int n_wg) {
+  float s0 = 0.f, s1 = 0.f, s2 = 0.f, s3 = 0.f;
+  int g = 0;
+  for (; g + 4 <= n_wg; g += 4) { s0 += p[(size_t)g * stride]; s1 += p[(size_t)(g + 1) * stride]; s2 += p[(size_t)(g + 2) * stride]; s3 += p[(size_t)(g + 3) * stride]; }
+  for (; g < n_wg; ++g) s0 += p[(size_t)g * stride];
+  return (s0 + s1) + (s2 + s3);
+}
+__device__ __forceinline__ void wgrad_reduce_bias(const float* __restrict__ partial_bias, const WgradJob& job, int n_wg, int e, float osc,
+                                                  float* __restrict__ grads) {
+  const int ldn = job.NT * 32;
+  if (job.write_bias && e < ldn) {
+    int dense;
+    const int fout = wgrad_out_feature(job, e, dense);
+    if (fout >= 0 && (e >> 5) < job.NTa) grads[nerf_boff(dense) + fout] = wgrad_sum_over(partial_bias + e, (size_t)ldn, n_wg) * osc;
+    if (job.bias_sigma && e == 0) grads[nerf_boff(8)] = wgrad_sum_over(partial_bias, (size_t)ldn, n_wg) * osc;
+  }
+}
+
 __global__ void __launch_bounds__(256) wgrad_reduce_kernel(const float* __restrict__ workspace, const WgradTable tab, float* __restrict__ grads,
                                                            const float* __restrict__ out_scale) {
   const float osc = out_scale ? *out_scale : 1.0f;
@@ -1881,50 +1927,49 @@
   const WgradJob job = tab.job[jb];
   const int n_wg = tab.wg0[jb + 1] - tab.wg0[jb];
   const float* __restrict__ partial = workspace + tab.poff[jb];
-  const float* __restrict__ partial_bias = workspace + tab.pboff[jb];
   const int ldn = job.NT * 32, rows = job.KT * 32;
   const int e = blockIdx.x * blockDim.x + threadIdx.x;
-  auto out_feature = [&](int J, int& dense) -> int {
-    int nt = J >> 5;
-    const int c = J & 31, a = c >> 4, hh = (c >> 3) & 1, j = c & 7;
-    const bool segb = nt >= job.NTa;
-    const int dkind = segb ? job.dkind2 : job.dkind;
-    dense = segb ? job.dense2 : job.dense;
-    if (segb) nt -= job.NTa;
-    if (dkind == 0) { const int n = prev_feature(2 * nt + a, hh, j); return n < nerf_dense(dense).out ? n : -1; }
-    if (a != 0 || hh != 0 || nt != 0) return -1;
-    if (dkind == 1) return j == 0 ? 0 : -1;
-    return (j >= 1 && j <= 3) ? j - 1 : -1;
-  };
-  auto sum_over = [&](const float* __restrict__ p, size_t stride) -> float {
-    float s0 = 0.f, s1 = 0.f, s2 = 0.f, s3 = 0.f;
-    int g = 0;
-    for (; g + 4 <= n_wg; g += 4) { s0 += p[(size_t)g * stride]; s1 += p[(size_t)(g + 1) * stride]; s2 += p[(size_t)(g + 2) * stride]; s3 += p[(size_t)(g + 3) * stride]; }
-    for (; g < n_wg; ++g) s0 += p[(size_t)g * stride];
-    return (s0 + s1) + (s2 + s3);
-  };
   if (e < rows * ldn) {
-    const int I = e / ldn, J = e % ldn;
-    int kt = I >> 5;
-    const int c = I & 31, a = c >> 4, hh = (c >> 3) & 1, j = c & 7;
-    const bool segb = kt >= job.KTa;
-    const int xkind = segb ? job.xkind2 : job.xkind, row_off = segb ? job.row_off2 : job.row_off;
-    if (segb) kt -= job.KTa;
-    const int s = 2 * kt + a;
-    int fin = xkind == 1 ? prev_feature(s, hh, j) : (xkind == 0 ? pe_feature(8 * s + j, hh) : view_feature(8 * s + j, hh));
-    int dense;
-    const int fout = out_feature(J, dense);
-    if (fin >= 0 && fout >= 0) {
-      fin += row_off;
-      if (fin < nerf_dense(dense).in) grads[nerf_koff(dense) + fin * nerf_dense(dense).out + fout] = sum_over(partial + e, (size_t)rows * ldn) * osc;
-    }
-  }
-  if (job.write_bias && e < ldn) {
-    int dense;
-    const int fout = out_feature(e, dense);
-    if (fout >= 0 && (e >> 5) < job.NTa) grads[nerf_boff(dense) + fout] = sum_over(partial_bias + e, (size_t)ldn) * osc;
-    if (job.bias_sigma && e == 0) grads[nerf_boff(8)] = sum_over(partial_bias, (size_t)ldn) * osc;
-  }
+    const int dst = wgrad_elem_dest(job, e);
+    if (dst >= 0) grads[dst] = wgrad_sum_over(partial + e, (size_t)rows * ldn, n_wg) * osc;
+  }
+  wgrad_reduce_bias(workspace + tab.pboff[jb], job, n_wg, e, osc, grads);
+}
+
+__global__ void __launch_bounds__(256) wgrad_reduce4_kernel(const float* __restrict__ workspace, const WgradTable tab, float* __restrict__ grads,
+                                                            const float* __restrict__ out_scale) {
+  const float osc = out_scale ? *out_scale : 1.0f;
+  const int jb = blockIdx.y;
+  const WgradJob job = tab.job[jb];
+  const int n_wg = tab.wg0[jb + 1] - tab.wg0[jb];
+  const int elems = job.KT * job.NT * 1024;
+  if ((int)blockIdx.x * 256 < elems) {
+    const int lane = threadIdx.x & 63, q = lane >> 4;
+    const int e = blockIdx.x * 256 + (threadIdx.x >> 6) * 64 + (lane & 15) * 4;
+    const float4* __restrict__ p = (const float4*)(workspace + tab.poff[jb] + e);
+    const size_t stride = (size_t)elems / 4;
+    float4 s = make_float4(0.f, 0.f, 0.f, 0.f);
+    auto add = [&](int g) { const float4 v = p[(size_t)g * stride]; s.x += v.x; s.y += v.y; s.z += v.z; s.w += v.w; };
+    const int n4 = n_wg & ~3;
+#pragma unroll 4
+    for (int g = q; g < n4; g += 4) add(g);
+    if (q == 0) for (int g = n4; g < n_wg; ++g) add(g);
+    float r[4];
+    const float mine[4] = {s.x, s.y, s.z, s.w};
+#pragma unroll
+    for (int i = 0; i < 4; ++i) {
+      const float s1 = __shfl_down(mine[i], 16), s2 = __shfl_down(mine[i], 32), s3 = __shfl_down(mine[i], 48);
+      r[i] = (mine[i] + s1) + (s2 + s3);
+    }
+    if (q == 0) {
+#pragma unroll
+      for (int i = 0; i < 4; ++i) {
+        const int dst = wgrad_elem_dest(job, e + i);
+        if (dst >= 0) grads[dst] = r[i] * osc;
+      }
+    }
+  }
+  wgrad_reduce_bias(workspace + tab.pboff[jb], job, n_wg, blockIdx.x * blockDim.x + threadIdx.x, osc, grads);
 }
 
 template <int NSTEP, int NT, typename WF, typename XF>
@@ -3010,6 +3055,17 @@
   return w.partial_floats * sizeof(float) + (size_t)w.max_wgs * 2 * sizeof(long long);
 }
 
+static int launch_wgrad_reduce(const WgradTable& tab, const float* workspace, float* grads, const float* out_scale, bool reference, hipStream_t st) {
+  RNERF_CHECK_ARG(((uintptr_t)workspace & 15) == 0, "rnerf_nerfmlp_wgrad: workspace must be 16-byte aligned");
+  int max_elems = 0;
+  for (int j = 0; j < tab.n; ++j) max_elems = tab.job[j].KT * tab.job[j].NT * 1024 > max_elems ? tab.job[j].KT * tab.job[j].NT * 1024 : max_elems;
+  const dim3 grid((max_elems + 255) / 256, tab.n);
+  if (reference) hipLaunchKernelGGL(wgrad_reduce_kernel, grid, dim3(256), 0, st, workspace, tab, grads, out_scale);
+  else hipLaunchKernelGGL(wgrad_reduce4_kernel, grid, dim3(256), 0, st, workspace, tab, grads, out_scale);
+  RNERF_CHECK_LAUNCH();
+  return RNERF_OK;
+}
+
 extern "C" int rnerf_nerfmlp_wgrad(int fwd_precision, int backward, const void* save, const void* dy, int64_t rows, float* grads, void* workspace,
                                    void* stream) {
   RNERF_CHECK_ARG(save && dy && grads && workspace, "rnerf_nerfmlp_wgrad: null pointer");
@@ -3053,10 +3109,7 @@
                        (float*)workspace, tab, trace);
     out_scale = (const float*)((const uint4*)dy + dy_plane_uint4(R, 2)) + R;
   }
-  int max_elems = 0;
-  for (int j = 0; j < tab.n; ++j) max_elems = tab.job[j].KT * tab.job[j].NT * 1024 > max_elems ? tab.job[j].KT * tab.job[j].NT * 1024 : max_elems;
-  hipLaunchKernelGGL(wgrad_reduce_kernel, dim3((max_elems + 255) / 256, tab.n), dim3(256), 0, st, (const float*)workspace, tab, grads, out_scale);
-  RNERF_CHECK_LAUNCH();
+  RNERF_TRY_(launch_wgrad_reduce(tab, (const float*)workspace, grads, out_scale, false, st));
   if (trace && backward != RNERF_BWD_BF16) {
     const int n_wg = tab.wg0[tab.n];
     std::vector<long long> h(2 * (size_t)n_wg);
@@ -3072,6 +3125,27 @@
     }
   }
   return RNERF_OK;
+}
+
+extern "C" int rnerf_nerfmlp_wgrad_reduce_ref(int backward, const void* dy, int64_t rows, const void* workspace, float* grads, void* stream) {
+  RNERF_CHECK_ARG(dy && grads && workspace, "rnerf_nerfmlp_wgrad_reduce_ref: null pointer");
+  RNERF_CHECK_ARG(bwd_ok(backward) && rows >= 1, "rnerf_nerfmlp_wgrad_reduce_ref: unknown backward mode or rows < 1");
+  const WgradTables& w = wgrad_tables();
+  const long long R = (rows + 255) / 256 * 256;
+  const WgradTable& tab = backward == RNERF_BWD_BF16 ? w.legacy : (rows <= kWgradSmallRows ? w.tr_small : w.tr);
+  const float* out_scale = backward == RNERF_BWD_BF16 ? nullptr : (const float*)((const uint4*)dy + dy_plane_uint4(R, backward == RNERF_BWD_F16 ? 1 : 2)) + R;
+  return launch_wgrad_reduce(tab, (const float*)workspace, grads, out_scale, true, (hipStream_t)stream);
+}
+
+extern "C" int rnerf_bkgd_forward_train_rows(const float* params, const float* dirs, int32_t dir_stride, int64_t dir_row0, const float* gather_dr,
+                                             const int32_t* gather_node, int32_t gather_B, int64_t n, int64_t row0, int64_t row1,
+                                             double rgb_padding, float* out_rgb, void* save, void* stream) {
+  RNERF_CHECK_ARG(params && out_rgb && save, "rnerf_bkgd_forward_train_rows: null pointer");
+  RNERF_CHECK_ARG(0 <= row0 && row0 < row1 && row1 <= n, "rnerf_bkgd_forward_train_rows: need 0 <= row0 < row1 <= n");
+  RNERF_CHECK_ARG(gather_dr ? (gather_node && gather_B >= row1) : (dirs && dir_stride >= 3 && dir_row0 <= row0),
+                  "rnerf_bkgd_forward_train_rows: give dirs (dir_stride >= 3, dir_row0 <= row0) or gather_dr with gather_node and gather_B >= row1");
+  return launch_bkgd16_fwd_rows(true, params, dirs, dir_stride, (long long)dir_row0, (const float4*)gather_dr, gather_node, gather_B, (long long)n,
+                                (long long)row0, (long long)row1, (float)(1 + 2 * rgb_padding), (float)rgb_padding, out_rgb, (float*)save, (hipStream_t)stream);
 }
 
 extern "C" int rnerf_bkgd_forward(const float* params, const float* dirs, int32_t dir_stride, int64_t n, double rgb_padding,
diff --git a/samplenerfro_amd/csrc/pipeline.hip b/samplenerfro_amd/csrc/pipeline.hip
--- a/samplenerfro_amd/csrc/pipeline.hip
+++ b/samplenerfro_amd/csrc/pipeline.hip
@@ -458,7 +458,7 @@
   FwdBuffers& f = t->f;
   f.path_pd = own_path ? k.take<float>(N * B * 4) : nullptr;
   f.path_dr = own_path ? k.take<float>(N * B * 4) : nullptr;
-  f.bk_dirs = k.take<float>((B + M) * 4);
+  f.bk_dirs = nullptr;
   t->out_all = k.take<float>((B + M) * 3);
   f.bkgd = t->out_all;
   f.raw_c = k.take<float>(Nc * B * 4);
@@ -508,6 +508,7 @@
 
 static int mark_point(hipStream_t first, hipEvent_t* out);
 static int wait_point(hipStream_t then, hipEvent_t e);
+static int order_after2(hipStream_t first, hipStream_t then_a, hipStream_t then_b);
 
 extern "C" int rnerf_train_forward_backward(const rnerf_model* m, const rnerf_train_cfg* c, const float* theta, const float* origins, const float* viewdirs,
                                             const float* pixels, const float* env_dirs, int32_t B, const uint32_t* keys4, const int32_t* jitter_override,
@@ -543,7 +544,7 @@
 
   void* aux = c->aux_stream;
   bool pre_zeroed = false;
-  struct Mark { hipEvent_t e = nullptr; ~Mark() { if (e) pool_put(e); } } fine_packed;
+  struct Mark { hipEvent_t e = nullptr; ~Mark() { if (e) pool_put(e); } } fine_packed, head_done;
   if (aux) {
     RNERF_TRY(rnerf_fork(stream, aux));
     void* streams[2] = {t.packed_c, t.packed_f};
@@ -562,11 +563,12 @@
     RNERF_TRY(rnerf_march(m->table, &m->grid, origins, viewdirs, B, m->near, m->far, N, f.path_pd, f.path_dr, nullptr, nullptr, stream));
     path_pd = f.path_pd; path_dr = f.path_dr;
   }
-  hipLaunchKernelGGL(bkgd_dirs_kernel, dim3((B + M + 255) / 256), dim3(256), 0, st, (const float4*)path_dr, jitter, Nc, B, env_dirs, M, (float4*)f.bk_dirs);
-  RNERF_CHECK_LAUNCH();
-  RNERF_TRY(rnerf_bkgd_forward_train(th_b, f.bk_dirs, 4, (int64_t)B + M, m->rgb_padding, t.out_all, t.save_bk, stream));
+  RNERF_TRY(rnerf_bkgd_forward_train_rows(th_b, nullptr, 0, 0, path_dr, jitter + (Nc - 1), B, (int64_t)B + M, 0, B, m->rgb_padding, t.out_all, t.save_bk, stream));
   const float* bkgd = t.out_all;
   const float* rgb_env = t.out_all + (size_t)3 * B;
+  auto env_rows_forward = [&](void* s) -> int {
+    return rnerf_bkgd_forward_train_rows(th_b, env_dirs, 3, B, nullptr, nullptr, 0, (int64_t)B + M, B, (int64_t)B + M, m->rgb_padding, t.out_all, t.save_bk, s);
+  };
   if (aux) {
     RNERF_TRY(rnerf_join(stream, aux));
     if (Nf > 0) {
@@ -577,6 +579,8 @@
     RNERF_TRY(rnerf_nerfmlp_pack_bwd(th_c, bwd, t.packed_bwd, aux));
     if (Nf > 0) RNERF_TRY(rnerf_nerfmlp_pack_bwd(th_f, bwd, t.packed_bwd_f, aux));
     RNERF_TRY(rnerf_theta_sumsq(theta, n_theta, stats8, aux));
+    RNERF_TRY(mark_point((hipStream_t)aux, &head_done.e));
+    if (smooth) RNERF_TRY(env_rows_forward(aux));
   } else {
     RNERF_TRY(rnerf_nerfmlp_pack(th_c, prec, t.packed_c, stream));
   }
@@ -603,13 +607,16 @@
   const double mse_scale = 2.0 / (3.0 * B);
   const double env_on = c->annealed_alpha > 0 ? 1.0 : 0.0;
   if (!aux) RNERF_CHECK_HIP(hipMemsetAsync(grads, 0, (size_t)(n_theta + 8) * sizeof(float), st));
-  auto march_next = [&]() -> int {
-    RNERF_CHECK_ARG(next->origins && next->viewdirs && next->path_pd && next->path_dr && next->side_stream, "rnerf_train_forward_backward: incomplete rnerf_prefetch");
-    RNERF_TRY(rnerf_fork(stream, next->side_stream));
+  if (next) RNERF_CHECK_ARG(next->origins && next->viewdirs && next->path_pd && next->path_dr && next->side_stream, "rnerf_train_forward_backward: incomplete rnerf_prefetch");
+  auto march_on_side = [&]() -> int {
     return rnerf_march(m->table, &m->grid, next->origins, next->viewdirs, B, m->near, m->far, N, next->path_pd, next->path_dr, nullptr, nullptr,
                        next->side_stream);
   };
-  if (aux) RNERF_TRY(rnerf_join(stream, aux));
+  auto march_next = [&]() -> int {
+    RNERF_TRY(rnerf_fork(stream, next->side_stream));
+    return march_on_side();
+  };
+  if (aux) { hipEvent_t e = head_done.e; head_done.e = nullptr; RNERF_TRY(wait_point(st, e)); }
   float* d_first = t.d_all;
   const bool split_levels = levels_side_by_side(m, c, B);
   float* d_raw_c = split_levels ? t.d_raw_c : t.d_raw;
@@ -642,20 +649,28 @@
   if (!aux) RNERF_TRY(rnerf_nerfmlp_pack_bwd(th_c, bwd, t.packed_bwd, stream));
   if (!split_levels)
     RNERF_TRY(nerfmlp_dgrad_impl(t.packed_bwd, t.packed_c, prec, bwd, t.save_c, t.d_raw, (int64_t)Nc * B, t.dy, !(pre_zeroed && Nf == 0), true, st));
-  if (next && Nf == 0) RNERF_TRY(march_next());
   const bool tail_on_aux = aux && !split_levels;
+  const bool march_here = next && Nf == 0;
   void* tail = tail_on_aux ? aux : stream;
-  if (tail_on_aux) RNERF_TRY(rnerf_fork(stream, aux));
+  if (tail_on_aux) {
+    RNERF_TRY(order_after2(st, (hipStream_t)aux, march_here ? (hipStream_t)next->side_stream : nullptr));
+    RNERF_TRY(rnerf_nerfmlp_wgrad(prec, bwd, t.save_c, t.dy, (int64_t)Nc * B, g_c, t.wgrad_ws, stream));
+    if (march_here) RNERF_TRY(march_on_side());
+  } else if (march_here) {
+    RNERF_TRY(march_next());
+  }
   if (!split_levels && !tail_on_aux) RNERF_TRY(rnerf_nerfmlp_wgrad(prec, bwd, t.save_c, t.dy, (int64_t)Nc * B, g_c, t.wgrad_ws, stream));
   if (!tail_on_aux && c->grads_stream) RNERF_TRY(rnerf_fork(stream, c->grads_stream));
   if (!split_levels) {
-    if (smooth) RNERF_TRY(rnerf_env_smooth_backward(rgb_env, ps, c->bg_smooth_weight * env_on, t.d_all + (size_t)3 * B, t.env_sum, tail));
+    if (smooth) {
+      if (!aux) RNERF_TRY(env_rows_forward(tail));
+      RNERF_TRY(rnerf_env_smooth_backward(rgb_env, ps, c->bg_smooth_weight * env_on, t.d_all + (size_t)3 * B, t.env_sum, tail));
+    }
     RNERF_TRY(rnerf_bkgd_backward(th_b, t.save_bk, t.d_all, (int64_t)B + M, m->rgb_padding, t.dy_bk, g_b, nullptr, tail));
   }
   RNERF_TRY(rnerf_train_stats(t.sums, B, Nf > 0, c->bg_weight * bg_on, smooth ? t.env_sum : nullptr, ps, env_on, aux ? nullptr : theta, n_theta, c->frozen_sq,
                               n_theta + c->frozen_count, stats8, tail));
   if (tail_on_aux) {
-    RNERF_TRY(rnerf_nerfmlp_wgrad(prec, bwd, t.save_c, t.dy, (int64_t)Nc * B, g_c, t.wgrad_ws, stream));
     if (c->grads_stream) RNERF_TRY(rnerf_fork(stream, c->grads_stream));
     RNERF_TRY(rnerf_join(stream, aux));
   }
@@ -783,6 +798,24 @@
   return RNERF_OK;
 }
 
+static int order_after2(hipStream_t first, hipStream_t then_a, hipStream_t then_b) {
+  hipEvent_t e = nullptr;
+  RNERF_CHECK_HIP(pool_get(&e));
+  hipStreamCaptureStatus cs = hipStreamCaptureStatusNone;
+  hipError_t err = hipStreamIsCapturing(first, &cs);
+  if (err == hipSuccess) err = hipEventRecord(e, first);
+  if (err == hipSuccess) err = hipStreamWaitEvent(then_a, e, 0);
+  if (err == hipSuccess && then_b) err = hipStreamWaitEvent(then_b, e, 0);
+  if (err != hipSuccess) {
+    (void)hipEventDestroy(e);
+    set_error("stream ordering failed: %s", hipGetErrorString(err));
+    return RNERF_ERR_HIP;
+  }
+  if (cs == hipStreamCaptureStatusNone) pool_put(e);
+  else tl_capture_events.push_back(e);
+  return RNERF_OK;
+}
+
 static int mark_point(hipStream_t first, hipEvent_t* out) {
   hipEvent_t e = nullptr;
   RNERF_CHECK_HIP(pool_get(&e));
```

After: 675,700, median of 5. Within noise of the previous version (+0.6%).
